# huggingface/diffusers

Measured on AMD Instinct MI355X. Metric: images/sec @ SDXL-base 1024x1024 50-step EulerDiscrete CFG bf16, higher is better.
Workload: dtype bf16

## Files before the change

diffusers_amd/_lib.py:

```python
from __future__ import annotations

import ctypes as C
import threading
from pathlib import Path

_PKG = Path(__file__).resolve().parent
LIB_PATH = _PKG / "_C" / "libdiffusers_amd.so"

DA_OK = 0
ERRORS = {1: "DA_ERR_INVALID", 2: "DA_ERR_LAUNCH", 3: "DA_ERR_UNSUPPORTED"}
ACT_NONE, ACT_GEGLU, ACT_GELU_TANH, ACT_SILU, ACT_GELU_ERF, ACT_QUICK_GELU, ACT_GEGLU_TANH = 0, 1, 2, 3, 4, 5, 6
(TILE_AUTO, TILE_128x128, TILE_64x128, TILE_128x64, TILE_64x64, TILE_256x128, TILE_128x256, TILE_256x256,
 TILE_128x128_W8, TILE_K2_128x128, TILE_K2_128x80, TILE_K2_128x160, TILE_K2_80x128, TILE_K2_128x64,
 TILE_K1_128x320, TILE_K1_256x128, TILE_K1_128x256, TILE_K1_256x160, TILE_K1_256x256, TILE_K1_256x320,
 TILE_K3_256x256, TILE_K3_256x320) = range(22)
TILE_NAMES = ("auto", "128x128", "64x128", "128x64", "64x64", "256x128", "128x256", "256x256", "128x128w8",
              "k2:128x128", "k2:128x80", "k2:128x160", "k2:80x128", "k2:128x64",
              "k1:128x320", "k1:256x128", "k1:128x256", "k1:256x160", "k1:256x256", "k1:256x320",
              "k3:256x256", "k3:256x320")
FIRST_K2_TILE = TILE_K2_128x128
STAGE_REGISTER, STAGE_LDS_DIRECT, STAGE_LDS_DIRECT3, STAGE_LDS_DIRECT4, STAGE_LDS_DIRECT6, STAGE_LDS_DIRECT8 = range(6)
STAGE_PINGPONG, STAGE_PINGPONG3 = 6, 7
RING_SLOTS = (2, 2, 3, 4, 6, 8)
DTYPE_BF16, DTYPE_F32 = 0, 1
SPLITK_FLAGS = 4096
SPLITK_ERR_SLOT = SPLITK_FLAGS - 1
SPLITK_MAX = 24
PRED_EPSILON, PRED_V, PRED_SAMPLE = 0, 1, 2
PRED_TYPES = {"epsilon": PRED_EPSILON, "v_prediction": PRED_V, "sample": PRED_SAMPLE}


class GemmParams(C.Structure):
    _fields_ = [
        ("A", C.c_void_p), ("A2", C.c_void_p), ("W", C.c_void_p), ("C", C.c_void_p),
        ("bias", C.c_void_p), ("rowvec", C.c_void_p), ("residual", C.c_void_p),
        ("bias_rows", C.c_void_p), ("gate", C.c_void_p),
        ("M", C.c_int), ("N", C.c_int), ("K", C.c_int),
        ("lda", C.c_int), ("ldw", C.c_int), ("ldc", C.c_int), ("ldr", C.c_int), ("ld_rowvec", C.c_int),
        ("ld_gate", C.c_int),
        ("rows_per_batch", C.c_int),
        ("alpha", C.c_float), ("out_scale", C.c_float),
        ("act", C.c_int), ("out_f32", C.c_int), ("conv", C.c_int),
        ("Hin", C.c_int), ("Win", C.c_int), ("C1", C.c_int), ("C2", C.c_int),
        ("Hout", C.c_int), ("Wout", C.c_int), ("stride", C.c_int), ("up", C.c_int), ("pad", C.c_int),
        ("tile", C.c_int), ("staging", C.c_int), ("gate_f32", C.c_int),
        ("split_k", C.c_int), ("workspace", C.c_void_p), ("sync_flags", C.c_void_p), ("workspace_bytes", C.c_longlong),
        ("stats_out", C.c_void_p), ("stats_ld", C.c_int), ("ln_stats", C.c_void_p), ("ln_stats_ld", C.c_int),
        ("ln_parts", C.c_int), ("ln_s", C.c_void_p), ("ln_c", C.c_void_p), ("ln_eps", C.c_float), ("k_valid", C.c_int),
        ("prefetch", C.c_void_p), ("prefetch_bytes", C.c_longlong),
        ("vt", C.c_void_p), ("vt_col0", C.c_int), ("ld_vt", C.c_longlong),
        ("xa_k", C.c_void_p), ("xa_vt", C.c_void_p), ("xa_skv", C.c_int), ("xa_skv_alloc", C.c_int), ("xa_k_ld", C.c_int),
        ("xa_vt_ld", C.c_longlong), ("xa_scale", C.c_float),
    ]


class AttentionParams(C.Structure):
    _fields_ = [
        ("q", C.c_void_p), ("k", C.c_void_p), ("vt", C.c_void_p), ("out", C.c_void_p),
        ("B", C.c_int), ("H", C.c_int), ("Sq", C.c_int), ("Skv", C.c_int), ("Skv_alloc", C.c_int), ("D", C.c_int),
        ("q_batch_stride", C.c_longlong), ("k_batch_stride", C.c_longlong),
        ("vt_batch_stride", C.c_longlong), ("o_batch_stride", C.c_longlong),
        ("q_row_stride", C.c_int), ("k_row_stride", C.c_int), ("vt_ld", C.c_int), ("o_row_stride", C.c_int),
        ("scale", C.c_float), ("ring_slots", C.c_int),
        ("bias", C.c_void_p), ("bias_batch_stride", C.c_longlong), ("bias_head_stride", C.c_longlong),
        ("bias_row_stride", C.c_int), ("bias_f32", C.c_int), ("causal", C.c_int), ("q_block", C.c_int), ("pv_delay", C.c_int),
        ("algo", C.c_int),
        ("split_ws", C.c_void_p), ("split_ws_bytes", C.c_longlong), ("kv_split", C.c_int),
    ]


ATTN_SPLIT_COUNTER_BYTES = 16384


PLAN_MAX_ARGS = 16
FN_IDS = {name: i + 1 for i, name in enumerate((
    "da_gemm_bf16", "da_gemm_pair_bf16", "da_attention_bf16", "da_groupnorm_nhwc_bf16", "da_rmsnorm_bf16", "da_layernorm_bf16",
    "da_rmsnorm_rope_bf16", "da_softmax_rows_f32_bf16", "da_rmsnorm_channels_bf16", "da_euler_scale_model_input", "da_euler_step",
    "da_x0_linear_step", "da_flowmatch_step", "da_unipc_flow_step", "da_advance_step", "da_cfg_rescale", "da_cast_f32_bf16",
    "da_mul_scalar", "da_bcast_add_f32", "da_patchify3d_bf16", "da_unpatchify3d_bf16", "da_transpose_bf16",
    "da_nhwc_take_nchw_bf16", "da_nhwc_take_postprocess", "da_permute_0213_bf16", "da_image_postprocess",
    "da_frames_to_ncthw_bf16", "da_timestep_embedding", "da_linear_small_m_bf16", "da_conv_thin_in_bf16",
    "da_conv_thin_out_bf16"))}
FN_COUNT = len(FN_IDS) + 1


class PlanOp(C.Structure):
    _fields_ = [("fn", C.c_int), ("reserved", C.c_int), ("arg", C.c_ulonglong * PLAN_MAX_ARGS)]


_vp, _i, _f, _ll = C.c_void_p, C.c_int, C.c_float, C.c_longlong

SIGNATURES = {
    "da_version": (_i, []),
    "da_sizeof_gemm_params": (C.c_size_t, []),
    "da_sizeof_attention_params": (C.c_size_t, []),
    "da_last_error": (C.c_char_p, []),
    "da_set_launch_events": (_i, [_vp, _vp]),
    "da_set_launch_flags": (_i, [C.c_uint]),
    "da_mfma_probe": (_i, [_i, _i, _vp, C.POINTER(C.c_double), _vp]),
    "da_gemm_bf16": (_i, [C.POINTER(GemmParams), _vp]),
    "da_gemm_pair_bf16": (_i, [C.POINTER(GemmParams), C.POINTER(GemmParams), _vp]),
    "da_gemm_stats_parts": (_i, [C.POINTER(GemmParams)]),
    "da_conv_chunk_channels": (_i, [C.POINTER(GemmParams), _i]),
    "da_gemm_tune": (_i, [C.POINTER(GemmParams), C.POINTER(GemmParams), _vp, _i, _vp, C.c_size_t, C.POINTER(C.c_int),
                          C.POINTER(C.c_int), C.POINTER(C.c_int), C.POINTER(C.c_float)]),
    "da_attention_bf16": (_i, [C.POINTER(AttentionParams), _vp]),
    "da_attention_split_plan": (_ll, [C.POINTER(AttentionParams), C.POINTER(C.c_int), C.POINTER(C.c_int), C.POINTER(C.c_int)]),
    "da_groupnorm_workspace_bytes": (C.c_size_t, [_i, _i, _i, _i]),
    "da_groupnorm_sync_bytes": (C.c_size_t, []),
    "da_groupnorm_nhwc_bf16": (_i, [_vp, _vp, _i, _vp, _vp, _vp, _vp, _i, _i, _i, _i, _f, _i, _vp, _vp]),
    "da_rmsnorm_bf16": (_i, [_vp, _vp, _vp, _i, _i, _i, _i, _f, _vp]),
    "da_layernorm_bf16": (_i, [_vp, _vp, _vp, _vp, _vp, _vp, _i, _i, _i, _i, _i, _i, _i, _f, _vp]),
    "da_rmsnorm_rope_bf16": (_i, [_vp, _i, _i, _i, _i, _i, _i, C.POINTER(C.c_int), C.POINTER(C.c_void_p), _f, _vp, _vp,
                                  _i, _i, _vp]),
    "da_softmax_rows_f32_bf16": (_i, [_vp, _vp, _i, _i, _ll, _ll, _vp]),
    "da_euler_scale_model_input": (_i, [_vp, _vp, _vp, _vp, _i, _ll, _i, _vp]),
    "da_euler_step": (_i, [_vp, _vp, _vp, _vp, _vp, _i, _f, _ll, _i, _i, _vp]),
    "da_x0_linear_step": (_i, [_vp, _vp, _vp, _ll, _vp, _vp, _vp, _i, _f, _ll, _i, _i, _vp]),
    "da_flowmatch_step": (_i, [_vp, _vp, _vp, _vp, _vp, _i, _f, _ll, _i, _i, _vp]),
    "da_unipc_flow_step": (_i, [_vp, _vp, _vp, _vp, _vp, _vp, _vp, _i, _f, _ll, _i, _i, _vp]),
    "da_advance_step": (_i, [_vp, _vp]),
    "da_cfg_rescale": (_i, [_vp, _vp, _vp, _i, _ll, _f, _f, _i, _vp]),
    "da_cast_f32_bf16": (_i, [_vp, _vp, _i, _ll, _vp]),
    "da_mul_scalar": (_i, [_vp, _vp, _f, _i, _ll, _i, _vp]),
    "da_bcast_add_f32": (_i, [_vp, _vp, _vp, _i, _i, _vp]),
    "da_patchify3d_bf16": (_i, [_vp, _vp, _i, _i, _i, _i, _i, _i, _i, _i, _vp]),
    "da_unpatchify3d_bf16": (_i, [_vp, _vp, _i, _i, _i, _i, _i, _i, _i, _i, _vp]),
    "da_transpose_bf16": (_i, [_vp, _vp, _i, _i, _ll, _ll, _vp]),
    "da_nhwc_take_nchw_bf16": (_i, [_vp, _vp, _ll, _ll, _i, _i, _vp]),
    "da_nhwc_take_postprocess": (_i, [_vp, _vp, _ll, _ll, _i, _i, _i, _vp]),
    "da_image_postprocess": (_i, [_vp, _vp, _i, _i, _ll, _i, _i, _vp]),
    "da_permute_0213_bf16": (_i, [_vp, _vp, _ll, _i, _i, _i, _vp]),
    "da_frames_to_ncthw_bf16": (_i, [_vp, _vp, _i, _i, _ll, _i, _i, _f, _f, _i, _vp]),
    "da_rmsnorm_channels_bf16": (_i, [_vp, _vp, _vp, _ll, _i, _f, _i, _vp]),
    "da_timestep_embedding": (_i, [_vp, _vp, _vp, _vp, _i, _i, _i, _f, _f, _f, _i, _vp]),
    "da_linear_small_m_bf16": (_i, [_vp, _vp, _vp, _vp, _vp, _i, _i, _i, _i, _i, _i, _i, _i, _vp]),
    "da_conv_thin_in_bf16": (_i, [_vp, _vp, _vp, _vp, _i, _i, _i, _i, _i, _i, _i, _f, _f, _vp]),
    "da_conv_thin_out_bf16": (_i, [_vp, _vp, _vp, _vp, _i, _i, _i, _i, _i, _i, _vp]),
    "da_vae_conv_in_image": (_i, [_vp, _i, _vp, _vp, _vp, _i, _i, _i, _i, _i, _vp]),
    "da_vae_posterior_latents": (_i, [_vp, _ll, _ll, _ll, _vp, _vp, _vp, _vp, _vp, _i, _ll, _i, _i, _i, _f, _f, _f, _f, _vp]),
    "da_plan_create": (_i, [C.POINTER(PlanOp), _i, C.POINTER(C.c_void_p)]),
    "da_plan_launch": (_i, [_vp, _vp, C.POINTER(C.c_int)]),
    "da_plan_relocate": (_i, [_vp, _i, C.POINTER(C.c_void_p), C.POINTER(C.c_ulonglong), C.POINTER(C.c_void_p),
                              C.POINTER(C.c_int)]),
    "da_plan_op_count": (_i, [_vp]),
    "da_plan_destroy": (None, [_vp]),
    "da_plan_arg_count": (_i, [_i]),
    "da_plan_arg_kinds": (C.c_char_p, [_i]),
}

IMAGE_F32_NCHW, IMAGE_F32_NHWC, IMAGE_U8_NHWC = 0, 1, 2
POSTERIOR_MOMENTS, POSTERIOR_MEAN, POSTERIOR_SAMPLE, POSTERIOR_NOISE = 0, 1, 2, 3
LATENTS_SHIFT, LATENTS_SCALE = 1, 2

ABI_VERSION = 6
_lib = None
_tls = threading.local()


def load() -> C.CDLL:
    global _lib
    rec = getattr(_tls, "recorder", None)
    if _lib is not None:
        return _lib if rec is None else rec.proxy
    if not LIB_PATH.exists():
        raise RuntimeError(
            f"{LIB_PATH} not found: the HIP extension is not built. Run `python -m diffusers_amd.build` "
            "(or __graft_entry__.build()). diffusers_amd has no CPU / PyTorch fallback path."
        )
    import torch
    lib = C.CDLL(str(LIB_PATH))
    for name, (res, args) in SIGNATURES.items():
        fn = getattr(lib, name)
        fn.restype = res
        fn.argtypes = args
    got = (lib.da_version(), lib.da_sizeof_gemm_params(), lib.da_sizeof_attention_params())
    want = (ABI_VERSION, C.sizeof(GemmParams), C.sizeof(AttentionParams))
    if got != want:
        raise RuntimeError(f"{LIB_PATH} has ABI (version, sizeof da_gemm_params, sizeof da_attention_params) = {got}, this package "
                           f"expects {want}: rebuild the extension (`python -m diffusers_amd.build`)")
    _lib = lib
    return lib if rec is None else rec.proxy


def check(status: int, what: str) -> None:
    if status != DA_OK:
        detail = ""
        if status == 2 and _lib is not None:
            detail = f" ({_lib.da_last_error().decode()})"
        raise RuntimeError(f"{what} failed: {ERRORS.get(status, status)}{detail}")
```

diffusers_amd/csrc/gemm.hip:

```cpp
#include "gemm_kernel.cuh"
#include "gemm2_shared.cuh"

namespace da_gemm {
int dispatch_conv(const da_gemm_params& p, int tile, int staging, hipStream_t s);
}
namespace da_gemm2 {
int dispatch_lin(const da_gemm_params& p, int tile, int staging, hipStream_t s);
int dispatch_conv(const da_gemm_params& p, int tile, int staging, hipStream_t s);
}
namespace da_gemm3 {
int dispatch_lin(const da_gemm_params& p, int tile, int staging, hipStream_t s);
}

namespace {

struct TileShape {
  int bm, bn, waves;
};
constexpr TileShape kTiles[] = {{0, 0, 0},      {128, 128, 4}, {64, 128, 4},  {128, 64, 4}, {64, 64, 4},
                                {256, 128, 8},  {128, 256, 8}, {256, 256, 8}, {128, 128, 8},
                                {128, 128, 8},  {128, 80, 8},  {128, 160, 8}, {80, 128, 8}, {128, 64, 8},
                                {128, 320, 8},  {256, 128, 8}, {128, 256, 8}, {256, 160, 8}, {256, 256, 8}, {256, 320, 8},
                                {256, 256, 8},  {256, 320, 8}};
static_assert(sizeof(kTiles) / sizeof(kTiles[0]) == DA_TILE_COUNT, "kTiles / DA_TILE_* mismatch");
inline bool is_k3(int tile) { return tile == DA_TILE_K3_256x256 || tile == DA_TILE_K3_256x320; }
inline bool is_k2(int tile) { return tile >= DA_TILE_K2_128x128 && !is_k3(tile); }
constexpr int kNumTiles = sizeof(kTiles) / sizeof(kTiles[0]);

int pick_tile(const da_gemm_params& p) {
  auto nblk = [&](int t) {
    return (long)((p.M + kTiles[t].bm - 1) / kTiles[t].bm) * ((p.N + kTiles[t].bn - 1) / kTiles[t].bn);
  };
  const bool geglu = (p.act == DA_ACT_GEGLU || p.act == DA_ACT_GEGLU_TANH);
  const bool narrow = !geglu && ((p.N & 127) != 0) && ((p.N % 128) <= 64);
  if (narrow) return (nblk(DA_TILE_128x64) >= 200) ? DA_TILE_128x64 : DA_TILE_64x64;
  if (nblk(DA_TILE_256x128) >= 480) return DA_TILE_256x128;
  if (nblk(DA_TILE_128x128) >= 128) return DA_TILE_128x128;
  if (nblk(DA_TILE_64x128) >= 128 || geglu) return DA_TILE_64x128;
  return DA_TILE_64x64;
}

int validate_conv(const da_gemm_params& p) {
  if (p.C1 <= 0 || (p.C1 & 63) || (p.C2 & 63) || p.C2 < 0) return DA_ERR_UNSUPPORTED;
  if (p.conv != 1 && p.conv != 3) return DA_ERR_UNSUPPORTED;
  if (p.K != p.conv * p.conv * (p.C1 + p.C2)) return DA_ERR_INVALID;
  if (p.stride != 1 && p.stride != 2) return DA_ERR_UNSUPPORTED;
  if (p.up != 0 && p.up != 1) return DA_ERR_INVALID;
  if (p.Hin <= 0 || p.Win <= 0 || p.Hout <= 0 || p.Wout <= 0) return DA_ERR_INVALID;
  if (p.M % (p.Hout * p.Wout)) return DA_ERR_INVALID;
  return DA_OK;
}

int validate(da_gemm_params& p) {
  if (p.M <= 0 || p.N <= 0 || p.K <= 0) return DA_ERR_INVALID;
  if ((p.K & 63) || (p.N & 3) || (p.ldc & 3)) return DA_ERR_UNSUPPORTED;
  if (!p.A || !p.W || !p.C) return DA_ERR_INVALID;
  if (p.residual && (p.ldr & 3)) return DA_ERR_UNSUPPORTED;
  if (p.rowvec && (p.rows_per_batch <= 0 || (p.ld_rowvec & 3))) return DA_ERR_INVALID;
  if (p.gate && (p.rows_per_batch <= 0 || (p.ld_gate & 3))) return DA_ERR_INVALID;
  if (p.alpha == 0.0f) p.alpha = 1.0f;
  if (p.out_scale == 0.0f) p.out_scale = 1.0f;
  if (p.conv) {
    const int v = validate_conv(p);
    if (v != DA_OK) return v;
    if (p.C2 > 0 && !p.A2) return DA_ERR_INVALID;
  } else {
    if ((p.lda & 7) || (p.ldw & 7)) return DA_ERR_UNSUPPORTED;
  }
  if ((p.act == DA_ACT_GEGLU || p.act == DA_ACT_GEGLU_TANH) &&
      ((p.N & 127) || p.out_f32 || p.residual || p.rowvec || p.gate || p.bias_rows))
    return DA_ERR_UNSUPPORTED;
  if (p.act < 0 || p.act > DA_ACT_GEGLU_TANH) return DA_ERR_INVALID;
  if (p.split_k < 0 || p.split_k > DA_SPLITK_MAX) return DA_ERR_INVALID;
  if (p.split_k > 1 && (p.stats_out || p.ln_stats)) return DA_ERR_UNSUPPORTED;
  if (p.k_valid < 0 || (p.k_valid > 0 && (p.k_valid > (p.conv ? p.C1 : p.K) || (p.conv && p.C2 != 0)))) return DA_ERR_INVALID;
  if (p.stats_out && (p.conv || p.out_f32 || p.act == DA_ACT_GEGLU || p.act == DA_ACT_GEGLU_TANH || p.stats_ld <= 0 || (p.stats_ld & 1)))
    return DA_ERR_UNSUPPORTED;
  if (p.ln_stats && (p.conv || !p.ln_s || !p.ln_c || p.ln_parts <= 0 || p.ln_parts > 4 * DA_LN_PAIR_LOADS ||
                     p.ln_stats_ld < 2 * DA_LN_MAX_PARTS || (p.ln_stats_ld & 3)))
    return DA_ERR_INVALID;
  return DA_OK;
}

int stats_parts(const da_gemm_params& p, int tile) {
  if (is_k2(tile)) {
    const int band = (tile == DA_TILE_K2_128x80 || tile == DA_TILE_K2_128x160) ? 80 : 0;
    return band ? (p.N + band - 1) / band : 0;
  }
  return (p.N + kTiles[tile].bn - 1) / kTiles[tile].bn;
}

bool tile_ok(const da_gemm_params& p, int tile) {
  if (tile <= 0 || tile >= kNumTiles) return false;
  if (is_k3(tile)) {
    if (p.conv || p.split_k > 1 || p.stats_out || (p.ln_stats && tile != DA_TILE_K3_256x320) || p.vt || p.xa_k) return false;
    if (tile == DA_TILE_K3_256x320)
      return (p.act == DA_ACT_GEGLU || p.act == DA_ACT_GEGLU_TANH) && (p.M % 256) == 0 && (p.N % 320) == 0 && !(p.ldc & 7) &&
             !((size_t)p.C & 15);
    return true;
  }
  if (is_k2(tile)) {
    const bool geglu = (p.act == DA_ACT_GEGLU || p.act == DA_ACT_GEGLU_TANH);
    const bool geglu_ok = tile == DA_TILE_K2_128x128 || tile == DA_TILE_K1_256x128 || tile == DA_TILE_K1_128x256 ||
                          tile == DA_TILE_K1_256x256 || tile == DA_TILE_K1_256x320 || (tile == DA_TILE_K1_128x320 && !p.conv);
    const bool lnf_lin = tile == DA_TILE_K2_128x80 || tile == DA_TILE_K2_128x160;
    const bool lnf_cons = lnf_lin || tile == DA_TILE_K1_128x256 || tile == DA_TILE_K1_256x128;
    if (p.xa_k) return !p.conv && p.split_k <= 1 && !geglu && !p.stats_out && !p.vt && tile == DA_TILE_K2_128x128;
    if (p.vt) return !p.conv && p.split_k <= 1 && !geglu && !p.stats_out && lnf_cons;
    if (p.stats_out || p.ln_stats) {
      if (p.conv || p.split_k > 1) return false;
      if (p.stats_out && (geglu || !lnf_lin)) return false;
      return geglu ? tile == DA_TILE_K1_128x320 : lnf_cons;
    }
    return p.split_k <= 1 && (!geglu || geglu_ok) &&
           !(p.conv && (tile == DA_TILE_K2_80x128 || tile == DA_TILE_K1_256x256 || tile == DA_TILE_K1_256x320));
  }
  if (p.vt || p.xa_k) return false;
  if ((p.act == DA_ACT_GEGLU || p.act == DA_ACT_GEGLU_TANH) &&
      (tile == DA_TILE_128x64 || tile == DA_TILE_64x64 || tile == DA_TILE_128x128_W8))
    return false;
  if (tile == DA_TILE_256x256 && (p.stats_out || p.ln_stats)) return false;
  return true;
}

__global__ __launch_bounds__(256) void touch_kernel(const uint4* __restrict__ src, size_t n, unsigned* __restrict__ sink) {
  unsigned acc = 0;
  for (size_t i = (size_t)blockIdx.x * 256 + threadIdx.x; i < n; i += (size_t)gridDim.x * 256) {
    const uint4 v = src[i];
    acc ^= v.x ^ v.y ^ v.z ^ v.w;
  }
  if (acc == 0x9e3779b9u) sink[0] = acc;
}

int run(const da_gemm_params& p, int tile, int staging, hipStream_t s, const da_gemm_params* pb = nullptr) {
  if (is_k3(tile)) return pb ? DA_ERR_UNSUPPORTED : da_gemm3::dispatch_lin(p, tile, staging, s);
  if (is_k2(tile)) {
    if (pb) return DA_ERR_UNSUPPORTED;
    return p.conv ? da_gemm2::dispatch_conv(p, tile, staging, s) : da_gemm2::dispatch_lin(p, tile, staging, s);
  }
  if (p.conv) return pb ? DA_ERR_UNSUPPORTED : da_gemm::dispatch_conv(p, tile, staging, s);
  return da_gemm::dispatch<false>(p, tile, staging, s, pb);
}

}

extern "C" int da_gemm_bf16(const da_gemm_params* pp, void* stream) {
  if (!pp) return DA_ERR_INVALID;
  da_gemm_params p = *pp;
  const int v = validate(p);
  if (v != DA_OK) return v;
  int tile = p.tile;
  if (tile == DA_TILE_AUTO) tile = pick_tile(p);
  if (!tile_ok(p, tile)) return DA_ERR_UNSUPPORTED;
  if (p.stats_out && (stats_parts(p, tile) <= 0 || p.stats_ld < 2 * stats_parts(p, tile))) return DA_ERR_INVALID;
  return run(p, tile, p.staging, (hipStream_t)stream);
}

extern "C" int da_gemm_stats_parts(const da_gemm_params* pp) {
  if (!pp || pp->N <= 0) return 0;
  int tile = pp->tile;
  if (tile == DA_TILE_AUTO) tile = pick_tile(*pp);
  if (tile <= 0 || tile >= kNumTiles) return 0;
  return stats_parts(*pp, tile);
}

extern "C" int da_conv_chunk_channels(const da_gemm_params* pp, int tile) {
  if (!pp || !pp->conv || pp->M <= 0 || pp->N <= 0) return -DA_ERR_INVALID;
  const da_gemm_params& p = *pp;
  const int v = validate_conv(p);
  if (v != DA_OK) return -v;
  if (!is_k2(tile) || !tile_ok(p, tile)) return -DA_ERR_UNSUPPORTED;
  return da_gemm2::conv_chunk_channels(p, kTiles[tile].bm, kTiles[tile].bn);
}

extern "C" int da_gemm_pair_bf16(const da_gemm_params* pa, const da_gemm_params* pb, void* stream) {
  if (!pa || !pb) return DA_ERR_INVALID;
  da_gemm_params a = *pa, b = *pb;
  int v = validate(a);
  if (v != DA_OK) return v;
  v = validate(b);
  if (v != DA_OK) return v;
  if (a.conv || b.conv || a.split_k > 1 || b.split_k > 1) return DA_ERR_UNSUPPORTED;
  int tile = a.tile;
  if (tile == DA_TILE_AUTO) tile = pick_tile(a);
  if (!tile_ok(a, tile) || !tile_ok(b, tile)) return DA_ERR_UNSUPPORTED;
  return run(a, tile, a.staging, (hipStream_t)stream, &b);
}

extern "C" int da_gemm_tune(const da_gemm_params* pp, const da_gemm_params* pair, void* stream, int iters, void* scratch,
                            size_t scratch_bytes, int* best_tile, int* best_staging, int* best_split, float* best_us) {
  if (!pp || !best_tile || !best_staging) return DA_ERR_INVALID;
  da_gemm_params p = *pp;
  int v = validate(p);
  if (v != DA_OK) return v;
  da_gemm_params pb{};
  if (pair) {
    pb = *pair;
    v = validate(pb);
    if (v != DA_OK) return v;
    if (p.conv || pb.conv) return DA_ERR_UNSUPPORTED;
  }
  if (iters <= 0) iters = 3;
  hipStream_t s = (hipStream_t)stream;
  hipEvent_t e0, e1;
  if (hipEventCreate(&e0) != hipSuccess || hipEventCreate(&e1) != hipSuccess) return DA_ERR_LAUNCH;
  float best = 3.0e38f;
  int bt = 0, bs = 0, bk = 1;
  static const int stagings[] = {DA_STAGE_LDS_DIRECT, DA_STAGE_LDS_DIRECT3, DA_STAGE_LDS_DIRECT4, DA_STAGE_LDS_DIRECT6,
                                 DA_STAGE_LDS_DIRECT8, DA_STAGE_PINGPONG, DA_STAGE_PINGPONG3};
  constexpr int n_stagings = sizeof(stagings) / sizeof(stagings[0]);
  static const int splits[] = {1, 2, 3, 4, 6, 8, 12, 16, 24};
  const int n_splits = (best_split && !pair && p.workspace && p.sync_flags) ? (int)(sizeof(splits) / sizeof(splits[0])) : 1;
  const int family = pp->tile;
  for (int spi = 0; spi < n_splits; ++spi) {
    const int split = splits[spi];
    p.split_k = split;
    for (int tile = 1; tile < kNumTiles; ++tile) {
      if ((family == DA_TILE_FAMILY_1 && (is_k2(tile) || is_k3(tile))) || (family == DA_TILE_FAMILY_K2 && !is_k2(tile) && !is_k3(tile))) continue;
      if (!tile_ok(p, tile) || (pair && !tile_ok(pb, tile))) continue;
      if (kTiles[tile].bm >= 2 * p.M + 64 || kTiles[tile].bn >= 2 * p.N + 64) continue;
      if (split > 1) {
        const long tiles = (long)((p.M + kTiles[tile].bm - 1) / kTiles[tile].bm) * ((p.N + kTiles[tile].bn - 1) / kTiles[tile].bn);
        if (tiles >= 256 || (p.K >> 6) < 4 * split) continue;
      }
      for (int si = 0; si < n_stagings; ++si) {
        const int st = stagings[si];
        int rc = run(p, tile, st, s, pair ? &pb : nullptr);
        if (rc == DA_ERR_UNSUPPORTED || (split > 1 && rc == DA_ERR_INVALID)) continue;
        if (rc != DA_OK) { (void)hipEventDestroy(e0); (void)hipEventDestroy(e1); return rc; }
        float tmin = 3.0e38f;
        for (int it = 0; it < iters; ++it) {
          if (scratch && scratch_bytes) {
            (void)hipMemsetAsync(scratch, 0, scratch_bytes, s);
            const da_gemm_params* both[2] = {&p, pair ? &pb : nullptr};
            for (int w = 0; w < 2; ++w) {
              if (!both[w]) continue;
              const da_gemm_params& q = *both[w];
              const size_t na = q.conv ? (size_t)(q.M / ((size_t)q.Hout * q.Wout)) * q.Hin * q.Win * q.C1 * 2
                                       : ((size_t)(q.M - 1) * q.lda + q.K) * 2;
              if (na <= ((size_t)192 << 20))
                DA_LAUNCH(touch_kernel, dim3(1024), dim3(256), 0, s, (const uint4*)q.A, na / 16, (unsigned*)scratch);
            }
          }
          (void)hipEventRecord(e0, s);
          rc = run(p, tile, st, s, pair ? &pb : nullptr);
          (void)hipEventRecord(e1, s);
// ... 20 lines not shown
```

diffusers_amd/csrc/gemm2_kernel.cuh:

```cuda
#pragma once
#include <cstdlib>
#include <type_traits>

#include "common.cuh"
#include "diffusers_amd.h"
#include "gemm2_shared.cuh"

namespace da_gemm2 {


#if defined(DA_GEMM2_TRACE)
__device__ unsigned long long* g_da2_trace;
#define DA2_TRACE(i) tr_[i] = __builtin_readcyclecounter()
#else
#define DA2_TRACE(i) ((void)0)
#endif



template <int KG, int WM, int WN, int MT, int NT, int NSLOT, bool CONV, bool PP = false, bool STREAMW = false, bool GIL = false,
          bool LNF = false, int XA = 0>
__global__ __launch_bounds__(512) void igemm2_bf16_kernel(const da_gemm_params p, const int xcd_gx_chunk) {
#if defined(__HIP_DEVICE_COMPILE__)
  const int xcd_gx = xcd_gx_chunk & 255;
  static_assert((KG == 1 || KG == 2) && KG * WM * WN == 8, "eight waves: one or two K-groups");
  constexpr int BM = 16 * MT * WM, BN = 16 * NT * WN;
  constexpr int PX = BM / 8, PW = BN / 8;
  constexpr int XBYTES = BM * 128, SLICE = (BM + BN) * 128, PAIR = KG * SLICE;
  static_assert(!PP || KG == 2, "ping-pong is a property of the two K-groups");
  static_assert(!STREAMW || (KG == 1 && NSLOT == 2 && !CONV), "streaming-W loop: one K-group, two-slice ring, nn.Linear");
  static_assert(!GIL || (KG == 1 && !CONV && WN == 2 && (NT % 2) == 0), "GEGLU-interleaved ownership: two wave columns, value / gate tile pairs");
  static_assert(!LNF || (!CONV && !STREAMW), "LayerNorm fold: nn.Linear instantiations of the ring loops");
  static_assert(XA == 0 || (LNF && KG == 2 && WM == 2 && WN == 2 && MT == 4 && NT == 4 && NSLOT == 2 && XA <= 8),
                "cross-attention epilogue: the 128 x 128 two-K-group tile (a wave finishes 32 rows x one 64-wide head)");
  constexpr int SW = PP ? 4 : 8;
  constexpr int UX = PP ? PX : KG * PX, UW = PP ? PW : KG * PW;
  constexpr int XI = (UX + SW - 1) / SW, WI = (UW + SW - 1) / SW;
  constexpr int XRAG = UX % SW ? 1 : 0, WRAG = UW % SW ? 1 : 0;
  static_assert(NSLOT == 2 || NSLOT == 3, "ring of 2 or 3 slice pairs");
  constexpr int DUMP = 1024;
  constexpr int LNSC = LNF ? 2 * BN * 4 : 0;
  constexpr int XA_K_OFF = 4 * MT * NT * 1024, XA_KB = XA * 16 * 128, XA_V_OFF = XA_K_OFF + 32768;
  static_assert(XA == 0 || (2 * XA_KB <= 32768 && XA_V_OFF + 32768 <= NSLOT * PAIR), "cross-attention operands do not fit the ring");
  static_assert(NSLOT * PAIR + DUMP + LNSC <= 160 * 1024, "LDS ring exceeds the 160 KiB of a CU");
  static_assert(BM % 8 == 0 && BN % 8 == 0, "tile rows are staged in 8-row pieces");
  static_assert(!CONV || (UX % SW) == 0, "conv: the slice of an activation piece must be a compile-time constant");
  static_assert((NSLOT - 1) * (XI + WI) <= 63, "vmcnt is a 6-bit counter");
  static_assert(KG == 1 || MT * NT * 1024 * 4 <= NSLOT * PAIR, "partial-sum exchange does not fit the ring");
  extern __shared__ __attribute__((aligned(16))) unsigned char smem[];

#if defined(DA_GEMM2_TRACE)
  unsigned long long tr_[8] = {0, 0, 0, 0, 0, 0, 0, 0};
#endif
  DA2_TRACE(0);
  const int t = threadIdx.x;
  const int lane = t & 63, wave = __builtin_amdgcn_readfirstlane(t >> 6);
  const int g = KG == 2 ? wave >> 2 : 0, wq = KG == 2 ? wave & 3 : wave;
  const int wm = wq / WN, wn = wq - wm * WN;
  const int r16 = lane & 15, kq = lane >> 4;

  const int tiles_n = (p.N + BN - 1) / BN, tiles_m = (p.M + BM - 1) / BM;
  const int gyn = 8 / xcd_gx;
  const int tm_per = (tiles_m + gyn - 1) / gyn, tn_per = (tiles_n + xcd_gx - 1) / xcd_gx;
  const int bid = (int)blockIdx.x;
  const int xcd = bid & 7, kblk = bid >> 3;
  const int gy = xcd / xcd_gx, gx = xcd - gy * xcd_gx;
  const int lm = kblk / tn_per, ln = kblk - lm * tn_per;
  const int tm = gy * tm_per + lm, tn = gx * tn_per + ln;
  if (tm >= tiles_m || tn >= tiles_n) return;
  const int m0 = tm * BM, n0 = tn * BN;

  const uint16_t* __restrict__ A = (const uint16_t*)p.A;
  const uint16_t* __restrict__ A2 = (const uint16_t*)p.A2;
  const uint16_t* __restrict__ Wt = (const uint16_t*)p.W;
  const int nk = p.K >> 6;
  const int nk2 = (nk + KG - 1) / KG;
  const int Ctot = CONV ? (p.C1 + p.C2) : 0;
  const int Hv = CONV ? (p.Hin << p.up) : 0, Wv = CONV ? (p.Win << p.up) : 0;

  int x_h[XI], x_r[XI], w_h[WI], w_r[WI];
  bool x_ok[XI], w_ok[WI];
#pragma unroll
  for (int i = 0; i < XI; ++i) {
    const int q = i * SW + (PP ? wq : wave);
    x_ok[i] = (i * SW + SW - 1 < UX) ? true : (q < UX);
    x_h[i] = (KG == 1 || PP) ? 0 : (i * 8 >= PX) ? 1 : (i * 8 + 7 < PX) ? 0 : (q >= PX ? 1 : 0);
    x_r[i] = q - x_h[i] * PX;
    if (!x_ok[i]) x_h[i] = 0, x_r[i] = 0;
  }
#pragma unroll
  for (int i = 0; i < WI; ++i) {
    const int q = i * SW + (PP ? wq : wave);
    w_ok[i] = (i * SW + SW - 1 < UW) ? true : (q < UW);
    w_h[i] = (KG == 1 || PP) ? 0 : (i * 8 >= PW) ? 1 : (i * 8 + 7 < PW) ? 0 : (q >= PW ? 1 : 0);
    w_r[i] = q - w_h[i] * PW;
    if (!w_ok[i]) w_h[i] = 0, w_r[i] = 0;
  }
  const int own_half = PP ? g * SLICE : 0;
  constexpr int my_loads = XI + WI;

  int xr_base[XI], xr_oy[XI], xr_ox[XI];
  if constexpr (CONV) {
    const int hw = p.Hout * p.Wout;
#pragma unroll
    for (int i = 0; i < XI; ++i) {
      const int m = m0 + x_r[i] * 8 + (lane >> 3);
      if (m < p.M) {
        const int b = m / hw;
        const int rem = m - b * hw;
        const int oy = rem / p.Wout;
        xr_base[i] = b * p.Hin;
        xr_oy[i] = oy * p.stride - p.pad;
        xr_ox[i] = (rem - oy * p.Wout) * p.stride - p.pad;
      } else {
        xr_base[i] = 0;
// ... 73 lines not shown
    if (PP) {
      if (g == 1 && nk > 1) cursor_step(0);
    } else if (KG == 2 && nk > 1) {
      cursor_step(1);
    }
    tap_offsets(0);
    if (KG == 2 && !PP) tap_offsets(1);
  }
  int st_woff[2] = {CONV ? w_off(0) : 0, CONV ? w_off(1) : 0};

#define DA2_LDS(ptr) ((__attribute__((address_space(3))) void*)(ptr))
  auto stage_issue_base = [&](unsigned char* base, auto which_c) {
    constexpr int WHICH = decltype(which_c)::value;
    auto issue_x = [&](auto ic) {
      constexpr int i = decltype(ic)::value;
      const int h = x_h[i];
      const int z = x_ok[i] ? (h ? st_zero[1] : st_zero[0]) : (int)0x80000000;
      unsigned char* dst = x_ok[i] ? base + own_half + h * SLICE + x_r[i] * 1024 : smem + NSLOT * PAIR;
      if constexpr (CONV) {
        const int c0 = h ? c_c0[1] : c_c0[0];
        if (p.C2 > 0 && c0 >= p.C1)
          __builtin_amdgcn_raw_ptr_buffer_load_lds(rs_x2, DA2_LDS(dst), 16, vo_x2[i] | z, (c0 - p.C1) * 2, 0, 0);
        else
          __builtin_amdgcn_raw_ptr_buffer_load_lds(rs_x, DA2_LDS(dst), 16, vo_x[i] | z, c0 * 2, 0, 0);
      } else {
        __builtin_amdgcn_raw_ptr_buffer_load_lds(rs_x, DA2_LDS(dst), 16, vo_x[i] | z, (h ? st_s[1] : st_s[0]) * 128, 0, 0);
      }
    };
    auto issue_w = [&](auto ic) {
      constexpr int i = decltype(ic)::value;
      const int h = w_h[i];
      const int z = w_ok[i] ? (h ? st_zero[1] : st_zero[0]) : (int)0x80000000;
      unsigned char* dst = w_ok[i] ? base + own_half + h * SLICE + XBYTES + w_r[i] * 1024 : smem + NSLOT * PAIR;
      if constexpr (CONV)
        __builtin_amdgcn_raw_ptr_buffer_load_lds(rs_w, DA2_LDS(dst), 16, vo_w[i] | z, h ? st_woff[1] : st_woff[0], 0, 0);
      else
        __builtin_amdgcn_raw_ptr_buffer_load_lds(rs_w, DA2_LDS(dst), 16, vo_w[i] | z, (h ? st_s[1] : st_s[0]) * 128, 0, 0);
    };
    if constexpr (WHICH >= 0) {
      if constexpr (WHICH < WI) issue_w(std::integral_constant<int, WHICH < WI ? WHICH : 0>{});
      else issue_x(std::integral_constant<int, WHICH >= WI ? WHICH - WI : 0>{});
    } else {
      static_for<XI>(issue_x);
      static_for<WI>(issue_w);
    }
  };
  auto stage_issue = [&](int slot) { stage_issue_base(smem + slot * PAIR, std::integral_constant<int, -1>{}); };
  auto stage_issue_one = [&](unsigned char* base, auto k_c) { stage_issue_base(base, k_c); };
  auto stage_advance = [&]() {
    ++st_pr;
#pragma unroll
    for (int h = 0; h < (PP ? 1 : KG); ++h) {
      const int want = min(KG * st_pr + (PP ? g : h), nk - 1);
      if constexpr (CONV) {
        const int kh0 = c_kh[h], kw0 = c_kw[h];
        while (st_s[h] < want) {
          cursor_step(h);
          ++st_s[h];
        }
        if (c_kh[h] != kh0 || c_kw[h] != kw0) tap_offsets(h);
        st_woff[h] = w_off(h);
      } else {
        st_s[h] = want;
      }
    }
    st_zero[0] = (KG * st_pr + (PP ? g : 0) < nk) ? 0 : (int)0x80000000;
    st_zero[1] = (KG * st_pr + 1 < nk) ? 0 : (int)0x80000000;
  };
#define DA2_WAIT_PAIRS(PAIRS) asm volatile("s_waitcnt vmcnt(%0)" ::"n"((PAIRS) * my_loads) : "memory")

  constexpr bool SPLIT_M = KG == 1 || (MT % 2) == 0;
  static_assert(SPLIT_M || (NT % 2) == 0, "one of the wave tile's dimensions must split between the two K-groups");
  constexpr int MH = (KG == 2 && SPLIT_M) ? MT / 2 : MT, NH = (KG == 1 || SPLIT_M) ? NT : NT / 2;
  const bool geglu = (p.act == DA_ACT_GEGLU || p.act == DA_ACT_GEGLU_TANH);
  auto row_of = [&](int ih) { return m0 + (wm * MT + (SPLIT_M ? g * MH : 0) + ih) * 16 + r16; };
  auto col_tile = [&](int jh) { return GIL ? 4 * (jh >> 1) + 2 * (jh & 1) + wn : wn * NT + (SPLIT_M ? 0 : g * NH) + jh; };
  auto col_of = [&](int jh) { return n0 + col_tile(jh) * 16 + 4 * kq; };
  constexpr bool PF = MH * NH <= (CONV ? 8 : 12);
  constexpr bool STG = NH >= 2;
  constexpr int PPR = 2 * NH, NPIECE = 16 * PPR, TT = (NPIECE + 63) / 64, ROWB = NH * 64 + 32;
  static_assert(!STG || (KG == 2 ? 4 * MT * NT * 1024 : 0) + 8 * 16 * ROWB <= NSLOT * PAIR, "output staging does not fit the ring");
  constexpr int STATS_OFF = (KG == 2 ? 4 * MT * NT * 1024 : 0) + 8 * 16 * ROWB;
  static_assert(!(LNF && STG) || STATS_OFF + 8 * TT * 64 * 8 <= NSLOT * PAIR, "statistics scratch does not fit the ring");
  const bool wide = STG && !GIL && !geglu && !p.out_f32 && !(p.ldc & 7) && !((size_t)p.C & 15) && !(p.N & 7) &&
                    (!p.residual || (!(p.ldr & 7) && !((size_t)p.residual & 15)));
  const int band_col0 = n0 + (wn * NT + (SPLIT_M ? 0 : g * NH)) * 16;
  auto band_row0 = [&](int ih) { return m0 + (wm * MT + (SPLIT_M ? g * MH : 0) + ih) * 16; };
  constexpr bool PFN = PF && !STG;
  uint2 res_v[PFN ? MH : 1][PFN ? NH : 1], bias_v[NH], rowvec_v[PF ? MH : 1][PF ? NH : 1];
  uint4 resw[(PF && STG) ? MH : 1][(PF && STG) ? TT : 1];
#pragma unroll
  for (int ih = 0; ih < (PF ? MH : 1); ++ih)
#pragma unroll
    for (int jh = 0; jh < (PF ? NH : 1); ++jh) rowvec_v[ih][jh] = make_uint2(0, 0);
#pragma unroll
  for (int ih = 0; ih < (PFN ? MH : 1); ++ih)
#pragma unroll
    for (int jh = 0; jh < (PFN ? NH : 1); ++jh) res_v[ih][jh] = make_uint2(0, 0);
#pragma unroll
  for (int ih = 0; ih < ((PF && STG) ? MH : 1); ++ih)
#pragma unroll
    for (int t = 0; t < ((PF && STG) ? TT : 1); ++t) resw[ih][t] = make_uint4(0, 0, 0, 0);
#pragma unroll
  for (int jh = 0; jh < NH; ++jh) bias_v[jh] = make_uint2(0, 0);
  constexpr bool LN_PF = LNF;
  float4 lnq[LN_PF ? MH : 1][3];
#pragma unroll
  for (int ih = 0; ih < (LN_PF ? MH : 1); ++ih)
#pragma unroll
    for (int u = 0; u < 3; ++u) lnq[ih][u] = make_float4(0.f, 0.f, 0.f, 0.f);
  auto ln_load = [&](int ih, float4* dst) {
    const int m = min(row_of(ih), p.M - 1);
    const float* sp = p.ln_stats + (size_t)m * p.ln_stats_ld;
#pragma unroll
    for (int u = 0; u < 3; ++u) dst[u] = *(const float4*)(sp + ((6 * kq + 2 * u < p.ln_parts) ? 12 * kq + 4 * u : 0));
  };
  float4 lnsc_v = make_float4(0.f, 0.f, 0.f, 0.f);
  auto prefetch_epilogue_operands = [&]() {
    if constexpr (LNF) {
      if (p.ln_stats) {
        if (t < BN / 2) {
          const int j = t < BN / 4 ? t : t - BN / 4;
          const int n = min(n0 + 4 * j, p.N - 4);
          lnsc_v = *(const float4*)((t < BN / 4 ? p.ln_s : p.ln_c) + n);
        }
      }
    }
    if constexpr (LN_PF) {
      if (p.ln_stats) {
#pragma unroll
        for (int ih = 0; ih < MH; ++ih) ln_load(ih, lnq[ih]);
      }
    }
    const uint16_t* __restrict__ resid = (const uint16_t*)p.residual;
    const uint16_t* __restrict__ bias = (const uint16_t*)p.bias;
    const uint16_t* __restrict__ rowvec = (const uint16_t*)p.rowvec;
    if constexpr (PFN) {
      if (resid) {
#pragma unroll
        for (int ih = 0; ih < MH; ++ih) {
          const int m = min(row_of(ih), p.M - 1);
#pragma unroll
          for (int jh = 0; jh < NH; ++jh) res_v[ih][jh] = *(const uint2*)(resid + (size_t)m * p.ldr + min(col_of(jh), p.N - 4));
        }
      }
    }
    if constexpr (PF && STG) {
      if (resid && wide) {
#pragma unroll
        for (int ih = 0; ih < MH; ++ih)
#pragma unroll
          for (int t = 0; t < TT; ++t) {
            const int q = (NPIECE % 64 == 0) ? lane + 64 * t : min(lane + 64 * t, NPIECE - 1);
            const int m = min(band_row0(ih) + q / PPR, p.M - 1), n = min(band_col0 + (q % PPR) * 8, p.N - 8);
            resw[ih][t] = *(const uint4*)(resid + (size_t)m * p.ldr + n);
          }
      }
    }
    if (!STREAMW && bias) {
#pragma unroll
      for (int jh = 0; jh < NH; ++jh) bias_v[jh] = *(const uint2*)(bias + min(col_of(jh), p.N - 4));
    }
    if (PF && rowvec) {
#pragma unroll
      for (int ih = 0; ih < (PF ? MH : 0); ++ih) {
        const int m = min(row_of(ih), p.M - 1);
// ... 420 lines not shown
          for (int u = 0; u < NT / 2; ++u) {
            const uint2 bh = bias_v[2 * u], bg = bias_v[2 * u + 1];
            float o[4], hq[4], gq[4];
#pragma unroll
            for (int e = 0; e < 4; ++e) hq[e] = keep[ih][2 * u][e] * p.alpha, gq[e] = keep[ih][2 * u + 1][e] * p.alpha;
            ln_apply4(hq, ih, min(col_of(2 * u), p.N - 4));
            ln_apply4(gq, ih, min(col_of(2 * u + 1), p.N - 4));
#pragma unroll
            for (int e = 0; e < 4; ++e) {
              float hv = hq[e], gv = gq[e];
              hv += (e == 0) ? bf_lo(bh.x) : (e == 1) ? bf_hi(bh.x) : (e == 2) ? bf_lo(bh.y) : bf_hi(bh.y);
              gv += (e == 0) ? bf_lo(bg.x) : (e == 1) ? bf_hi(bg.x) : (e == 2) ? bf_lo(bg.y) : bf_hi(bg.y);
              hv = bf2f(f2bf(hv));
              gv = bf2f(f2bf(gv));
              o[e] = hv * bf2f(f2bf(TANH ? gelu_tanh_f(gv) : gelu_erf_f(gv)));
            }
            uint2 pk;
            pk.x = pack_bf2(o[0], o[1]);
            pk.y = pack_bf2(o[2], o[3]);
            *(uint2*)(orow + u * 64) = pk;
          }
        }
      };
      if (p.act == DA_ACT_GEGLU) body(std::false_type{});
      else body(std::true_type{});
      asm volatile("s_waitcnt lgkmcnt(0)" ::: "memory");
      __builtin_amdgcn_s_barrier();
      asm volatile("" ::: "memory");
      constexpr int OPR = BN / 16, NOP = BM * OPR;
      const int no0 = n0 >> 1, Nout = p.N >> 1;
#pragma unroll
      for (int k = 0; k < (NOP + 511) / 512; ++k) {
        const int q = t + 512 * k;
        if (NOP % 512 != 0 && q >= NOP) continue;
        const int row = q / OPR, c = q % OPR;
        if (m0 + row >= p.M || no0 + c * 8 >= Nout) continue;
        *(uint4*)((uint16_t*)p.C + (size_t)(m0 + row) * p.ldc + no0 + c * 8) = *(const uint4*)(smem + row * OROW + c * 16);
      }
      DA2_TRACE_END();
      return;
    }
    if constexpr (!GIL && SPLIT_M && (NT % 4) == 0) {
      auto body = [&](auto tanh_c) __attribute__((always_inline)) {
        constexpr bool TANH = decltype(tanh_c)::value;
#pragma unroll
        for (int ih = 0; ih < MH; ++ih) {
          const int m = row_of(ih);
          if (m >= p.M) continue;
#pragma unroll
          for (int u = 0; u < NT / 4; ++u)
#pragma unroll
            for (int v = 0; v < 2; ++v) {
              const int jv = 4 * u + v, jg = jv + 2;
              const int nv = col_of(jv);
              if (nv >= p.N) continue;
              const int no = (n0 >> 1) + (wn * (NT / 4) + u) * 32 + v * 16 + 4 * kq;
              const uint2 bh = bias_v[jv], bg = bias_v[jg];
              float o[4], hq[4], gq[4];
#pragma unroll
              for (int e = 0; e < 4; ++e) hq[e] = keep[ih][jv][e] * p.alpha, gq[e] = keep[ih][jg][e] * p.alpha;
              ln_apply4(hq, ih, nv);
              ln_apply4(gq, ih, col_of(jg));
#pragma unroll
              for (int e = 0; e < 4; ++e) {
                float hv = hq[e], gv = gq[e];
                hv += (e == 0) ? bf_lo(bh.x) : (e == 1) ? bf_hi(bh.x) : (e == 2) ? bf_lo(bh.y) : bf_hi(bh.y);
                gv += (e == 0) ? bf_lo(bg.x) : (e == 1) ? bf_hi(bg.x) : (e == 2) ? bf_lo(bg.y) : bf_hi(bg.y);
                hv = bf2f(f2bf(hv));
                gv = bf2f(f2bf(gv));
                o[e] = hv * bf2f(f2bf(TANH ? gelu_tanh_f(gv) : gelu_erf_f(gv)));
              }
              uint2 pk;
              pk.x = pack_bf2(o[0], o[1]);
              pk.y = pack_bf2(o[2], o[3]);
              *(uint2*)((uint16_t*)p.C + (size_t)m * p.ldc + no) = pk;
            }
        }
      };
      if (p.act == DA_ACT_GEGLU) body(std::false_type{});
      else body(std::true_type{});
    }
    return;
  }
  auto wide_body = [&](auto act_c, auto gate_c, auto packed_c) __attribute__((always_inline)) {
    constexpr int ACT = decltype(act_c)::value, GATE = decltype(gate_c)::value;
    constexpr bool PACKED = decltype(packed_c)::value;
    if constexpr (STG) {
      if constexpr (KG == 1) {
        asm volatile("s_waitcnt lgkmcnt(0)" ::: "memory");
        __builtin_amdgcn_s_barrier();
        asm volatile("" ::: "memory");
      }
      unsigned char* stg = smem + ((KG == 2 && !xa_on) ? 4 * MT * NT * 1024 : 0) + wave * (16 * ROWB);
      unsigned char* stg_w = stg + r16 * ROWB + kq * 16;
      const uint16_t* __restrict__ resid = (const uint16_t*)p.residual;
#pragma unroll
      for (int ih = 0; ih < MH; ++ih) {
        const int mc = min(row_of(ih), p.M - 1);
        const int bidx = (GATE != 0 || (!PF && has_rowvec)) ? (mc / p.rows_per_batch) : 0;
        const float brow = bias_rows ? bf2f(bias_rows[mc]) : 0.f;
#pragma unroll
        for (int jh = 0; jh < NH; ++jh) {
          const int n = min(col_of(jh), p.N - 4);
          float o[4];
          if (XA > 0 && xa_on) {
#pragma unroll
            for (int e = 0; e < 4; ++e) o[e] = keep[ih][jh][e];
          } else {
#pragma unroll
          for (int e = 0; e < 4; ++e) o[e] = keep[ih][jh][e] * p.alpha;
          ln_apply4(o, ih, n);
          uint2 rvv = make_uint2(0, 0);
          if constexpr (PF) rvv = rowvec_v[ih][jh];
          else if (has_rowvec) rvv = *(const uint2*)((const uint16_t*)p.rowvec + (size_t)bidx * p.ld_rowvec + n);
          epilogue4<ACT, GATE, false>(p, o, n, bidx, brow, bias_v[jh], rvv, make_uint2(0, 0));
          }
          if constexpr (PACKED) {
            uint2 pk;
            pk.x = pack_bf2(o[0], o[1]);
            pk.y = pack_bf2(o[2], o[3]);
            *(uint2*)(stg + r16 * (ROWB / 2) + kq * 8 + jh * 32) = pk;
          } else {
            *(float4*)(stg_w + jh * 64) = make_float4(o[0], o[1], o[2], o[3]);
          }
        }
        float2* part = (float2*)(smem + STATS_OFF) + wave * (TT * 64);
#pragma unroll
        for (int t = 0; t < TT; ++t) {
          const int q = lane + 64 * t;
          if (NPIECE % 64 != 0 && q >= NPIECE) continue;
          const int row = q / PPR, c8 = q % PPR;
          const int mo = band_row0(ih) + row, no = band_col0 + c8 * 8;
          const bool inside = mo < p.M && no < p.N;
          uint4 pk;
          if constexpr (PACKED) {
            pk = *(const uint4*)(stg + row * (ROWB / 2) + c8 * 16);
          } else {
            const float4 lo = *(const float4*)(stg + row * ROWB + c8 * 32), hi = *(const float4*)(stg + row * ROWB + c8 * 32 + 16);
            float o[8] = {lo.x, lo.y, lo.z, lo.w, hi.x, hi.y, hi.z, hi.w};
            uint4 rw = make_uint4(0, 0, 0, 0);
            if constexpr (PF) rw = resw[ih][t];
            else if (has_res && inside) rw = *(const uint4*)(resid + (size_t)mo * p.ldr + no);
            o[0] += bf_lo(rw.x); o[1] += bf_hi(rw.x); o[2] += bf_lo(rw.y); o[3] += bf_hi(rw.y);
            o[4] += bf_lo(rw.z); o[5] += bf_hi(rw.z); o[6] += bf_lo(rw.w); o[7] += bf_hi(rw.w);
#pragma unroll
            for (int e = 0; e < 8; ++e) o[e] *= p.out_scale;
            pk.x = pack_bf2(o[0], o[1]); pk.y = pack_bf2(o[2], o[3]); pk.z = pack_bf2(o[4], o[5]); pk.w = pack_bf2(o[6], o[7]);
          }
          if (inside) *(uint4*)((uint16_t*)p.C + (size_t)mo * p.ldc + no) = pk;
          if constexpr (LNF) {
            if (p.stats_out) {
              float r[8];
              unpack8(pk, r);
              const float s1 = ((r[0] + r[1]) + (r[2] + r[3])) + ((r[4] + r[5]) + (r[6] + r[7]));
              const float s2 = ((r[0] * r[0] + r[1] * r[1]) + (r[2] * r[2] + r[3] * r[3])) +
                               ((r[4] * r[4] + r[5] * r[5]) + (r[6] * r[6] + r[7] * r[7]));
              part[q] = inside ? make_float2(s1, s2) : make_float2(0.f, 0.f);
            }
          }
        }
        if constexpr (LNF) {
          if (p.stats_out) {
            asm volatile("s_waitcnt lgkmcnt(0)" ::: "memory");
            if (lane < 16) {
              float a = 0.f, b = 0.f;
#pragma unroll
              for (int c = 0; c < PPR; ++c) {
                const float2 v = part[lane * PPR + c];
                a += v.x;
                b += v.y;
              }
              const int mo = band_row0(ih) + lane;
              if (mo < p.M && band_col0 < p.N)
                *(float2*)(p.stats_out + (size_t)mo * p.stats_ld + 2 * (band_col0 / (16 * NH))) = make_float2(a, b);
            }
            asm volatile("s_waitcnt lgkmcnt(0)" ::: "memory");
          }
        }
      }
    }
  };
  auto narrow_body = [&](auto act_c, auto gate_c) __attribute__((always_inline)) {
    constexpr int ACT = decltype(act_c)::value, GATE = decltype(gate_c)::value;
#pragma unroll
    for (int ih = 0; ih < MH; ++ih) {
      const int m = row_of(ih);
      if (m >= p.M) continue;
      const int bidx = (GATE != 0 || (!PF && has_rowvec)) ? (m / p.rows_per_batch) : 0;
      const float brow = bias_rows ? bf2f(bias_rows[m]) : 0.f;
#pragma unroll
      for (int jh = 0; jh < NH; ++jh) {
        const int n = col_of(jh);
        if (n >= p.N) continue;
        float o[4];
#pragma unroll
        for (int e = 0; e < 4; ++e) o[e] = keep[ih][jh][e] * p.alpha;
        ln_apply4(o, ih, n);
        uint2 rvv = make_uint2(0, 0), rsv = make_uint2(0, 0);
        if constexpr (PF) rvv = rowvec_v[ih][jh];
        else if (has_rowvec) rvv = *(const uint2*)((const uint16_t*)p.rowvec + (size_t)bidx * p.ld_rowvec + n);
        if constexpr (PFN) rsv = res_v[ih][jh];
        else if (has_res) rsv = *(const uint2*)((const uint16_t*)p.residual + (size_t)m * p.ldr + n);
        epilogue4<ACT, GATE, true>(p, o, n, bidx, brow, bias_v[jh], rvv, rsv);
        if (p.out_f32) {
          *(float4*)((float*)p.C + (size_t)m * p.ldc + n) = make_float4(o[0], o[1], o[2], o[3]);
        } else {
          uint2 pk;
          pk.x = pack_bf2(o[0], o[1]);
          pk.y = pack_bf2(o[2], o[3]);
          *(uint2*)((uint16_t*)p.C + (size_t)m * p.ldc + n) = pk;
        }
      }
    }
  };
  if constexpr (LNF && !GIL) {
    if (p.vt && n0 >= p.vt_col0) {
      uint16_t* __restrict__ vt = (uint16_t*)p.vt;
#pragma unroll
      for (int ih = 0; ih < MH; ++ih) {
        const int m = row_of(ih);
#pragma unroll
        for (int jh = 0; jh < NH; ++jh) {
          const int n = col_of(jh);
          if (n >= p.N) continue;
          float o[4];
#pragma unroll
          for (int e = 0; e < 4; ++e) o[e] = keep[ih][jh][e] * p.alpha;
          ln_apply4(o, ih, n);
          const uint2 bv = bias_v[jh];
          o[0] += bf_lo(bv.x); o[1] += bf_hi(bv.x); o[2] += bf_lo(bv.y); o[3] += bf_hi(bv.y);
          if (m < p.M) {
            uint16_t* dst = vt + (size_t)(n - p.vt_col0) * p.ld_vt + m;
#pragma unroll
            for (int e = 0; e < 4; ++e) dst[(size_t)e * p.ld_vt] = f2bf(o[e]);
          }
        }
      }
      DA2_TRACE_END();
      return;
    }
  }
  {
    using std::integral_constant;
    auto by_act = [&](auto&& f, auto... tail) __attribute__((always_inline)) {
      if (p.act == DA_ACT_NONE) f(integral_constant<int, DA_ACT_NONE>{}, tail...);
      else if (p.act == DA_ACT_GELU_TANH) f(integral_constant<int, DA_ACT_GELU_TANH>{}, tail...);
      else if (p.act == DA_ACT_SILU) f(integral_constant<int, DA_ACT_SILU>{}, tail...);
      else if (p.act == DA_ACT_GELU_ERF) f(integral_constant<int, DA_ACT_GELU_ERF>{}, tail...);
      else f(integral_constant<int, DA_ACT_QUICK_GELU>{}, tail...);
    };
    constexpr integral_constant<int, -1> RT{};
    constexpr integral_constant<int, 0> G0{};
    if (STG && wide) {
      const bool packed = !has_res && p.out_scale == 1.0f;
      if (p.gate && p.gate_f32) wide_body(RT, integral_constant<int, 2>{}, std::false_type{});
      else if (p.gate) wide_body(RT, integral_constant<int, 1>{}, std::false_type{});
      else if (packed) by_act(wide_body, G0, std::true_type{});
      else by_act(wide_body, G0, std::false_type{});
    } else {
      if (p.gate && p.gate_f32) narrow_body(RT, integral_constant<int, 2>{});
      else if (p.gate) narrow_body(RT, integral_constant<int, 1>{});
      else if constexpr (STG) narrow_body(RT, G0);
      else by_act(narrow_body, G0);
    }
  }
  DA2_TRACE_END();
#undef DA2_TRACE_END
#undef DA2_LDS
#undef DA2_WAIT_PAIRS
#undef DA2_SG_DS
#undef DA2_SG_MF
#undef DA2_SG_VM
#endif
}



template <int KG, int WM, int WN, int MT, int NT, int NSLOT, bool CONV, bool PP = false, bool STREAMW = false, bool GIL = false,
          bool LNF = false, int XA = 0>
int launch(const da_gemm_params& p, hipStream_t s) {
  constexpr int BM = 16 * MT * WM, BN = 16 * NT * WN;
  const LaunchGeom geom = launch_geom(p, BM, BN, CONV);
  constexpr size_t lds = (size_t)NSLOT * KG * (BM + BN) * 128 + 1024 + (LNF ? 2 * BN * 4 : 0);
  auto kern = igemm2_bf16_kernel<KG, WM, WN, MT, NT, NSLOT, CONV, PP, STREAMW, GIL, LNF, XA>;
  static bool attr_set = false;
  if (!attr_set) {
    if (hipFuncSetAttribute((const void*)kern, hipFuncAttributeMaxDynamicSharedMemorySize, (int)lds) != hipSuccess)
      return DA_ERR_LAUNCH;
    attr_set = true;
  }
  DA_LAUNCH(kern, dim3(geom.grid), dim3(512), lds, s, p, geom.gx | (CONV ? conv_chunk_slices(p, geom.rows_xcd) << 8 : 0));
  DA_CHECK_LAUNCH();
  return DA_OK;
}

inline int stats_band_cols(int tile) { return (tile == DA_TILE_K2_128x80 || tile == DA_TILE_K2_128x160) ? 80 : 0; }

inline int dispatch_lnf(const da_gemm_params& p, int tile, int staging, hipStream_t s) {
  const bool geglu = (p.act == DA_ACT_GEGLU || p.act == DA_ACT_GEGLU_TANH);
  const int ns = (staging == DA_STAGE_LDS_DIRECT || staging == DA_STAGE_PINGPONG) ? 2
                 : (staging == DA_STAGE_LDS_DIRECT3 || staging == DA_STAGE_PINGPONG3) ? 3 : 0;
  const bool pp = staging == DA_STAGE_PINGPONG || staging == DA_STAGE_PINGPONG3;
  if (ns == 0) return DA_ERR_UNSUPPORTED;
  if (p.xa_k) {
    if (tile != DA_TILE_K2_128x128 || ns != 2 || geglu || !p.xa_vt || p.vt || p.stats_out || p.residual || p.gate || p.rowvec ||
        p.bias_rows || p.out_f32 || p.act != DA_ACT_NONE || p.out_scale != 1.0f || (p.N & 127) || (p.ldc & 7) ||
        ((size_t)p.C & 15) || p.rows_per_batch <= 0 || (p.rows_per_batch & 127) || (p.M % p.rows_per_batch) || p.xa_skv <= 0 ||
        p.xa_skv > p.xa_skv_alloc || p.xa_skv_alloc > 80 || (p.xa_skv_alloc & 7) || (p.xa_k_ld & 7) || (p.xa_vt_ld & 7) ||
        p.xa_k_ld < p.N || p.xa_vt_ld < (long long)(p.M / p.rows_per_batch) * p.xa_skv_alloc ||
        ((size_t)p.xa_k & 15) || ((size_t)p.xa_vt & 15) ||
        (size_t)(p.M / p.rows_per_batch) * p.xa_skv_alloc * p.xa_k_ld * 2 >= 0x7fffffffull || (size_t)p.N * p.xa_vt_ld * 2 >= 0x7fffffffull)
      return DA_ERR_UNSUPPORTED;
    return pp ? launch<2, 2, 2, 4, 4, 2, false, true, false, false, true, 5>(p, s)
              : launch<2, 2, 2, 4, 4, 2, false, false, false, false, true, 5>(p, s);
  }
  if (p.vt) {
    const int bn = tile == DA_TILE_K2_128x80 ? 80 : tile == DA_TILE_K2_128x160 ? 160 : tile == DA_TILE_K1_128x256 ? 256
                   : tile == DA_TILE_K1_256x128 ? 128 : 0;
    if (bn == 0 || geglu || p.stats_out || p.residual || p.gate || p.rowvec || p.bias_rows || p.out_f32 || p.act != DA_ACT_NONE ||
        p.vt_col0 <= 0 || p.vt_col0 >= p.N || (p.vt_col0 % bn) || (p.vt_col0 & 15) || p.ld_vt < p.M || p.out_scale != 1.0f)
      return DA_ERR_UNSUPPORTED;
  }
  if (p.stats_out) {
    if (geglu || p.out_f32 || (p.ldc & 7) || ((size_t)p.C & 15) || (p.N & 7) || p.gate ||
        (p.residual && ((p.ldr & 7) || ((size_t)p.residual & 15))) || stats_band_cols(tile) == 0)
      return DA_ERR_UNSUPPORTED;
  }
  switch (tile) {
    case DA_TILE_K2_128x80:
      if (geglu) break;
      if (pp) return ns == 2 ? launch<2, 4, 1, 2, 5, 2, false, true, false, false, true>(p, s)
                             : launch<2, 4, 1, 2, 5, 3, false, true, false, false, true>(p, s);
      return ns == 2 ? launch<2, 4, 1, 2, 5, 2, false, false, false, false, true>(p, s)
                     : launch<2, 4, 1, 2, 5, 3, false, false, false, false, true>(p, s);
    case DA_TILE_K2_128x160:
      if (geglu || ns != 2) break;
      return pp ? launch<2, 2, 2, 4, 5, 2, false, true, false, false, true>(p, s)
                : launch<2, 2, 2, 4, 5, 2, false, false, false, false, true>(p, s);
    case DA_TILE_K1_128x320:
      if (!geglu || p.stats_out || ns != 2 || pp || (p.ldc & 7) || ((size_t)p.C & 15) || (p.N & 15)) break;
      return launch<1, 4, 2, 2, 10, 2, false, false, false, true, true>(p, s);
    case DA_TILE_K1_128x256:
      if (geglu || p.stats_out || pp) break;
      return ns == 2 ? launch<1, 2, 4, 4, 4, 2, false, false, false, false, true>(p, s)
                     : launch<1, 2, 4, 4, 4, 3, false, false, false, false, true>(p, s);
    case DA_TILE_K1_256x128:
      if (geglu || p.stats_out || pp) break;
      return ns == 2 ? launch<1, 4, 2, 4, 4, 2, false, false, false, false, true>(p, s)
                     : launch<1, 4, 2, 4, 4, 3, false, false, false, false, true>(p, s);
  }
  return DA_ERR_UNSUPPORTED;
}

template <bool CONV>
int dispatch(const da_gemm_params& p, int tile, int staging, hipStream_t s) {
  if (p.split_k > 1 || !staging_fits(p)) return DA_ERR_UNSUPPORTED;
  if (p.stats_out || p.ln_stats || p.vt || p.xa_k) {
    if constexpr (CONV) return DA_ERR_UNSUPPORTED;
    else return dispatch_lnf(p, tile, staging, s);
  }
  const bool geglu = (p.act == DA_ACT_GEGLU || p.act == DA_ACT_GEGLU_TANH);
  if (geglu && tile != DA_TILE_K2_128x128 && tile != DA_TILE_K1_256x128 && tile != DA_TILE_K1_128x256 && tile != DA_TILE_K1_256x256 &&
      tile != DA_TILE_K1_256x320 && tile != DA_TILE_K1_128x320)
    return DA_ERR_UNSUPPORTED;
  const int ns = (staging == DA_STAGE_LDS_DIRECT || staging == DA_STAGE_PINGPONG) ? 2
                 : (staging == DA_STAGE_LDS_DIRECT3 || staging == DA_STAGE_PINGPONG3) ? 3 : 0;
  if (ns == 0) return DA_ERR_UNSUPPORTED;
  if (staging == DA_STAGE_PINGPONG || staging == DA_STAGE_PINGPONG3) {
    switch (tile) {
      case DA_TILE_K2_128x128:
        if (ns == 2) return launch<2, 2, 2, 4, 4, 2, CONV, true>(p, s);
        break;
      case DA_TILE_K2_128x80:
        return ns == 2 ? launch<2, 4, 1, 2, 5, 2, CONV, true>(p, s) : launch<2, 4, 1, 2, 5, 3, CONV, true>(p, s);
      case DA_TILE_K2_128x160:
        if (ns == 2) return launch<2, 2, 2, 4, 5, 2, CONV, true>(p, s);
        break;
      case DA_TILE_K2_80x128:
        if constexpr (!CONV) return ns == 2 ? launch<2, 1, 4, 5, 2, 2, false, true>(p, s) : launch<2, 1, 4, 5, 2, 3, false, true>(p, s);
        break;
      case DA_TILE_K2_128x64:
        return ns == 2 ? launch<2, 2, 2, 4, 2, 2, CONV, true>(p, s) : launch<2, 2, 2, 4, 2, 3, CONV, true>(p, s);
    }
    return DA_ERR_UNSUPPORTED;
  }
  switch (tile) {
    case DA_TILE_K2_128x128:
      if (ns == 2) return launch<2, 2, 2, 4, 4, 2, CONV>(p, s);
      break;
    case DA_TILE_K2_128x80:
      return ns == 2 ? launch<2, 4, 1, 2, 5, 2, CONV>(p, s) : launch<2, 4, 1, 2, 5, 3, CONV>(p, s);
    case DA_TILE_K2_128x160:
      if (ns == 2) return launch<2, 2, 2, 4, 5, 2, CONV>(p, s);
      break;
    case DA_TILE_K2_80x128:
      if constexpr (!CONV) return ns == 2 ? launch<2, 1, 4, 5, 2, 2, false>(p, s) : launch<2, 1, 4, 5, 2, 3, false>(p, s);
      break;
    case DA_TILE_K2_128x64:
      return ns == 2 ? launch<2, 2, 2, 4, 2, 2, CONV>(p, s) : launch<2, 2, 2, 4, 2, 3, CONV>(p, s);
    case DA_TILE_K1_128x320:
      if (ns != 2) break;
      if (!geglu) return launch<1, 4, 2, 2, 10, 2, CONV>(p, s);
      if constexpr (!CONV) {
        if ((p.ldc & 7) || ((size_t)p.C & 15) || (p.N & 15)) break;
        return launch<1, 4, 2, 2, 10, 2, false, false, false, true>(p, s);
      }
      break;
    case DA_TILE_K1_256x128:
      return ns == 2 ? launch<1, 4, 2, 4, 4, 2, CONV>(p, s) : launch<1, 4, 2, 4, 4, 3, CONV>(p, s);
    case DA_TILE_K1_128x256:
      return ns == 2 ? launch<1, 2, 4, 4, 4, 2, CONV>(p, s) : launch<1, 2, 4, 4, 4, 3, CONV>(p, s);
    case DA_TILE_K1_256x160:
      if (ns == 2) return launch<1, 4, 2, 4, 5, 2, CONV>(p, s);
      break;
    case DA_TILE_K1_256x320:
      if constexpr (!CONV) {
        if (ns != 2) break;
        if (!geglu) return launch<1, 4, 2, 4, 10, 2, false, false, true, false>(p, s);
        if ((p.ldc & 7) || ((size_t)p.C & 15) || (p.N & 15)) break;
        return launch<1, 4, 2, 4, 10, 2, false, false, true, true>(p, s);
      }
      break;
    case DA_TILE_K1_256x256:
      if constexpr (!CONV) {
        if (ns == 2) return launch<1, 2, 4, 8, 4, 2, false>(p, s);
      }
      break;
  }
  return DA_ERR_UNSUPPORTED;
}

}
```

diffusers_amd/csrc/norm.hip:

```cpp
#include <cstdlib>

#include "common.cuh"

namespace {

__global__ void gn_stats_kernel(const uint16_t* __restrict__ x, const uint16_t* __restrict__ x2, int C1,
                                float* __restrict__ ws, int HW, int C, int G, int pix_per_blk, int krows) {
  extern __shared__ __attribute__((aligned(16))) float sm[];
  const int cpr = C >> 3;
  const int t = threadIdx.x;
  const int cc = t % cpr, prow = t / cpr;
  const int b = blockIdx.y, blk = blockIdx.x;
  const int p0 = blk * pix_per_blk;
  const int p1 = min(HW, p0 + pix_per_blk);
  float s[8], q[8];
#pragma unroll
  for (int e = 0; e < 8; ++e) s[e] = q[e] = 0.f;
  const bool second = (cc * 8 >= C1);
  const int Cs = second ? (C - C1) : C1;
  const uint16_t* xb = (second ? x2 + (size_t)(cc * 8 - C1) : x + (size_t)cc * 8) + (size_t)b * HW * Cs;
  for (int pix = p0 + prow; pix < p1; pix += 4 * krows) {
    uint4 v[4];
#pragma unroll
    for (int u = 0; u < 4; ++u) {
// ... 625 lines not shown
  if (!on) return f;
  const int cpg = C / G;
  int gs = 1;
  while (gs <= 4 && ((gs * cpg) & 7)) ++gs;
  if (gs > 4 || (G % gs)) return f;
  const int cw = gs * cpg, nch = cw / 8;
  int lcm = 64;
  while (lcm % nch) lcm += 64;
  if (lcm > 1024) return f;
  const int threads = (1024 / lcm) * lcm;
  const size_t slab = (size_t)HW * cw * 2;
  const long long wgs = (long long)B * (G / gs);
  if (wgs < min_wg) return f;
  const bool res = slab <= 144 * 1024;
  if (!res && multi && have_sync && gs <= 2 && wgs <= kGnSyncCounters) {
    int parts = 2;
    while (parts <= 32 && (size_t)((HW + parts - 1) / parts) * cw * 2 > 144 * 1024) parts *= 2;
    while (parts * 2 <= 32 && wgs * parts * 2 <= 256 && (HW + parts * 2 - 1) / (parts * 2) >= 4 * (threads / nch)) parts *= 2;
    if (parts <= 32 && wgs * parts <= 256) {
      f.gs = gs, f.threads = threads, f.resident = 1, f.parts = parts;
      f.lds = (size_t)((HW + parts - 1) / parts) * cw * 2;
      return f;
    }
  }
  if (!res && slab > (size_t)max_kb * 1024) return f;
  f.gs = gs, f.threads = threads, f.resident = res, f.lds = res ? slab : 0;
  return f;
}

extern "C" size_t da_groupnorm_workspace_bytes(int B, int HW, int C, int G) {
  if (B <= 0 || HW <= 0 || C <= 0 || G <= 0) return 0;
  GnPlan g = gn_plan(B, HW, C);
  return (size_t)B * g.nblk * G * 2 * sizeof(float);
}

extern "C" size_t da_groupnorm_sync_bytes(void) { return kGnSyncBytes; }

extern "C" int da_groupnorm_nhwc_bf16(const void* x, const void* x2, int C1, const void* gamma, const void* beta,
                                      void* y, void* workspace, int B, int HW, int C, int G, float eps, int act,
                                      void* sync, void* stream) {
  if (!x || !gamma || !beta || !y || !workspace) return DA_ERR_INVALID;
  if (!x2) C1 = C;
  if (C1 <= 0 || C1 > C || (C1 & 7) || (x2 == nullptr && C1 != C)) return DA_ERR_INVALID;
  if (B <= 0 || HW <= 0 || C <= 0 || G <= 0 || G > 64 || (C % G) || (C & 7)) return DA_ERR_UNSUPPORTED;
  if (C / 8 > 512) return DA_ERR_UNSUPPORTED;
  hipStream_t s = (hipStream_t)stream;
  const GnFused ff = gn_fused_plan(B, HW, C, C1, G, sync != nullptr);
  if (ff.gs) {
    const dim3 grid(G / ff.gs, B, ff.parts), block(ff.threads);
#define DA_GNF(GS_, RES_)                                                                                              \
  do {                                                                                                                 \
    auto kern = gn_fused_kernel<GS_, RES_>;                                                                            \
    static bool attr_set = false;                                                                                      \
    if (RES_ && !attr_set) {                                                                                           \
      if (hipFuncSetAttribute((const void*)kern, hipFuncAttributeMaxDynamicSharedMemorySize, 144 * 1024) != hipSuccess) \
        return DA_ERR_LAUNCH;                                                                                          \
      attr_set = true;                                                                                                 \
    }                                                                                                                  \
    DA_LAUNCH(kern, grid, block, ff.lds, s, (const uint16_t*)x, (const uint16_t*)x2, C1, (const uint16_t*)gamma,       \
              (const uint16_t*)beta, (uint16_t*)y, HW, C, G, eps, act, (unsigned char*)sync);                          \
  } while (0)
    if (ff.resident) {
      if (ff.gs == 1) DA_GNF(1, true); else if (ff.gs == 2) DA_GNF(2, true); else if (ff.gs == 3) DA_GNF(3, true); else DA_GNF(4, true);
    } else {
      if (ff.gs == 1) DA_GNF(1, false); else if (ff.gs == 2) DA_GNF(2, false); else if (ff.gs == 3) DA_GNF(3, false); else DA_GNF(4, false);
    }
#undef DA_GNF
    DA_CHECK_LAUNCH();
    return DA_OK;
  }
  GnPlan g = gn_plan(B, HW, C);
  const size_t lds = (size_t)g.krows * C * 2 * sizeof(float);
  if (lds > 64 * 1024) return DA_ERR_UNSUPPORTED;
  DA_LAUNCH(gn_stats_kernel, dim3(g.nblk, B), dim3(g.threads), lds, s, (const uint16_t*)x, (const uint16_t*)x2,
                     C1, (float*)workspace, HW, C, G, g.pix_per_blk, g.krows);
  DA_CHECK_LAUNCH();
  DA_LAUNCH(gn_apply_kernel, dim3(g.nblk, B), dim3(g.threads), 0, s, (const uint16_t*)x,
                     (const uint16_t*)x2, C1, (const uint16_t*)gamma, (const uint16_t*)beta, (uint16_t*)y, (const float*)workspace, g.nblk, HW,
                     C, G, eps, act, g.pix_per_blk, g.krows);
  DA_CHECK_LAUNCH();
  return DA_OK;
}

template <int NCH>
__global__ __launch_bounds__(256) void rmsnorm_rows_kernel(const uint16_t* __restrict__ x, const uint16_t* __restrict__ gamma,
                                                           uint16_t* __restrict__ y, int M, int C, int ldx, int ldy, float eps) {
  const int lane = threadIdx.x & 63;
  const int row = blockIdx.x * 4 + (threadIdx.x >> 6);
  if (row >= M) return;
  const int nchunks = C >> 3;
  float v[NCH][8];
  const uint16_t* xr = x + (size_t)row * ldx;
  float sq = 0.f;
  uint4 xq[NCH];
#pragma unroll
  for (int i = 0; i < NCH; ++i) xq[i] = *(const uint4*)(xr + min(lane + 64 * i, nchunks - 1) * 8);
#pragma unroll
  for (int i = 0; i < NCH; ++i) {
    const int ch = lane + 64 * i;
    unpack8(xq[i], v[i]);
    if (ch < nchunks) {
#pragma unroll
      for (int e = 0; e < 8; ++e) sq += v[i][e] * v[i][e];
    }
  }
  sq = wave_sum(sq);
  const float rstd = rsqrtf(sq / (float)C + eps);
  uint16_t* yr = y + (size_t)row * ldy;
#pragma unroll
  for (int i = 0; i < NCH; ++i) {
    const int ch = lane + 64 * i;
    if (ch < nchunks) {
      float g[8], o[8];
      unpack8(*(const uint4*)(gamma + ch * 8), g);
#pragma unroll
      for (int e = 0; e < 8; ++e) o[e] = g[e] * bf2f(f2bf(v[i][e] * rstd));
      *(uint4*)(yr + ch * 8) = pack8(o);
    }
  }
}

extern "C" int da_rmsnorm_bf16(const void* x, const void* gamma, void* y, int M, int C, int ldx, int ldy, float eps,
                               void* stream) {
  if (!x || !gamma || !y) return DA_ERR_INVALID;
  if (M <= 0 || C <= 0 || (C & 7) || (ldx & 7) || (ldy & 7)) return DA_ERR_UNSUPPORTED;
  hipStream_t s = (hipStream_t)stream;
  const int nch = (C / 8 + 63) / 64;
  dim3 grid((M + 3) / 4), block(256);
#define DA_RMS(N) \
  DA_LAUNCH(rmsnorm_rows_kernel<N>, grid, block, 0, s, (const uint16_t*)x, (const uint16_t*)gamma, (uint16_t*)y, M, C, ldx, ldy, eps)
  if (nch <= 1) DA_RMS(1);
  else if (nch <= 2) DA_RMS(2);
  else if (nch <= 4) DA_RMS(4);
  else if (nch <= 8) DA_RMS(8);
  else return DA_ERR_UNSUPPORTED;
#undef DA_RMS
  DA_CHECK_LAUNCH();
  return DA_OK;
}

extern "C" int da_layernorm_bf16(const void* x, const void* gamma, const void* beta, void* y, const void* mod_scale,
                                 const void* mod_shift, int mod_ld, int mod_f32, int rows_per_batch, int M, int C,
                                 int ldx, int ldy, float eps, void* stream) {
  if (!x || !y) return DA_ERR_INVALID;
  if (M <= 0 || C <= 0 || (C & 7) || (ldx & 7) || (ldy & 7)) return DA_ERR_UNSUPPORTED;
  if ((mod_scale == nullptr) != (mod_shift == nullptr)) return DA_ERR_INVALID;
  if (mod_scale && (rows_per_batch <= 0 || (mod_ld & 7))) return DA_ERR_INVALID;
  hipStream_t s = (hipStream_t)stream;
  const int nch = (C / 8 + 63) / 64;
  dim3 grid((M + 3) / 4), block(256);
#define DA_LN(N)                                                                                                  \
  DA_LAUNCH(layernorm_kernel<N>, grid, block, 0, s, (const uint16_t*)x, (const uint16_t*)gamma,          \
                     (const uint16_t*)beta, (uint16_t*)y, (const uint16_t*)mod_scale, (const uint16_t*)mod_shift, \
                     mod_ld, mod_f32, rows_per_batch, M, C, ldx, ldy, eps)
  if (nch <= 1) DA_LN(1);
  else if (nch <= 2) DA_LN(2);
  else if (nch <= 3) DA_LN(3);
  else if (nch <= 4) DA_LN(4);
  else if (nch <= 6) DA_LN(6);
  else if (nch <= 8) DA_LN(8);
  else return DA_ERR_UNSUPPORTED;
#undef DA_LN
  DA_CHECK_LAUNCH();
  return DA_OK;
}

// ... 55 lines not shown
```

diffusers_amd/csrc/plan.hip:

```cpp
#include <cstdint>
#include <cstring>
#include <memory>
#include <vector>

#include "common.cuh"

namespace {

const char* const kSig[DA_FN_COUNT] = {
    nullptr,
     "G",
     "GG",
     "A",
     "ppippppiiiifip",
     "pppiiiif",
     "ppppppiiiiiiif",
     "piiiiinIQfppii",
     "ppiill",
     "ppplifi",
     "ppppili",
     "pppppiflii",
     "ppplpppiflii",
     "pppppiflii",
     "pppppppiflii",
     "p",
     "pppilffi",
     "ppil",
     "ppfili",
     "pppii",
     "ppiiiiiiii",
     "ppiiiiiiii",
     "ppiill",
     "ppllii",
     "ppllii" "i",
     "ppliii",
     "ppiilii",
     "ppiiliiffi",
     "ppppiiifffi",
     "pppppiiiiiiii",
     "ppppiiiiiiiff",
     "ppppiiiiii",
};

struct Op {
  int fn;
  unsigned long long a[DA_PLAN_MAX_ARGS];
};

}

struct da_plan {
  std::vector<Op> ops;
  std::vector<std::unique_ptr<da_gemm_params>> gemm;
  std::vector<std::unique_ptr<da_attention_params>> attn;
  std::vector<std::unique_ptr<std::vector<int>>> ints;
  std::vector<std::unique_ptr<std::vector<const void*>>> ptrs;
};

namespace {

inline float as_float(unsigned long long v) {
  uint32_t u = (uint32_t)v;
  float f;
  std::memcpy(&f, &u, 4);
  return f;
}

template <class F>
void for_each_device_pointer(da_plan* plan, F&& f) {
  for (Op& op : plan->ops) {
    const char* sig = kSig[op.fn];
    for (int i = 0; sig[i]; ++i)
      if (sig[i] == 'p') {
        void* p = (void*)(uintptr_t)op.a[i];
        f(p);
        op.a[i] = (unsigned long long)(uintptr_t)p;
      }
  }
  auto cv = [&](const void*& p) { void* q = const_cast<void*>(p); f(q); p = q; };
  auto cf = [&](const float*& p) { void* q = (void*)p; f(q); p = (const float*)q; };
  for (auto& g : plan->gemm) {
    cv(g->A), cv(g->A2), cv(g->W), f(g->C), cv(g->bias), cv(g->rowvec), cv(g->residual), cv(g->bias_rows), cv(g->gate);
    f(g->workspace), f(g->sync_flags);
    { void* q = g->stats_out; f(q); g->stats_out = (float*)q; }
    cf(g->ln_stats), cf(g->ln_s), cf(g->ln_c), cv(g->prefetch), f(g->vt), cv(g->xa_k), cv(g->xa_vt);
  }
  for (auto& t : plan->attn) cv(t->q), cv(t->k), cv(t->vt), f(t->out), cv(t->bias), f(t->split_ws);
  for (auto& v : plan->ptrs)
    for (const void*& p : *v) cv(p);
}

int run_op(const Op& op, void* s) {
  const unsigned long long* a = op.a;
#define P(i) ((void*)(uintptr_t)a[i])
#define CF(i) ((const float*)(uintptr_t)a[i])
#define CI(i) ((const int*)(uintptr_t)a[i])
#define I(i) ((int)(long long)a[i])
#define LL(i) ((long long)a[i])
#define F(i) (as_float(a[i]))
  switch (op.fn) {
    case DA_FN_GEMM: return da_gemm_bf16((const da_gemm_params*)P(0), s);
    case DA_FN_GEMM_PAIR: return da_gemm_pair_bf16((const da_gemm_params*)P(0), (const da_gemm_params*)P(1), s);
    case DA_FN_ATTENTION: return da_attention_bf16((const da_attention_params*)P(0), s);
    case DA_FN_GROUPNORM_NHWC:
      return da_groupnorm_nhwc_bf16(P(0), P(1), I(2), P(3), P(4), P(5), P(6), I(7), I(8), I(9), I(10), F(11), I(12), P(13), s);
    case DA_FN_RMSNORM: return da_rmsnorm_bf16(P(0), P(1), P(2), I(3), I(4), I(5), I(6), F(7), s);
    case DA_FN_LAYERNORM:
      return da_layernorm_bf16(P(0), P(1), P(2), P(3), P(4), P(5), I(6), I(7), I(8), I(9), I(10), I(11), I(12), F(13), s);
    case DA_FN_RMSNORM_ROPE:
      return da_rmsnorm_rope_bf16(P(0), I(1), I(2), I(3), I(4), I(5), I(6), CI(7), (const void* const*)P(8), F(9), CF(10), CF(11),
                                  I(12), I(13), s);
    case DA_FN_SOFTMAX_ROWS: return da_softmax_rows_f32_bf16(P(0), P(1), I(2), I(3), LL(4), LL(5), s);
    case DA_FN_RMSNORM_CHANNELS: return da_rmsnorm_channels_bf16(P(0), P(1), P(2), LL(3), I(4), F(5), I(6), s);
    case DA_FN_EULER_SCALE_MODEL_INPUT: return da_euler_scale_model_input(P(0), P(1), CF(2), CI(3), I(4), LL(5), I(6), s);
    case DA_FN_EULER_STEP: return da_euler_step(P(0), P(1), P(2), CF(3), CI(4), I(5), F(6), LL(7), I(8), I(9), s);
    case DA_FN_X0_LINEAR_STEP:
      return da_x0_linear_step(P(0), P(1), P(2), LL(3), P(4), CF(5), CI(6), I(7), F(8), LL(9), I(10), I(11), s);
    case DA_FN_FLOWMATCH_STEP: return da_flowmatch_step(P(0), P(1), P(2), CF(3), CI(4), I(5), F(6), LL(7), I(8), I(9), s);
    case DA_FN_UNIPC_FLOW_STEP:
      return da_unipc_flow_step(P(0), P(1), P(2), P(3), P(4), CF(5), CI(6), I(7), F(8), LL(9), I(10), I(11), s);
    case DA_FN_ADVANCE_STEP: return da_advance_step((int*)P(0), s);
    case DA_FN_CFG_RESCALE: return da_cfg_rescale(P(0), P(1), (float*)P(2), I(3), LL(4), F(5), F(6), I(7), s);
    case DA_FN_CAST_F32_BF16: return da_cast_f32_bf16(CF(0), P(1), I(2), LL(3), s);
    case DA_FN_MUL_SCALAR: return da_mul_scalar(P(0), P(1), F(2), I(3), LL(4), I(5), s);
    case DA_FN_BCAST_ADD_F32: return da_bcast_add_f32(CF(0), P(1), (float*)P(2), I(3), I(4), s);
    case DA_FN_PATCHIFY3D: return da_patchify3d_bf16(P(0), P(1), I(2), I(3), I(4), I(5), I(6), I(7), I(8), I(9), s);
    case DA_FN_UNPATCHIFY3D: return da_unpatchify3d_bf16(P(0), P(1), I(2), I(3), I(4), I(5), I(6), I(7), I(8), I(9), s);
    case DA_FN_TRANSPOSE: return da_transpose_bf16(P(0), P(1), I(2), I(3), LL(4), LL(5), s);
    case DA_FN_NHWC_TAKE_NCHW: return da_nhwc_take_nchw_bf16(P(0), P(1), LL(2), LL(3), I(4), I(5), s);
    case DA_FN_NHWC_TAKE_POSTPROCESS: return da_nhwc_take_postprocess(P(0), P(1), LL(2), LL(3), I(4), I(5), I(6), s);
    case DA_FN_PERMUTE_0213: return da_permute_0213_bf16(P(0), P(1), LL(2), I(3), I(4), I(5), s);
    case DA_FN_IMAGE_POSTPROCESS: return da_image_postprocess(P(0), P(1), I(2), I(3), LL(4), I(5), I(6), s);
    case DA_FN_FRAMES_TO_NCTHW:
      return da_frames_to_ncthw_bf16(P(0), P(1), I(2), I(3), LL(4), I(5), I(6), F(7), F(8), I(9), s);
    case DA_FN_TIMESTEP_EMBEDDING:
      return da_timestep_embedding(CF(0), CF(1), CI(2), P(3), I(4), I(5), I(6), F(7), F(8), F(9), I(10), s);
    case DA_FN_LINEAR_SMALL_M:
      return da_linear_small_m_bf16(P(0), P(1), P(2), P(3), P(4), I(5), I(6), I(7), I(8), I(9), I(10), I(11), I(12), s);
    case DA_FN_CONV_THIN_IN:
      return da_conv_thin_in_bf16(P(0), P(1), P(2), P(3), I(4), I(5), I(6), I(7), I(8), I(9), I(10), F(11), F(12), s);
    case DA_FN_CONV_THIN_OUT: return da_conv_thin_out_bf16(P(0), P(1), P(2), P(3), I(4), I(5), I(6), I(7), I(8), I(9), s);
  }
#undef P
#undef CF
#undef CI
#undef I
#undef LL
#undef F
  return DA_ERR_INVALID;
}

}

extern "C" int da_plan_arg_count(int fn) {
  if (fn <= 0 || fn >= DA_FN_COUNT) return -1;
  return (int)std::strlen(kSig[fn]);
}

extern "C" const char* da_plan_arg_kinds(int fn) { return (fn <= 0 || fn >= DA_FN_COUNT) ? nullptr : kSig[fn]; }

extern "C" int da_plan_create(const da_plan_op* ops, int n_ops, da_plan** out) {
  if (!out) return DA_ERR_INVALID;
  *out = nullptr;
  if (n_ops < 0 || (n_ops > 0 && !ops)) return DA_ERR_INVALID;
  std::unique_ptr<da_plan> plan(new da_plan);
  plan->ops.reserve(n_ops);
  for (int o = 0; o < n_ops; ++o) {
    const da_plan_op& src = ops[o];
    if (src.fn <= 0 || src.fn >= DA_FN_COUNT) return DA_ERR_INVALID;
    const char* sig = kSig[src.fn];
    Op op;
    op.fn = src.fn;
    std::memset(op.a, 0, sizeof(op.a));
    int parts = 0;
    for (int i = 0; sig[i]; ++i) {
      const unsigned long long v = src.arg[i];
      switch (sig[i]) {
        case 'G': {
          if (!v) return DA_ERR_INVALID;
          plan->gemm.emplace_back(new da_gemm_params(*(const da_gemm_params*)(uintptr_t)v));
          op.a[i] = (unsigned long long)(uintptr_t)plan->gemm.back().get();
          break;
        }
        case 'A': {
          if (!v) return DA_ERR_INVALID;
          plan->attn.emplace_back(new da_attention_params(*(const da_attention_params*)(uintptr_t)v));
          op.a[i] = (unsigned long long)(uintptr_t)plan->attn.back().get();
          break;
        }
        case 'n':
          parts = (int)(long long)v;
          if (parts < 0 || parts > 64) return DA_ERR_INVALID;
          op.a[i] = v;
          break;
        case 'I': {
          if (!v && parts) return DA_ERR_INVALID;
          const int* h = (const int*)(uintptr_t)v;
          plan->ints.emplace_back(new std::vector<int>(h, h + parts));
          op.a[i] = (unsigned long long)(uintptr_t)plan->ints.back()->data();
          break;
        }
        case 'Q': {
          if (!v && parts) return DA_ERR_INVALID;
          const void* const* h = (const void* const*)(uintptr_t)v;
          plan->ptrs.emplace_back(new std::vector<const void*>(h, h + parts));
          op.a[i] = (unsigned long long)(uintptr_t)plan->ptrs.back()->data();
          break;
        }
        default: op.a[i] = v;
      }
    }
    plan->ops.push_back(op);
  }
  *out = plan.release();
  return DA_OK;
}

extern "C" int da_plan_op_count(const da_plan* plan) { return plan ? (int)plan->ops.size() : -1; }

extern "C" int da_plan_launch(const da_plan* plan, void* stream, int* failed_op) {
  if (failed_op) *failed_op = -1;
  if (!plan) return DA_ERR_INVALID;
  const int n = (int)plan->ops.size();
  for (int o = 0; o < n; ++o) {
// ... 32 lines not shown
```

diffusers_amd/layers.py:

```python
from __future__ import annotations

import os
from typing import Dict, Optional

import torch

from . import _lib as L
from . import ops

bf16 = torch.bfloat16


class Weights:

    def __init__(self, state_dict: Dict[str, torch.Tensor], device):
        self.sd = state_dict
        self.device = torch.device(device)
        self.used = set()

    def has(self, name: str) -> bool:
        return name in self.sd

    def get(self, name: str) -> torch.Tensor:
        if name not in self.sd:
            raise KeyError(f"missing weight '{name}' in state_dict")
        self.used.add(name)
        return self.sd[name].detach().to(device=self.device, dtype=bf16).contiguous()

    def get_f32(self, name: str) -> torch.Tensor:
        if name not in self.sd:
            raise KeyError(f"missing weight '{name}' in state_dict")
        self.used.add(name)
        return self.sd[name].detach().to(device=self.device, dtype=torch.float32).contiguous()

    def opt(self, name: str) -> Optional[torch.Tensor]:
        return self.get(name) if name in self.sd else None

    def unused(self):
        return sorted(set(self.sd.keys()) - self.used)


class Linear:

    def __init__(self, w: Weights, prefix: str):
        self.weight = w.get(prefix + ".weight")
        self.bias = w.opt(prefix + ".bias")

    def __call__(self, x, **kw):
        return ops.linear(x, self.weight, self.bias, **kw)

    @property
    def in_features(self) -> int:
        return self.weight.shape[1]

    @property
    def out_features(self) -> int:
        return self.weight.shape[0]


class Conv3x3:

    def __init__(self, w: Weights, prefix: str):
        self.weight = ops.pack_conv_weight(w.get(prefix + ".weight"))
        self.bias = w.opt(prefix + ".bias")
        self.ksize = 3

    def __call__(self, x, **kw):
        return ops.conv2d_nhwc(x, self.weight, self.bias, ksize=3, **kw)


class Conv1x1:

    def __init__(self, w: Weights, prefix: str):
        wt = w.get(prefix + ".weight")
        self.weight = wt.reshape(wt.shape[0], -1).contiguous()
        self.bias = w.opt(prefix + ".bias")

    def __call__(self, x, x2=None, **kw):
        if x2 is None:
            B, H, W_, C = x.shape
            y = ops.linear(x.view(B * H * W_, C), self.weight, self.bias, **kw)
            return y.view(B, H, W_, -1)
        return ops.conv2d_nhwc(x, self.weight, self.bias, ksize=1, x2=x2, **kw)


class GroupNorm:
    def __init__(self, w: Weights, prefix: str, groups: int, eps: float):
        self.weight = w.get(prefix + ".weight")
        self.bias = w.get(prefix + ".bias")
        self.groups, self.eps = groups, eps

    def __call__(self, x, silu=False, x2=None):
        return ops.group_norm_nhwc(x, self.weight, self.bias, self.groups, self.eps, silu=silu, x2=x2)


class LayerNorm:
    def __init__(self, w: Weights, prefix: str, eps: float = 1e-5, affine: bool = True):
        self.weight = w.get(prefix + ".weight") if affine else None
        self.bias = w.get(prefix + ".bias") if affine else None
        self.eps = eps

    def __call__(self, x, **kw):
        return ops.layer_norm(x, self.weight, self.bias, self.eps, **kw)


class ResnetBlock2D:

    def __init__(self, w: Weights, prefix: str, groups: int, eps: float, output_scale_factor: float = 1.0):
        self.norm1 = GroupNorm(w, prefix + ".norm1", groups, eps)
        self.conv1 = Conv3x3(w, prefix + ".conv1")
        self.has_temb = w.has(prefix + ".time_emb_proj.weight")
        if self.has_temb:
            self.time_emb_proj = Linear(w, prefix + ".time_emb_proj")
        self.norm2 = GroupNorm(w, prefix + ".norm2", groups, eps)
        self.conv2 = Conv3x3(w, prefix + ".conv2")
        self.shortcut = Conv1x1(w, prefix + ".conv_shortcut") if w.has(prefix + ".conv_shortcut.weight") else None
        self.out_scale = 1.0 / output_scale_factor

    def __call__(self, x, temb=None, skip=None):
        h = self.norm1(x, silu=True, x2=skip)
        tvec = None
        if self.has_temb and temb is not None:
            if isinstance(temb, ProjectedTemb):
                tvec = temb.all[:, self.temb_off:self.temb_off + self.temb_c]
            elif self.time_emb_proj is None:
                raise ValueError("ResnetBlock2D: this block's time_emb_proj lives in the model's TimeProjections; pass its output")
            else:
                tvec = ops.linear_small_m(temb, self.time_emb_proj.weight, self.time_emb_proj.bias, act_in=L.ACT_SILU)
        h = self.conv1(h, rowvec=tvec)
        h = self.norm2(h, silu=True)
        if self.shortcut is not None:
            res = self.shortcut(x, x2=skip)
        else:
            if skip is not None:
                raise ValueError("ResnetBlock2D: concat input requires a conv_shortcut")
            res = x
        return self.conv2(h, residual=res, out_scale=self.out_scale)


class ProjectedTemb:

    def __init__(self, t: torch.Tensor):
        self.all = t


class TimeProjections:

    def __init__(self, resnets):
        rs = [r for r in resnets if r.has_temb]
        self.weight = self.bias = None
        if not rs or os.environ.get("DIFFUSERS_AMD_TEMB_STACK", "1") == "0":
            return
        biased = [r.time_emb_proj.bias is not None for r in rs]
        if any(biased) and not all(biased):
            return
        self.weight = torch.cat([r.time_emb_proj.weight for r in rs], dim=0).contiguous()
        self.bias = torch.cat([r.time_emb_proj.bias for r in rs], dim=0).contiguous() if all(biased) else None
        off = 0
        for r in rs:
            r.temb_off, r.temb_c = off, r.time_emb_proj.weight.shape[0]
            off += r.temb_c
            r.time_emb_proj = None

    def __call__(self, temb: torch.Tensor):
        if self.weight is None:
            return temb
        return ProjectedTemb(ops.linear_small_m(temb, self.weight, self.bias, act_in=L.ACT_SILU))


class Downsample2D:

    def __init__(self, w: Weights, prefix: str, padding: int = 1):
        if padding not in (0, 1):
            raise ValueError("Downsample2D: padding must be 0 or 1")
        self.conv = Conv3x3(w, prefix + ".conv")
        self.padding = padding

    def __call__(self, x):
        if self.padding == 1:
            return self.conv(x, stride=2)
        return self.conv(x, stride=2, pad=0, pad_after=1)


class Upsample2D:

    def __init__(self, w: Weights, prefix: str):
        self.conv = Conv3x3(w, prefix + ".conv")

    def __call__(self, x):
        return self.conv(x, up=True)


class CrossKV:

    __slots__ = ("k", "vt", "skv", "skv_alloc", "batch", "bias", "buf")

    def __init__(self, k, vt, skv, skv_alloc, batch, bias=None, buf=None):
        self.k, self.vt, self.skv, self.skv_alloc, self.batch = k, vt, skv, skv_alloc, batch
        self.buf = buf
        self.bias = bias


KERNEL_HEAD_DIMS = (64, 96, 128, 160)


def kernel_head_dim(d: int) -> int:
    for k in KERNEL_HEAD_DIMS:
        if d <= k:
            return k
    raise ValueError(f"attention head_dim {d} exceeds the largest flash-kernel head size {KERNEL_HEAD_DIMS[-1]}")


def pad_head_rows(w: torch.Tensor, heads: int, d: int, dp: int) -> torch.Tensor:
    if d == dp:
        return w
    out = torch.zeros((heads, dp) + tuple(w.shape[1:]), device=w.device, dtype=w.dtype)
    out[:, :d] = w.view((heads, d) + tuple(w.shape[1:]))
    return out.view((heads * dp,) + tuple(w.shape[1:])).contiguous()


def pad_head_cols(w: torch.Tensor, heads: int, d: int, dp: int) -> torch.Tensor:
    if d == dp:
        return w
    out = torch.zeros((w.shape[0], heads, dp), device=w.device, dtype=w.dtype)
    out[:, :, :d] = w.view(w.shape[0], heads, d)
    return out.view(w.shape[0], heads * dp).contiguous()


class Attention:

    def __init__(self, w: Weights, prefix: str, heads: int, cross: bool):
        self.heads = heads
        self.cross = cross
        wq = w.get(prefix + ".to_q.weight")
        wk = w.get(prefix + ".to_k.weight")
        wv = w.get(prefix + ".to_v.weight")
        inner = wq.shape[0]
        self.head_dim = inner // heads
        self.kdim = kernel_head_dim(self.head_dim)
        self.inner = heads * self.kdim
        d, dp = self.head_dim, self.kdim
        wq, wk, wv = (pad_head_rows(t, heads, d, dp) for t in (wq, wk, wv))
        if cross:
            self.wq, self.wk, self.wv = wq, wk, wv
        else:
            self.wqk = torch.cat([wq, wk], dim=0).contiguous()
            self.wv = wv
            self.wqkv_ln = self.fold1 = None
        self.to_out = Linear(w, prefix + ".to_out.0")
        self.to_out.weight = pad_head_cols(self.to_out.weight, heads, d, dp)
        self.scale = self.head_dim ** -0.5

    def precompute_kv(self, ehs_pad: torch.Tensor, batch: int, skv: int, skv_alloc: int, bias=None) -> CrossKV:
        if bias is not None and self.kdim != 64:
            raise ValueError(f"encoder_attention_mask: the masked attention kernel exists for head sizes <= 64 "
                             f"(this layer: {self.head_dim})")
        rows, inner = ehs_pad.shape[0], self.wk.shape[0]
        buf = torch.empty(2 * rows * inner, device=ehs_pad.device, dtype=ehs_pad.dtype)
        k = ops.linear(ehs_pad, self.wk, out=buf[: rows * inner].view(rows, inner))
        vt = ops.linear(self.wv, ehs_pad, out=buf[rows * inner:].view(inner, rows))
        return CrossKV(k, vt, skv, skv_alloc, batch, bias, buf)

    def fold_norm(self, norm: "LayerNorm") -> None:
        self.wq_ln, self.fold = ops.fold_layernorm(self.wq, norm.weight, norm.bias, norm.eps)

    def fold_norm1(self, norm: "LayerNorm") -> None:
        if (2 * self.inner) % 80 != 0:
            return
        wqkv = torch.cat([self.wqk, self.wv], dim=0).contiguous()
        self.wqkv_ln, self.fold1 = ops.fold_layernorm(wqkv, norm.weight, norm.bias, norm.eps)

    def __call__(self, x, batch: int, seq: int, residual, kv: Optional[CrossKV] = None, stats=None, stats_out=None):
        Hh, D = self.heads, self.kdim
# ... 32 lines not shown
            wl, fold = ops.fold_layernorm(w1, norm.weight, norm.bias, norm.eps)
            wl, _ = ops.pack_geglu(wl, None)
            n = w1.shape[0] // 2
            idx = torch.arange(n, device=w1.device).view(n // 32, 32)
            order = torch.cat([idx, idx + n], dim=1).reshape(-1)
            self.w1_ln = wl
            self.fold = ops.LNFold(fold.s.index_select(0, order).contiguous(), fold.c.index_select(0, order).contiguous(),
                                   fold.eps)

    def folds_here(self, rows: int) -> bool:
        if self.w1_ln is None:
            return False
        return int(ops.LN_FOLD) == 1 or ops.geglu_fold_on_k3(rows, self.w1_ln.shape[0], self.w1_ln.shape[1])

    def __call__(self, x, residual, stats=None, stats_out=None):
        if stats is not None:
            h = ops.linear(x, self.w1_ln, self.b1, act=L.ACT_GEGLU, ln=(stats, self.fold))
        else:
            h = ops.linear(x, self.w1, self.b1, act=L.ACT_GEGLU)
        return self.out(h, residual=residual, stats_out=stats_out)


class BasicTransformerBlock:

    def __init__(self, w: Weights, prefix: str, heads: int):
        self.norm1 = LayerNorm(w, prefix + ".norm1")
        self.attn1 = Attention(w, prefix + ".attn1", heads, cross=False)
        self.norm2 = LayerNorm(w, prefix + ".norm2")
        self.attn2 = Attention(w, prefix + ".attn2", heads, cross=True)
        self.norm3 = LayerNorm(w, prefix + ".norm3")
        self.folded = int(ops.LN_FOLD)
        self.ff = FeedForwardGEGLU(w, prefix + ".ff", norm=self.norm3 if self.folded in (1, 3) else None)
        if self.folded:
            self.attn2.fold_norm(self.norm2)
            self.attn1.fold_norm1(self.norm1)
        self.folds_norm1 = bool(self.folded) and self.attn1.wqkv_ln is not None

    def __call__(self, x, batch, seq, kv: CrossKV, stats_in=None, stats_out=None):
        mode = int(ops.LN_FOLD)
        if mode and (not self.folded or (mode in (1, 3) and self.folded not in (1, 3))):
            raise RuntimeError("ops.LN_FOLD was switched on after this model was loaded: the folded weights are built at "
                               "load_state_dict() time (set DIFFUSERS_AMD_LN_FOLD / ops.LN_FOLD before loading)")
        if not mode:
            x = self.attn1(self.norm1(x), batch, seq, residual=x)
            x = self.attn2(self.norm2(x), batch, seq, residual=x, kv=kv)
            return self.ff(self.norm3(x), residual=x)
        use1 = stats_in is not None and self.folds_norm1
        if mode == 2:
            st1 = ops.RowStats(x.shape[0], x.device)
            if use1:
                x = self.attn1(x, batch, seq, residual=x, stats=stats_in, stats_out=st1)
            else:
                x = self.attn1(self.norm1(x), batch, seq, residual=x, stats_out=st1)
            x = self.attn2(x, batch, seq, residual=x, kv=kv, stats=st1)
            return self.ff(self.norm3(x), residual=x, stats_out=stats_out)
        fold3 = self.ff.folds_here(x.shape[0])
        st1 = ops.RowStats(x.shape[0], x.device)
        st2 = ops.RowStats(x.shape[0], x.device) if fold3 else None
        if use1:
            x = self.attn1(x, batch, seq, residual=x, stats=stats_in, stats_out=st1)
        else:
            x = self.attn1(self.norm1(x), batch, seq, residual=x, stats_out=st1)
        x = self.attn2(x, batch, seq, residual=x, kv=kv, stats=st1, stats_out=st2)
        if fold3:
            return self.ff(x, residual=x, stats=st2, stats_out=stats_out)
        return self.ff(self.norm3(x), residual=x, stats_out=stats_out)


class Transformer2DModel:

    def __init__(self, w: Weights, prefix: str, heads: int, layers: int, groups: int):
        self.norm = GroupNorm(w, prefix + ".norm", groups, 1e-6)
        pw = w.get(prefix + ".proj_in.weight")
        self.proj_in_w = pw.reshape(pw.shape[0], -1).contiguous()
        self.proj_in_b = w.opt(prefix + ".proj_in.bias")
        self.blocks = [BasicTransformerBlock(w, f"{prefix}.transformer_blocks.{i}", heads) for i in range(layers)]
        pw = w.get(prefix + ".proj_out.weight")
        self.proj_out_w = pw.reshape(pw.shape[0], -1).contiguous()
        self.proj_out_b = w.opt(prefix + ".proj_out.bias")

    def precompute_kv(self, ehs_pad, batch, skv, skv_alloc, bias=None):
        return [blk.attn2.precompute_kv(ehs_pad, batch, skv, skv_alloc, bias) for blk in self.blocks]

    def __call__(self, x, kvs):
        B, H, W_, C = x.shape
        res = x.view(B * H * W_, C)
        h = self.norm(x).view(B * H * W_, C)
        chain = bool(ops.LN_FOLD) and ops.LN_FOLD_NORM1 and all(b.folds_norm1 for b in self.blocks)
        st = ops.RowStats(h.shape[0], h.device) if chain else None
        h = ops.linear(h, self.proj_in_w, self.proj_in_b, stats_out=st)
        for i, (blk, kv) in enumerate(zip(self.blocks, kvs)):
            nxt = ops.RowStats(h.shape[0], h.device) if chain and i + 1 < len(self.blocks) else None
            h = blk(h, B, H * W_, kv, stats_in=st, stats_out=nxt)
            st = nxt
        h = ops.linear(h, self.proj_out_w, self.proj_out_b, residual=res)
        return h.view(B, H, W_, C)


class TimestepEmbedding:

    def __init__(self, w: Weights, prefix: str):
        self.l1 = Linear(w, prefix + ".linear_1")
        self.l2 = Linear(w, prefix + ".linear_2")

    def __call__(self, x, residual=None):
        h = ops.linear_small_m(x, self.l1.weight, self.l1.bias, act_out=L.ACT_SILU)
        return ops.linear_small_m(h, self.l2.weight, self.l2.bias, residual=residual)

    @property
    def linear_1(self) -> Linear:
        return self.l1

    @property
    def linear_2(self) -> Linear:
        return self.l2


def encoder_mask_bias(mask: torch.Tensor, batch: int, skv: int) -> torch.Tensor:
    if mask.dim() == 2:
        bias = (1 - mask.to(bf16)) * -10000.0
    elif mask.dim() == 3 and mask.shape[1] == 1:
        bias = mask[:, 0].to(bf16)
    else:
        raise ValueError("encoder_attention_mask must be [batch][key_tokens] or a [batch][1][key_tokens] bias")
    if bias.shape[0] != batch or bias.shape[1] != skv:
        raise ValueError(f"encoder_attention_mask shape {tuple(mask.shape)} does not match ({batch}, {skv}) text tokens")
    out = torch.zeros((batch, 1, 1, (skv + 63) // 64 * 64), device=mask.device, dtype=bf16)
    out[:, 0, 0, :skv] = bias
    return out


def pad_encoder_states(ehs: torch.Tensor):
    B, S, C = ehs.shape
    s_alloc = ((S + 15) // 16) * 16
    if s_alloc == S:
        return ehs.reshape(B * S, C).contiguous(), S, s_alloc
    pad = torch.zeros((B, s_alloc, C), device=ehs.device, dtype=ehs.dtype)
    pad[:, :S].copy_(ehs)
    return pad.view(B * s_alloc, C), S, s_alloc
```

diffusers_amd/ops.py:

```python
from __future__ import annotations

import ctypes as C
import os
import threading
import weakref
from typing import Optional

import torch

from . import _lib as L
from . import tuning

bf16 = torch.bfloat16

DEFAULT_STAGING = L.STAGE_LDS_DIRECT
DEFAULT_TILE = L.TILE_AUTO
TUNING = True

PREFETCH = os.environ.get("DIFFUSERS_AMD_PREFETCH", "1") != "0"
_prefetch_tls = threading.local()


class WeightPrefetch:
    def __init__(self, models=(), owner=None, slots=()):
        self._models = tuple(m for m in models if m is not None)
        self._owner = weakref.ref(owner) if owner is not None else None
        self._slots = tuple(slots)
        self.ptrs = set()
        self.seq = []
        self.mode = None
        self.idx = 0
        self.ok = True
        self.applied = 0

    @property
    def models(self):
        owner = self._owner() if self._owner is not None else None
        found = tuple(m for m in (getattr(owner, n, None) for n in self._slots) if m is not None) if owner is not None else ()
        return self._models + found

    def refresh(self):
        from .packed_cache import packed_tensors
        self.ptrs = {t.data_ptr() for m in self.models for t in packed_tensors(m).values() if t.is_cuda}


class weight_prefetch:

    def __init__(self, pf: Optional[WeightPrefetch], mode: str):
        self.pf, self.mode = pf, mode

    def __enter__(self):
        self.prev = getattr(_prefetch_tls, "pf", None)
        if self.pf is not None and PREFETCH:
            pf = self.pf
            pf.mode, pf.idx, pf.applied = self.mode, 0, 0
            pf.ok = True
            if self.mode == "record":
                pf.seq = []
                pf.refresh()
            _prefetch_tls.pf = pf
        return self.pf

    def __exit__(self, *exc):
        pf = self.pf
        if pf is not None and PREFETCH and getattr(_prefetch_tls, "pf", None) is pf and pf.mode == "apply" and pf.idx != len(pf.seq):
            pf.ok = False
        _prefetch_tls.pf = self.prev
        return False


def _nbytes16(t: torch.Tensor) -> int:
    return (t.numel() * t.element_size()) & ~15


PREFETCH_CAP_BYTES = int(float(os.environ.get("DIFFUSERS_AMD_PREFETCH_CAP_MB", "0")) * (1 << 20)) & ~1023


def _prefetch_hook(p: "L.GemmParams", x: torch.Tensor, w: torch.Tensor) -> None:
    pf = getattr(_prefetch_tls, "pf", None)
    if pf is None:
        return
    mine = (w.data_ptr(), _nbytes16(w)) if w.data_ptr() in pf.ptrs else (x.data_ptr(), _nbytes16(x)) if x.data_ptr() in pf.ptrs else None
    if pf.mode == "record":
        pf.seq.append(mine)
        return
    i = pf.idx
    pf.idx += 1
    if not pf.ok or i >= len(pf.seq) or pf.seq[i] != mine:
        if pf.ok and os.environ.get("DIFFUSERS_AMD_PREFETCH_DEBUG"):
            print(f"[prefetch] launch {i}: operands {tuple(x.shape)} / {tuple(w.shape)} are not the recorded step's", flush=True)
        pf.ok = False
        return
    nxt = pf.seq[(i + 1) % len(pf.seq)]
    if nxt is not None:
        p.prefetch, p.prefetch_bytes = nxt[0], (min(nxt[1], PREFETCH_CAP_BYTES) if PREFETCH_CAP_BYTES else nxt[1])
        pf.applied += 1


SPLITK_WS_BYTES = 64 << 20
_splitk_ws = {}


def splitk_workspace(device: torch.device, stream: int):
    key = (device.index if device.index is not None else torch.cuda.current_device(), stream)
    ent = _splitk_ws.get(key)
    if ent is None:
        ent = (torch.empty(SPLITK_WS_BYTES, dtype=torch.uint8, device=device),
               torch.zeros(L.SPLITK_FLAGS, dtype=torch.int32, device=device))
        _splitk_ws[key] = ent
    return ent


ATTN_SPLIT = os.environ.get("DIFFUSERS_AMD_ATTN_SPLIT", "1") == "1"
ATTN_SPLIT_WS_BYTES = 128 << 20
_attn_split_ws = {}


def attn_split_workspace(device: torch.device, stream: int) -> torch.Tensor:
    key = (device.index if device.index is not None else torch.cuda.current_device(), stream)
    ws = _attn_split_ws.get(key)
    if ws is None:
        ws = torch.empty(ATTN_SPLIT_WS_BYTES, dtype=torch.uint8, device=device)
        ws[:L.ATTN_SPLIT_COUNTER_BYTES].zero_()
        _attn_split_ws[key] = ws
    return ws


def splitk_error(device=None) -> bool:
    return any(bool(f[L.SPLITK_ERR_SLOT].item()) for (d, _), (_, f) in _splitk_ws.items()
               if device is None or d == torch.device(device).index)


LN_FOLD = int(os.environ.get("DIFFUSERS_AMD_LN_FOLD", "3"))
LN_FOLD_NORM1 = os.environ.get("DIFFUSERS_AMD_LN_FOLD_NORM1", "1") == "1"
LN_FOLD_K2 = os.environ.get("DIFFUSERS_AMD_LN_FOLD_K2", "1") == "1"
LN_FOLD_K3 = os.environ.get("DIFFUSERS_AMD_LN_FOLD_K3", "1") == "1"
STATS_MAX_PARTS = 64
STATS_MAX_CONSUMED = 24


class RowStats:

    __slots__ = ("buf", "parts")

    def __init__(self, rows: int, device):
        self.buf = torch.empty((rows, STATS_MAX_PARTS, 2), device=device, dtype=torch.float32)
        self.parts = 0


def geglu_fold_on_k3(rows: int, n_packed: int, k: int) -> bool:
    if not (LN_FOLD_K3 and TUNING) or rows % 256 or n_packed % 320:
        return False
    ent = tuning.table().get(f"lin:M{tuning._m_key(int(rows))}:N{int(n_packed)}:K{int(k)}:a{L.ACT_GEGLU}:f0:r0")
    return ent is not None and ent[0] == L.TILE_K3_256x320


class LNFold:

    def __init__(self, s, c, eps):
        self.s, self.c, self.eps = s, c, eps


def fold_layernorm(w: torch.Tensor, gamma: Optional[torch.Tensor], beta: Optional[torch.Tensor], eps: float):
    wf = w.float()
    wp = (wf * gamma.float()[None, :]).to(bf16) if gamma is not None else w
    s = wp.float().sum(dim=1).contiguous()
    c = (wf @ beta.float()).contiguous() if beta is not None else torch.zeros_like(s)
    return wp.contiguous(), LNFold(s, c, float(eps))


def _select_variant(p: "L.GemmParams", tile: Optional[int], staging: Optional[int], stream: int,
                    inplace: bool = False, split_k: Optional[int] = None, device=None) -> None:
    p.split_k = 1
    auto = (TUNING and tile is None and staging is None and split_k is None and DEFAULT_TILE == L.TILE_AUTO
            and DEFAULT_STAGING == L.STAGE_LDS_DIRECT)
    ent = tuning.table().get(tuning.key_of(p)) if auto else None
    want_ws = device is not None and ((auto and (tuning.SPLIT_K or (ent is not None and ent[3] > 1))) or (split_k or 1) > 1)
    if want_ws and not inplace:
        ws, flags = splitk_workspace(device, stream)
        p.workspace, p.sync_flags, p.workspace_bytes = ws.data_ptr(), flags.data_ptr(), ws.numel()
    p._auto = auto
    if auto:
        p.tile, p.staging, sk = tuning.lookup(p, stream, inplace=inplace)
        p.split_k = sk if p.workspace else 1
    else:
        p.tile = DEFAULT_TILE if tile is None else tile
        p.staging = DEFAULT_STAGING if staging is None else staging
        p.split_k = split_k or 1


def _stream() -> int:
    return torch.cuda.current_stream().cuda_stream


DA_ERR_UNSUPPORTED = 3


def _launch_gemm(p: "L.GemmParams", st: int, what: str) -> None:
    rc = L.load().da_gemm_bf16(C.byref(p), st)
    if rc == DA_ERR_UNSUPPORTED and getattr(p, "_auto", False) and p.tile != L.TILE_AUTO:
        p.tile, p.staging, p.split_k = L.TILE_AUTO, L.STAGE_LDS_DIRECT, 1
        rc = L.load().da_gemm_bf16(C.byref(p), st)
    L.check(rc, what)


def _ptr(t: Optional[torch.Tensor]) -> Optional[int]:
    return None if t is None else t.data_ptr()


def _req(t: torch.Tensor, name: str, dtype=bf16) -> None:
    if not t.is_cuda:
        raise RuntimeError(f"{name}: diffusers_amd ops need a HIP device tensor (got {t.device}); there is no CPU path")
    if dtype is not None and t.dtype != dtype:
        raise TypeError(f"{name}: expected {dtype}, got {t.dtype}")


def require_hip(t: torch.Tensor, name: str, dtypes=(bf16,)) -> None:
    if t.dtype not in dtypes or not t.is_cuda:
        kinds = " / ".join(str(d).replace("torch.", "").replace("bfloat16", "bf16").replace("float32", "fp32") for d in dtypes)
        raise ValueError(f"{name} must be a {kinds} HIP tensor (there is no CPU / fp32 fallback)")


def _rows2d(t: torch.Tensor, name: str) -> int:
    if t.dim() != 2 or t.stride(1) != 1:
        raise ValueError(f"{name}: expected a 2-D tensor with contiguous last dim, got shape {tuple(t.shape)} "
                         f"strides {t.stride()}")
    return t.stride(0) if t.shape[0] > 1 else max(t.stride(0), t.shape[1])


QKV_CANDIDATES = ((L.TILE_K2_128x80, L.STAGE_PINGPONG), (L.TILE_K2_128x80, L.STAGE_PINGPONG3), (L.TILE_K2_128x160, L.STAGE_PINGPONG),
                  (L.TILE_K2_128x160, L.STAGE_LDS_DIRECT), (L.TILE_K1_128x256, L.STAGE_LDS_DIRECT), (L.TILE_K1_128x256, L.STAGE_LDS_DIRECT3),
                  (L.TILE_K1_256x128, L.STAGE_LDS_DIRECT), (L.TILE_K1_256x128, L.STAGE_LDS_DIRECT3))
QKV_RETUNE = os.environ.get("DIFFUSERS_AMD_QKV_RETUNE", "0") == "1"
_qkv_retuned = set()
QKV_TILE_COLS = {L.TILE_K2_128x80: 80, L.TILE_K2_128x160: 160, L.TILE_K1_128x256: 256, L.TILE_K1_256x128: 128}


def qkv_variant(p: "L.GemmParams", stream: int):
    key = "qkv:" + tuning.key_of(p)
    ent = tuning.table().get(key) if TUNING else None
    if ent is not None and not (QKV_RETUNE and key not in _qkv_retuned):
        return ent[0], ent[1]
    _qkv_retuned.add(key)
    field = QKV_CANDIDATES if tuning.FAMILY == "all" else tuple(c for c in QKV_CANDIDATES if c[0] < L.TILE_K1_128x320)
    ok = [(t, s) for t, s in field if p.vt_col0 % QKV_TILE_COLS[t] == 0]
    if not ok:
        raise ValueError(f"linear(vt_out=): column origin {p.vt_col0} is not a multiple of a tile width {sorted(set(QKV_TILE_COLS.values()))}")
    if not (TUNING and tuning.LIVE) or torch.cuda.is_current_stream_capturing():
        return ok[0]
    lib, best = L.load(), None
    for t, s in ok:
        p.tile, p.staging, p.split_k = t, s, 1
        if lib.da_gemm_bf16(C.byref(p), stream) != 0:
            continue
        e0, e1 = torch.cuda.Event(enable_timing=True), torch.cuda.Event(enable_timing=True)
        e0.record()
        for _ in range(3):
            lib.da_gemm_bf16(C.byref(p), stream)
        e1.record()
        e1.synchronize()
        us = e0.elapsed_time(e1) * 1e3 / 3
        if best is None or us < best[2]:
            best = (t, s, us)
    if best is None:
        raise RuntimeError("linear(vt_out=): no kernel variant accepted this problem")
    tuning.table()[key] = (best[0], best[1], best[2], 1)
    tuning.mark_dirty()
    return best[0], best[1]


XATTN = os.environ.get("DIFFUSERS_AMD_XATTN", "0") == "1"
KV_PREFETCH = os.environ.get("DIFFUSERS_AMD_KV_PREFETCH", "0") == "1"
XATTN_MAX_KEYS = 80
XATTN_STAGING = L.STAGE_PINGPONG if os.environ.get("DIFFUSERS_AMD_XATTN_STAGE", "pp") == "pp" else L.STAGE_LDS_DIRECT
XATTN_MIN_TILES = int(os.environ.get("DIFFUSERS_AMD_XATTN_MIN_TILES", "0"))


def xattn_eligible(M: int, N: int, seq: int, head_dim: int, skv_alloc: int) -> bool:
    return head_dim == 64 and N % 128 == 0 and seq > 0 and seq % 128 == 0 and M % seq == 0 and M > 8 and \
        0 < skv_alloc <= XATTN_MAX_KEYS and skv_alloc % 8 == 0


def linear_qkv(x: torch.Tensor, wqkv: torch.Tensor, col0: int, bias: Optional[torch.Tensor] = None, ln: Optional[tuple] = None):
    M = x.shape[0]
    vt = torch.empty((wqkv.shape[0] - col0, M), device=x.device, dtype=bf16)
    qk = linear(x, wqkv, bias, ln=ln, vt_out=(vt, col0))
    return qk, vt


def linear(x: torch.Tensor, w: torch.Tensor, bias: Optional[torch.Tensor] = None, *, act: int = L.ACT_NONE,
           residual: Optional[torch.Tensor] = None, rowvec: Optional[torch.Tensor] = None, rows_per_batch: int = 0,
           alpha: float = 1.0, out_scale: float = 1.0, out: Optional[torch.Tensor] = None, out_f32: bool = False,
           bias_rows: Optional[torch.Tensor] = None, gate: Optional[torch.Tensor] = None,
           tile: Optional[int] = None, staging: Optional[int] = None, split_k: Optional[int] = None,
           stats_out: Optional[RowStats] = None, ln: Optional[tuple] = None, k_valid: int = 0,
           prefetch: Optional[torch.Tensor] = None, vt_out: Optional[tuple] = None,
           xattn: Optional[dict] = None) -> torch.Tensor:
    p, st = _linear_params(x, w, bias, act=act, residual=residual, rowvec=rowvec, rows_per_batch=rows_per_batch,
                           alpha=alpha, out_scale=out_scale, out=out, out_f32=out_f32, bias_rows=bias_rows, gate=gate,
                           tile=tile, staging=staging, split_k=split_k, stats_out=stats_out, ln=ln, k_valid=k_valid,
                           prefetch=prefetch, vt_out=vt_out, xattn=xattn)
    if p is None:
        return st
    _launch_gemm(p, st, "da_gemm_bf16(linear)")
    return p._out


def linear_pair(a: dict, b: dict):
    if a["x"].shape[0] <= 8 or b["x"].shape[0] <= 8:
        return linear(**a), linear(**b)
    pa, st = _linear_params(**a)
    pb, _ = _linear_params(**b)
    if pa is None or pb is None:
        raise ValueError("linear_pair: both problems must take the MFMA GEMM path (M > 8)")
    lib = L.load()
    pair = tuning.lookup_pair(pa, pb, st) if TUNING else None
    if pair is not None:
        sep = (tuning.table().get(tuning.key_of(pa)), tuning.table().get(tuning.key_of(pb)))
        if all(sep) and pair[2] >= sep[0][2] + sep[1][2]:
            pair = None
    if pair is None:
        _launch_gemm(pa, st, "da_gemm_bf16(linear)")
        _launch_gemm(pb, st, "da_gemm_bf16(linear)")
    else:
        pa.tile, pa.staging, pa.split_k, pb.split_k = pair[0], pair[1], 1, 1
        L.check(lib.da_gemm_pair_bf16(C.byref(pa), C.byref(pb), st), "da_gemm_pair_bf16")
    return pa._out, pb._out


def _linear_params(x: torch.Tensor, w: torch.Tensor, bias: Optional[torch.Tensor] = None, *, act: int = L.ACT_NONE,
                   residual: Optional[torch.Tensor] = None, rowvec: Optional[torch.Tensor] = None,
                   rows_per_batch: int = 0, alpha: float = 1.0, out_scale: float = 1.0,
                   out: Optional[torch.Tensor] = None, out_f32: bool = False, bias_rows: Optional[torch.Tensor] = None,
                   gate: Optional[torch.Tensor] = None, tile: Optional[int] = None, staging: Optional[int] = None,
                   split_k: Optional[int] = None, stats_out: Optional[RowStats] = None, ln: Optional[tuple] = None,
                   k_valid: int = 0, prefetch: Optional[torch.Tensor] = None, vt_out: Optional[tuple] = None,
                   xattn: Optional[dict] = None):
    _req(x, "x"), _req(w, "w")
    M, K = x.shape
    N, Kw = w.shape
    if K != Kw:
        raise ValueError(f"linear: K mismatch {K} vs {Kw}")
    n_out = N // 2 if act in (L.ACT_GEGLU, L.ACT_GEGLU_TANH) else N
    if vt_out is not None:
        vt_t, vt_col0 = vt_out
        _req(vt_t, "vt_out")
        if vt_t.dim() != 2 or vt_t.stride(1) != 1 or vt_t.shape[0] != N - vt_col0 or vt_t.shape[1] < M or not 0 < vt_col0 < N:
            raise ValueError("linear(vt_out=): expected (bf16 [N - col0][>= M], col0)")
        if M <= 8 or act != L.ACT_NONE or residual is not None or gate is not None or rowvec is not None or stats_out is not None:
            raise ValueError("linear(vt_out=): plain / LayerNorm-folded projections of more than 8 rows only")
        n_out = vt_col0
    if M <= 8 and act in (L.ACT_NONE, L.ACT_SILU, L.ACT_GELU_TANH) and rowvec is None and not out_f32 \
            and alpha == 1.0 and out_scale == 1.0 and bias_rows is None and gate is None and stats_out is None and ln is None:
        return None, linear_small_m(x, w, bias, act_out=act, residual=residual, out=out)
    if out is None:
        out = torch.empty((M, n_out), device=x.device, dtype=torch.float32 if out_f32 else bf16)
    p = L.GemmParams()
    p.A, p.A2, p.W, p.C = x.data_ptr(), None, w.data_ptr(), out.data_ptr()
    p.bias, p.rowvec, p.residual = _ptr(bias), _ptr(rowvec), _ptr(residual)
    p.M, p.N, p.K = M, N, K
    p.lda, p.ldw, p.ldc = _rows2d(x, "x"), _rows2d(w, "w"), _rows2d(out, "out")
    p.ldr = _rows2d(residual, "residual") if residual is not None else 0
    p.ld_rowvec = _rows2d(rowvec, "rowvec") if rowvec is not None else 0
    p.bias_rows, p.gate = _ptr(bias_rows), _ptr(gate)
    p.ld_gate = _rows2d(gate, "gate") if gate is not None else 0
    _prefetch_hook(p, x, w)
    if prefetch is not None:
        p.prefetch, p.prefetch_bytes = prefetch.data_ptr(), (prefetch.numel() * prefetch.element_size()) & ~15
    if gate is not None:
        if gate.dtype not in (bf16, torch.float32):
            raise TypeError("linear: gate must be bf16 (Flux rounding) or float32 (Wan rounding)")
        p.gate_f32 = int(gate.dtype == torch.float32)
    inplace = residual is not None and out.data_ptr() == residual.data_ptr()
    if inplace and p.ldr != p.ldc:
        raise ValueError("linear: an aliased residual must have the output's row stride")
    p.rows_per_batch = rows_per_batch
    p.alpha, p.out_scale, p.act, p.out_f32, p.conv = alpha, out_scale, act, int(out_f32), 0
    if not 0 <= k_valid <= K:
        raise ValueError(f"linear: k_valid {k_valid} outside [0, K = {K}]")
    p.k_valid = 0 if k_valid == K else k_valid
    st = _stream()
    if ln is not None:
        rs, fold = ln
        if rs.parts <= 0 or rs.buf.shape[0] != M or fold.s.numel() != N or fold.c.numel() != N:
            raise ValueError("linear(ln=): statistics / fold vectors do not match this problem (was the producer run?)")
        p.ln_stats, p.ln_stats_ld, p.ln_parts = rs.buf.data_ptr(), rs.buf.shape[1] * 2, rs.parts
        p.ln_s, p.ln_c, p.ln_eps = fold.s.data_ptr(), fold.c.data_ptr(), fold.eps
    if vt_out is not None:
        p.vt, p.vt_col0, p.ld_vt = vt_out[0].data_ptr(), int(vt_out[1]), vt_out[0].stride(0)
    if xattn is not None:
        xk, xvt = xattn["k"], xattn["vt"]
        _req(xk, "xattn k"), _req(xvt, "xattn vt")
        if not xattn_eligible(M, N, xattn["seq"], 64, xattn["skv_alloc"]) or xk.shape[1] != N or xvt.shape[0] != N:
            raise ValueError("linear(xattn=): heads of 64 channels in pairs (N % 128 == 0), row tiles of 128 inside one batch, "
                             f"<= {XATTN_MAX_KEYS} text tokens")
        if act != L.ACT_NONE or residual is not None or gate is not None or rowvec is not None or stats_out is not None \
                or vt_out is not None or out_f32 or out_scale != 1.0 or bias_rows is not None or M <= 8:
            raise ValueError("linear(xattn=): nothing but bias / the LayerNorm fold combines with the attention epilogue")
        p.xa_k, p.xa_vt = xk.data_ptr(), xvt.data_ptr()
        p.xa_skv, p.xa_skv_alloc, p.xa_k_ld, p.xa_vt_ld = int(xattn["skv"]), int(xattn["skv_alloc"]), _rows2d(xk, "xattn k"), _rows2d(xvt, "xattn vt")
        p.xa_scale = float(xattn["scale"])
        p.rows_per_batch = int(xattn["seq"])
        p._keep_xa = (xk, xvt)
        if tile is None:
            tile, staging, split_k = L.TILE_K2_128x128, XATTN_STAGING, 1
    tile_given = tile is not None
    if vt_out is not None and tile is None:
        tile, staging = qkv_variant(p, st)
        split_k = 1
    if (stats_out is not None or ln is not None) and tile is None:
        geglu_ = act in (L.ACT_GEGLU, L.ACT_GEGLU_TANH)
        ent = tuning.table().get(tuning.key_of(p)) if TUNING else None
        k3_geglu = (geglu_ and LN_FOLD_K3 and ent is not None and ent[0] == L.TILE_K3_256x320 and ln is not None and stats_out is None
                    and M % 256 == 0 and N % 320 == 0)
        if geglu_ and not k3_geglu and ent is not None and ent[0] in (L.TILE_K1_256x256, L.TILE_K1_128x256, L.TILE_K1_256x128,
                                                                      L.TILE_K1_256x320, L.TILE_K3_256x256, L.TILE_K3_256x320):
            ent = (L.TILE_K1_128x320, L.STAGE_LDS_DIRECT) + tuple(ent[2:])
        k2_ok = (ent is not None and ent[0] in ((L.TILE_K1_128x320, L.TILE_K3_256x320) if geglu_ else (L.TILE_K2_128x80, L.TILE_K2_128x160))
                 and not out_f32 and p.ldc % 8 == 0 and out.data_ptr() % 16 == 0 and N % 16 == 0 and gate is None
                 and (residual is None or (p.ldr % 8 == 0 and residual.data_ptr() % 16 == 0))
                 and not (ent[0] == L.TILE_K2_128x160 and ent[1] in (L.STAGE_LDS_DIRECT3, L.STAGE_PINGPONG3))
                 and not (geglu_ and ent[1] != L.STAGE_LDS_DIRECT))
        if k2_ok and LN_FOLD_K2:
            tile, staging, split_k = ent[0], ent[1], 1
        else:
            tile, staging, split_k = ((L.TILE_128x128, L.STAGE_LDS_DIRECT) if geglu_ else (L.TILE_128x64, L.STAGE_LDS_DIRECT3)) + (1,)
    _select_variant(p, tile, staging, st, inplace=inplace, split_k=split_k, device=x.device)
    if stats_out is not None:
        if act in (L.ACT_GEGLU, L.ACT_GEGLU_TANH) or out_f32 or stats_out.buf.shape[0] != M:
            raise ValueError("linear(stats_out=): bf16 non-GEGLU outputs only, one statistics row per output row")
        p.stats_out, p.stats_ld = stats_out.buf.data_ptr(), stats_out.buf.shape[1] * 2
        stats_out.parts = int(L.load().da_gemm_stats_parts(C.byref(p)))
        if stats_out.parts > STATS_MAX_CONSUMED and not tile_given:
            p.tile, p.staging, p.split_k = (L.TILE_128x128 if N <= 128 * STATS_MAX_CONSUMED else L.TILE_128x256), L.STAGE_LDS_DIRECT, 1
            stats_out.parts = int(L.load().da_gemm_stats_parts(C.byref(p)))
        if not 0 < stats_out.parts <= min(stats_out.buf.shape[1], STATS_MAX_CONSUMED):
            raise ValueError(f"linear(stats_out=): {stats_out.parts} column tiles: the consumer reads at most "
                             f"{STATS_MAX_CONSUMED} partials per row (use a wider tile for this producer)")
    p._out = out
    p._keep = (x, w, bias, residual, rowvec, bias_rows, gate, stats_out, ln, vt_out)
    return p, st


def conv2d_nhwc(x: torch.Tensor, w: torch.Tensor, bias: Optional[torch.Tensor] = None, *, ksize: int = 3,
                x2: Optional[torch.Tensor] = None, stride: int = 1, up: bool = False, pad: Optional[int] = None,
                rowvec: Optional[torch.Tensor] = None, residual: Optional[torch.Tensor] = None,
                out_scale: float = 1.0, act: int = L.ACT_NONE, tile: Optional[int] = None,
                staging: Optional[int] = None, pad_after: int = 0, out: Optional[torch.Tensor] = None,
                split_k: Optional[int] = None, k_valid: int = 0) -> torch.Tensor:
    _req(x, "x"), _req(w, "w")
    if x2 is not None:
        _req(x2, "x2")
    p = _conv_params(x, w, ksize, x2, stride, up, pad, pad_after)
    B, Hout, Wout, Cout = x.shape[0], p.Hout, p.Wout, p.N
    if out is None:
        out = torch.empty((B, Hout, Wout, Cout), device=x.device, dtype=bf16)
    else:
        _req(out, "out")
        if tuple(out.shape) != (B, Hout, Wout, Cout) or not out.is_contiguous():
            raise ValueError("conv2d_nhwc: out must be contiguous [B][Hout][Wout][Cout]")
    inplace = residual is not None and residual.data_ptr() == out.data_ptr()
    p.A, p.A2, p.W, p.C = x.data_ptr(), _ptr(x2), w.data_ptr(), out.data_ptr()
    p.bias, p.rowvec, p.residual = _ptr(bias), _ptr(rowvec), _ptr(residual)
    if residual is not None:
        _req(residual, "residual")
        if tuple(residual.shape) != (B, Hout, Wout, Cout) or not residual.is_contiguous():
            raise ValueError("conv2d_nhwc: residual must be contiguous [B][Hout][Wout][Cout]")
        p.ldr = Cout
    if rowvec is not None:
        _req(rowvec, "rowvec")
        p.ld_rowvec = _rows2d(rowvec, "rowvec")
        p.rows_per_batch = Hout * Wout
    p.alpha, p.out_scale, p.act, p.out_f32 = 1.0, out_scale, act, 0
    C1, C2 = p.C1, p.C2
    if not 0 <= k_valid <= C1 or (k_valid and C2):
        raise ValueError(f"conv2d_nhwc: k_valid {k_valid} outside [0, C1 = {C1}] (or given with a second source)")
    p.k_valid = 0 if k_valid == C1 else k_valid
    _prefetch_hook(p, x, w)
    st = _stream()
    _select_variant(p, tile, staging, st, inplace=inplace, split_k=split_k, device=x.device)
    _launch_gemm(p, st, "da_gemm_bf16(conv)")
    return out


def _conv_params(x: torch.Tensor, w: torch.Tensor, ksize: int, x2: Optional[torch.Tensor], stride: int, up: bool,
                 pad: Optional[int], pad_after: int) -> "L.GemmParams":
    B, H, W_, C1 = x.shape
    C2 = 0
    if x2 is not None:
        if x2.shape[:3] != x.shape[:3]:
            raise ValueError("conv2d_nhwc: x2 spatial shape mismatch")
        C2 = x2.shape[3]
    if not x.is_contiguous() or (x2 is not None and not x2.is_contiguous()):
        raise ValueError("conv2d_nhwc: inputs must be contiguous NHWC")
    Cout, K = w.shape
    if K != ksize * ksize * (C1 + C2):
        raise ValueError(f"conv2d_nhwc: weight K={K} != {ksize}*{ksize}*{C1 + C2}")
    if pad is None:
        pad = (ksize - 1) // 2
    Hv, Wv = (2 * H, 2 * W_) if up else (H, W_)
    Hout = (Hv + 2 * pad + pad_after - ksize) // stride + 1
    Wout = (Wv + 2 * pad + pad_after - ksize) // stride + 1
    p = L.GemmParams()
    p.M, p.N, p.K = B * Hout * Wout, Cout, K
    p.lda, p.ldw, p.ldc = 0, K, Cout
    p.conv = ksize
    p.Hin, p.Win, p.C1, p.C2, p.Hout, p.Wout = H, W_, C1, C2, Hout, Wout
    p.stride, p.up, p.pad = stride, int(up), pad
    return p


def conv_chunk_channels(x: torch.Tensor, w: torch.Tensor, tile: int, *, ksize: int = 3, x2: Optional[torch.Tensor] = None,
                        stride: int = 1, up: bool = False, pad: Optional[int] = None, pad_after: int = 0) -> int:
    p = _conv_params(x, w, ksize, x2, stride, up, pad, pad_after)
    r = int(L.load().da_conv_chunk_channels(C.byref(p), int(tile)))
    if r < 0:
        L.check(-r, f"da_conv_chunk_channels(tile {L.TILE_NAMES[tile] if 0 <= tile < len(L.TILE_NAMES) else tile})")
    return r


def linear_small_m(x: torch.Tensor, w: torch.Tensor, bias: Optional[torch.Tensor] = None, *, act_in: int = L.ACT_NONE,
                   act_out: int = L.ACT_NONE, residual: Optional[torch.Tensor] = None,
                   out: Optional[torch.Tensor] = None) -> torch.Tensor:
    _req(x, "x"), _req(w, "w")
    M, K = x.shape
    N = w.shape[0]
    if w.shape[1] != K or not w.is_contiguous():
        raise ValueError("linear_small_m: weight must be contiguous [N][K]")
    if out is None:
        out = torch.empty((M, N), device=x.device, dtype=bf16)
    L.check(L.load().da_linear_small_m_bf16(
        x.data_ptr(), w.data_ptr(), _ptr(bias), _ptr(residual), out.data_ptr(), M, N, K, _rows2d(x, "x"),
        _rows2d(out, "out"), _rows2d(residual, "residual") if residual is not None else 0, act_in, act_out, _stream()),
        "da_linear_small_m_bf16")
    return out


def pack_geglu(w: torch.Tensor, bias: Optional[torch.Tensor]):
    n2 = w.shape[0]
    n = n2 // 2
    if n % 64:
        raise ValueError("pack_geglu: inner dim must be a multiple of 64")
    idx = torch.arange(n, device=w.device).view(n // 32, 32)
    order = torch.cat([idx, idx + n], dim=1).reshape(-1)
    wp = w.index_select(0, order).contiguous()
    bp = bias.index_select(0, order).contiguous() if bias is not None else None
    return wp, bp


def pack_conv_weight(w: torch.Tensor) -> torch.Tensor:
    co, ci, kh, kw = w.shape
    return w.permute(0, 2, 3, 1).reshape(co, kh * kw * ci).contiguous()


def attention(q: torch.Tensor, k: torch.Tensor, vt: torch.Tensor, *, B: int, H: int, D: int, Sq: int, Skv: int,
              Skv_alloc: int, q_row_stride: int, k_row_stride: int, q_batch_stride: int, k_batch_stride: int,
              vt_ld: int, vt_batch_stride: int, scale: Optional[float] = None,
              out: Optional[torch.Tensor] = None, ring_slots: int = 0, causal: bool = False,
              bias: Optional[torch.Tensor] = None, q_block: int = 0, pv_delay: int = 0, algo: int = 0,
              kv_split: int = 0) -> torch.Tensor:
    _req(q, "q"), _req(k, "k"), _req(vt, "vt")
    if out is None:
        out = torch.empty((B * Sq, H * D), device=q.device, dtype=bf16)
    o_row_stride = _rows2d(out, "out")
    p = L.AttentionParams()
    p.q, p.k, p.vt, p.out = q.data_ptr(), k.data_ptr(), vt.data_ptr(), out.data_ptr()
    p.B, p.H, p.Sq, p.Skv, p.Skv_alloc, p.D = B, H, Sq, Skv, Skv_alloc, D
    p.q_batch_stride, p.k_batch_stride, p.vt_batch_stride = q_batch_stride, k_batch_stride, vt_batch_stride
    p.o_batch_stride = Sq * o_row_stride
    p.q_row_stride, p.k_row_stride, p.vt_ld, p.o_row_stride = q_row_stride, k_row_stride, vt_ld, o_row_stride
    p.scale = (D ** -0.5) if scale is None else scale
    p.ring_slots = ring_slots
    p.q_block = q_block
    p.pv_delay = pv_delay
    p.algo = algo
    p.causal = int(causal)
    p.kv_split = kv_split if ATTN_SPLIT or kv_split > 1 else 1
    if p.kv_split != 1 and bias is None and not causal and D in (64, 128) and Skv >= 256 and B * H * ((Sq + 127) // 128) >= 64:
        ws = attn_split_workspace(q.device, _stream())
        p.split_ws, p.split_ws_bytes = ws.data_ptr(), ws.numel()
    if bias is not None:
        _req(bias, "bias", None)
        if bias.dtype not in (bf16, torch.float32) or bias.dim() != 4 or bias.stride(3) != 1 or \
                (bias.shape[2] != 1 and bias.shape[2] < Sq):
            raise ValueError("attention: bias must be a bf16 / fp32 [B|1][H|1][Sq|1][>= ceil64(Skv)] tensor, last dim contiguous")
        if bias.shape[0] not in (1, B) or bias.shape[1] not in (1, H):
            raise ValueError("attention: bias batch / head dims must be 1 or match")
        p.bias, p.bias_f32 = bias.data_ptr(), int(bias.dtype == torch.float32)
        p.bias_batch_stride = bias.stride(0) if bias.shape[0] > 1 else 0
        p.bias_head_stride = bias.stride(1) if bias.shape[1] > 1 else 0
        p.bias_row_stride = bias.stride(2) if bias.shape[2] > 1 else 0
    L.check(L.load().da_attention_bf16(C.byref(p), _stream()), "da_attention_bf16")
    return out


def softmax_rows(scores: torch.Tensor, out: Optional[torch.Tensor] = None) -> torch.Tensor:
    _req(scores, "scores", torch.float32)
    M, N = scores.shape
    if out is None:
        out = torch.empty((M, N), device=scores.device, dtype=bf16)
    else:
        _req(out, "out")
        if out.shape[0] != M or out.shape[1] < N:
            raise ValueError("softmax_rows: out must be [M][>= N]")
    L.check(L.load().da_softmax_rows_f32_bf16(scores.data_ptr(), out.data_ptr(), M, N, _rows2d(scores, "scores"),
                                              _rows2d(out, "out"), _stream()), "da_softmax_rows_f32_bf16")
    return out


_gn_ws = {}
GN_MULTI = os.environ.get("DIFFUSERS_AMD_GN_MULTI", "0") == "1"
_gn_sync = {}


def gn_sync_workspace(device: torch.device, stream: int) -> torch.Tensor:
    key = (device.index if device.index is not None else torch.cuda.current_device(), stream)
    ws = _gn_sync.get(key)
    if ws is None:
        ws = torch.zeros(int(L.load().da_groupnorm_sync_bytes()), dtype=torch.uint8, device=device)
        _gn_sync[key] = ws
    return ws


def gn_sync_error(device=None) -> bool:
    off = 4096 * 4
    return any(bool(w[off:off + 4].view(torch.int32).item()) for (d, _), w in _gn_sync.items()
               if device is None or d == torch.device(device).index)


def group_norm_nhwc(x: torch.Tensor, gamma: torch.Tensor, beta: torch.Tensor, groups: int, eps: float,
                    silu: bool = False, x2: Optional[torch.Tensor] = None) -> torch.Tensor:
    _req(x, "x"), _req(gamma, "gamma"), _req(beta, "beta")
    if not x.is_contiguous() or (x2 is not None and not x2.is_contiguous()):
        raise ValueError("group_norm_nhwc: contiguous channels-last input required")
    B = x.shape[0]
    C1 = x.shape[-1]
    Ctot = C1 + (x2.shape[-1] if x2 is not None else 0)
    HW = x.numel() // (B * C1)
    lib = L.load()
    nbytes = lib.da_groupnorm_workspace_bytes(B, HW, Ctot, groups)
    ws = torch.empty((max(nbytes, 4) // 4,), device=x.device, dtype=torch.float32)
    y = torch.empty(tuple(x.shape[:-1]) + (Ctot,), device=x.device, dtype=bf16)
    sync = gn_sync_workspace(x.device, _stream()).data_ptr() if GN_MULTI and B * HW * Ctot >= (1 << 20) else None
    L.check(lib.da_groupnorm_nhwc_bf16(x.data_ptr(), _ptr(x2), C1, gamma.data_ptr(), beta.data_ptr(), y.data_ptr(),
                                       ws.data_ptr(), B, HW, Ctot, groups, eps, L.ACT_SILU if silu else L.ACT_NONE,
                                       sync, _stream()), "da_groupnorm_nhwc_bf16")
    return y


def rms_norm(x: torch.Tensor, gamma: torch.Tensor, eps: float) -> torch.Tensor:
    _req(x, "x"), _req(gamma, "gamma")
    M, Cc = x.shape
    y = torch.empty((M, Cc), device=x.device, dtype=bf16)
    L.check(L.load().da_rmsnorm_bf16(x.data_ptr(), gamma.data_ptr(), y.data_ptr(), M, Cc, _rows2d(x, "x"), Cc, eps, _stream()),
            "da_rmsnorm_bf16")
    return y


def rmsnorm_channels(x: torch.Tensor, gamma: torch.Tensor, *, real_channels: int, silu: bool = False) -> torch.Tensor:
    _req(x, "x"), _req(gamma, "gamma")
    Cc = x.shape[-1]
    if not x.is_contiguous() or gamma.numel() != Cc:
        raise ValueError("rmsnorm_channels: contiguous channels-last input and a [C] gamma required")
    y = torch.empty_like(x)
    L.check(L.load().da_rmsnorm_channels_bf16(x.data_ptr(), gamma.data_ptr(), y.data_ptr(), x.numel() // Cc, Cc,
                                              float(real_channels) ** 0.5, L.ACT_SILU if silu else L.ACT_NONE,
                                              _stream()), "da_rmsnorm_channels_bf16")
    return y


def layer_norm(x: torch.Tensor, gamma: Optional[torch.Tensor], beta: Optional[torch.Tensor], eps: float, *,
               mod_scale: Optional[torch.Tensor] = None, mod_shift: Optional[torch.Tensor] = None,
               rows_per_batch: int = 0) -> torch.Tensor:
    _req(x, "x")
    M, Cc = x.shape
    y = torch.empty((M, Cc), device=x.device, dtype=bf16)
    mod_ld = _rows2d(mod_scale, "mod_scale") if mod_scale is not None else 0
    mod_f32 = 0
    if mod_scale is not None:
        if mod_scale.dtype != mod_shift.dtype or mod_scale.dtype not in (bf16, torch.float32):
            raise TypeError("layer_norm: mod_scale / mod_shift must both be bf16 or both float32")
        mod_f32 = int(mod_scale.dtype == torch.float32)
    L.check(L.load().da_layernorm_bf16(x.data_ptr(), _ptr(gamma), _ptr(beta), y.data_ptr(), _ptr(mod_scale),
                                       _ptr(mod_shift), mod_ld, mod_f32, rows_per_batch, M, Cc, _rows2d(x, "x"), Cc,
                                       eps, _stream()), "da_layernorm_bf16")
    return y


def rmsnorm_rope_(x: torch.Tensor, *, heads: int, head_dim: int, col_offsets, weights=None, eps: float = 1e-6,
                  cos: Optional[torch.Tensor] = None, sin: Optional[torch.Tensor] = None, rope_row0: int = 0,
                  rows_per_batch: int = 0, norm: str = "per_head") -> torch.Tensor:
    _req(x, "x")
    rows = x.shape[0]
    ld = _rows2d(x, "x")
    parts = len(col_offsets)
    offs = (C.c_int * parts)(*[int(o) for o in col_offsets])
    wptr = None
    if weights is not None:
        for w_ in weights:
            if w_ is not None:
                _req(w_, "weight")
        wptr = (C.c_void_p * parts)(*[(w_.data_ptr() if w_ is not None else None) for w_ in weights])
    if cos is not None:
        _req(cos, "cos", torch.float32), _req(sin, "sin", torch.float32)
        if cos.shape[-1] != head_dim or not cos.is_contiguous() or not sin.is_contiguous():
            raise ValueError("rmsnorm_rope_: cos / sin must be contiguous [rows][head_dim] fp32")
    mode = {"none": 0, "per_head": 1, "across_heads": 2}[norm]
    L.check(L.load().da_rmsnorm_rope_bf16(x.data_ptr(), ld, rows, rows_per_batch or rows, heads, head_dim, parts, offs,
                                          wptr, eps, _ptr(cos), _ptr(sin), rope_row0, mode, _stream()),
            "da_rmsnorm_rope_bf16")
    return x


def _dt(t: torch.Tensor) -> int:
    if t.dtype == bf16:
        return L.DTYPE_BF16
    if t.dtype == torch.float32:
        return L.DTYPE_F32
    raise TypeError(f"sampler kernels support bf16 / fp32 latents, got {t.dtype}")


def _check_sampler(what: str, x: torch.Tensor, model_out: torch.Tensor, out: Optional[torch.Tensor], cfg: bool,
# ... 390 lines not shown
```

diffusers_amd/unet_2d_condition.py:

```python
from __future__ import annotations

from dataclasses import dataclass
from typing import Any, Dict, List, Optional

import torch

from . import ops
from .config_utils import check_to
from .loading import PretrainedMixin
from .layers import (Downsample2D, GroupNorm, ResnetBlock2D, TimeProjections, TimestepEmbedding, Transformer2DModel,
                     Upsample2D, Weights, encoder_mask_bias, pad_encoder_states)

bf16 = torch.bfloat16


@dataclass
class UNet2DConditionOutput:
    sample: torch.Tensor


class FrozenConfig(dict):
    def __getattr__(self, k):
        try:
            return self[k]
# ... 181 lines not shown
            return cond
        self._cond_cache = (key, cond, (encoder_hidden_states, added.get("text_embeds"), added.get("time_ids"),
                                        encoder_attention_mask))
        return cond

    @staticmethod
    def _nhwc(r: torch.Tensor, like: torch.Tensor) -> torch.Tensor:
        ops.require_hip(r, "additional residual", (bf16, torch.float16, torch.float32))
        if r.dim() != 4 or tuple(r.shape) != (like.shape[0], like.shape[3], like.shape[1], like.shape[2]):
            raise ValueError(f"additional residual of shape {tuple(r.shape)} does not match the activation "
                             f"{(like.shape[0], like.shape[3], like.shape[1], like.shape[2])} (NCHW)")
        return r.to(bf16).permute(0, 2, 3, 1).contiguous()

    def _text_time_embedding(self, added_cond_kwargs, B):
        if added_cond_kwargs is None or "text_embeds" not in added_cond_kwargs:
            raise ValueError(f"{self.__class__} has the config param `addition_embed_type` set to 'text_time' which "
                             "requires the keyword argument `text_embeds` to be passed in `added_cond_kwargs`")
        if "time_ids" not in added_cond_kwargs:
            raise ValueError(f"{self.__class__} has the config param `addition_embed_type` set to 'text_time' which "
                             "requires the keyword argument `time_ids` to be passed in `added_cond_kwargs`")
        text_embeds = added_cond_kwargs["text_embeds"].to(device=self.device, dtype=bf16).contiguous()
        time_ids = added_cond_kwargs["time_ids"].to(device=self.device, dtype=torch.float32).contiguous()
        c = self.config
        n_ids = time_ids.shape[1]
        te = ops.timestep_embedding(time_ids.reshape(-1), c.addition_time_embed_dim, batch=B * n_ids,
                                    flip_sin_to_cos=c.flip_sin_to_cos, shift=float(c.freq_shift))
        te = te.view(B, n_ids * c.addition_time_embed_dim)
        add = torch.cat([text_embeds, te], dim=-1).contiguous()
        return self.add_embedding(add)

    def __call__(self, *a, **k):
        return self.forward(*a, **k)

    def forward(self, sample: torch.Tensor, timestep, encoder_hidden_states: torch.Tensor, class_labels=None,
                timestep_cond=None, attention_mask=None, cross_attention_kwargs=None, added_cond_kwargs=None,
                down_block_additional_residuals=None, mid_block_additional_residual=None,
                down_intrablock_additional_residuals=None, encoder_attention_mask=None, return_dict: bool = True,
                conditioning: Optional[Dict[str, Any]] = None, sampler_table=None, step_idx=None):
        if not self._built:
            raise RuntimeError("UNet2DConditionModel: call load_state_dict() first")
        for name, v in (("class_labels", class_labels), ("timestep_cond", timestep_cond),
                        ("attention_mask", attention_mask),
                        ("down_intrablock_additional_residuals", down_intrablock_additional_residuals)):
            if v is not None:
                raise ValueError(f"diffusers_amd UNet2DConditionModel.forward: `{name}` is not supported on the HIP path")
        if cross_attention_kwargs:
            extra = {k: v for k, v in cross_attention_kwargs.items() if not (k == "scale" and float(v) == 1.0)}
            if extra:
                raise ValueError(f"diffusers_amd UNet2DConditionModel.forward: cross_attention_kwargs {sorted(extra)} are not "
                                 "supported on the HIP path (LoRA scales: fuse_lora(scale) packs them into the weights)")
        if (down_block_additional_residuals is None) != (mid_block_additional_residual is None):
            raise ValueError("ControlNet residuals: pass both down_block_additional_residuals and "
                             "mid_block_additional_residual (unet_2d_condition.py:1104)")
        ops.require_hip(sample, "sample")
        c = self.config
        B, Cin, H, W_ = sample.shape
        n_up = len(c.block_out_channels) - 1
        if H % (2 ** n_up) or W_ % (2 ** n_up):
            raise ValueError("sample height/width must be divisible by 2**(num_upsamplers)")
        if conditioning is None:
            conditioning = self._cached_conditioning(encoder_hidden_states, added_cond_kwargs, encoder_attention_mask)
        elif encoder_attention_mask is not None:
            raise ValueError("pass encoder_attention_mask to precompute_conditioning() when `conditioning` is given")
        if conditioning["batch"] != B:
            raise ValueError("conditioning batch does not match sample batch")
        kvs = conditioning["kvs"]

        if sampler_table is not None:
            t_emb = ops.timestep_embedding(None, c.block_out_channels[0], batch=B, flip_sin_to_cos=c.flip_sin_to_cos,
                                           shift=float(c.freq_shift), table=sampler_table, step_idx=step_idx)
        else:
            if not torch.is_tensor(timestep):
                timestep = torch.tensor([float(timestep)], dtype=torch.float32)
            t = timestep.to(device=self.device, dtype=torch.float32).reshape(-1)
            if t.numel() == 1:
                t = t.expand(B)
            t_emb = ops.timestep_embedding(t.contiguous(), c.block_out_channels[0], batch=B,
                                           flip_sin_to_cos=c.flip_sin_to_cos, shift=float(c.freq_shift))
        emb = self.time_embedding(t_emb, residual=conditioning["aug_emb"])
        emb = self.time_proj(emb)

        x = ops.conv_thin_in(sample.contiguous(), self.conv_in_w, self.conv_in_b, ksize=3, in_nchw=True)

        ki = 0
        skips = [x]
        for st in self.down:
            for j, rn in enumerate(st["resnets"]):
                x = rn(x, emb)
                if st["attns"]:
                    x = st["attns"][j](x, kvs[ki])
                    ki += 1
                skips.append(x)
            if st["down"] is not None:
                x = st["down"](x)
                skips.append(x)

        if down_block_additional_residuals is not None:
            if len(down_block_additional_residuals) != len(skips):
                raise ValueError(f"down_block_additional_residuals: expected {len(skips)} tensors, got "
                                 f"{len(down_block_additional_residuals)}")
            skips = [s_ + self._nhwc(r, s_) for s_, r in zip(skips, down_block_additional_residuals)]

        x = self.mid["resnets"][0](x, emb)
        x = self.mid["attns"][0](x, kvs[ki])
        ki += 1
        x = self.mid["resnets"][1](x, emb)
        if mid_block_additional_residual is not None:
            x = x + self._nhwc(mid_block_additional_residual, x)

        for st in self.up:
            for j, rn in enumerate(st["resnets"]):
                skip = skips.pop()
                x = rn(x, emb, skip=skip)
                if st["attns"]:
                    x = st["attns"][j](x, kvs[ki])
                    ki += 1
            if st["up"] is not None:
                x = st["up"](x)

        x = self.conv_norm_out(x, silu=True)
        out = ops.conv_thin_out(x, self.conv_out_w, self.conv_out_b)
        if not return_dict:
            return (out,)
        return UNet2DConditionOutput(sample=out)
```

include/diffusers_amd.h:

```cpp
#ifndef DIFFUSERS_AMD_H
#define DIFFUSERS_AMD_H

#include <stddef.h>
#include <stdint.h>

#ifdef __cplusplus
extern "C" {
#endif

#define DA_OK 0
#define DA_ERR_INVALID 1
#define DA_ERR_LAUNCH 2
#define DA_ERR_UNSUPPORTED 3

#define DA_ACT_NONE 0
#define DA_ACT_GEGLU 1
#define DA_ACT_GELU_TANH 2
#define DA_ACT_SILU 3
#define DA_ACT_GELU_ERF 4
#define DA_ACT_QUICK_GELU 5
#define DA_ACT_GEGLU_TANH 6

#define DA_TILE_AUTO 0
#define DA_TILE_128x128 1
#define DA_TILE_64x128 2
#define DA_TILE_128x64 3
#define DA_TILE_64x64 4
#define DA_TILE_256x128 5
#define DA_TILE_128x256 6
#define DA_TILE_256x256 7
#define DA_TILE_128x128_W8 8

#define DA_TILE_K2_128x128 9
#define DA_TILE_K2_128x80 10
#define DA_TILE_K2_128x160 11
#define DA_TILE_K2_80x128 12
#define DA_TILE_K2_128x64 13
#define DA_TILE_K1_128x320 14
#define DA_TILE_K1_256x128 15
#define DA_TILE_K1_128x256 16
#define DA_TILE_K1_256x160 17
#define DA_TILE_K1_256x256 18
#define DA_TILE_K1_256x320 19
#define DA_TILE_K3_256x256 20
#define DA_TILE_K3_256x320 21
#define DA_TILE_COUNT 22
#define DA_TILE_FAMILY_1 (-1)
#define DA_TILE_FAMILY_K2 (-2)

#define DA_STAGE_REGISTER 0
#define DA_STAGE_LDS_DIRECT 1
#define DA_STAGE_LDS_DIRECT3 2
#define DA_STAGE_LDS_DIRECT4 3
#define DA_STAGE_LDS_DIRECT6 4
#define DA_STAGE_LDS_DIRECT8 5
#define DA_STAGE_PINGPONG 6
#define DA_STAGE_PINGPONG3 7

#define DA_ABI_VERSION 6
int da_version(void);
size_t da_sizeof_gemm_params(void);
size_t da_sizeof_attention_params(void);
int da_set_launch_events(void* start_event, void* stop_event);
int da_set_launch_flags(unsigned flags);
int da_mfma_probe(int blocks, int iters, void* sink, double* flop, void* stream);
const char* da_last_error(void);

typedef struct da_gemm_params {
  const void* A;
  const void* A2;
  const void* W;
  void* C;
  const void* bias;
  const void* rowvec;
  const void* residual;
  const void* bias_rows;
  const void* gate;
  int M, N, K;
  int lda, ldw, ldc, ldr, ld_rowvec, ld_gate;
  int rows_per_batch;
  float alpha;
  float out_scale;
  int act;
  int out_f32;
  int conv;
  int Hin, Win, C1, C2, Hout, Wout, stride, up, pad;
  int tile;
  int staging;
  int gate_f32;
  int split_k;
  void* workspace;
  void* sync_flags;
  long long workspace_bytes;
  float* stats_out;
  int stats_ld;
  const float* ln_stats;
  int ln_stats_ld, ln_parts;
  const float* ln_s;
  const float* ln_c;
  float ln_eps;
  int k_valid;
  const void* prefetch;
  long long prefetch_bytes;
  void* vt;
  int vt_col0;
  long long ld_vt;
  const void* xa_k;
  const void* xa_vt;
  int xa_skv, xa_skv_alloc, xa_k_ld;
  long long xa_vt_ld;
  float xa_scale;
} da_gemm_params;

int da_gemm_stats_parts(const da_gemm_params* p);

int da_conv_chunk_channels(const da_gemm_params* p, int tile);

#define DA_LN_MAX_PARTS 64
#define DA_LN_PAIR_LOADS 6
#define DA_SPLITK_FLAGS 4096
#define DA_SPLITK_MAX 24
#define DA_SPLITK_ERR_SLOT (DA_SPLITK_FLAGS - 1)

int da_gemm_bf16(const da_gemm_params* p, void* stream);

int da_gemm_pair_bf16(const da_gemm_params* a, const da_gemm_params* b, void* stream);

int da_gemm_tune(const da_gemm_params* p, const da_gemm_params* pair, void* stream, int iters, void* scratch,
                 size_t scratch_bytes, int* best_tile, int* best_staging, int* best_split, float* best_us);

typedef struct da_attention_params {
  const void* q;
  const void* k;
  const void* vt;
  void* out;
  int B, H, Sq, Skv, Skv_alloc, D;
  long long q_batch_stride, k_batch_stride, vt_batch_stride, o_batch_stride;
  int q_row_stride, k_row_stride, vt_ld, o_row_stride;
  float scale;
  int ring_slots;
  const void* bias;
  long long bias_batch_stride, bias_head_stride;
  int bias_row_stride, bias_f32, causal;
  int q_block;
  int pv_delay;
  int algo;
  void* split_ws;
  long long split_ws_bytes;
  int kv_split;
} da_attention_params;
#define DA_ATTN_SPLIT_COUNTER_BYTES 16384
long long da_attention_split_plan(const da_attention_params* p, int* full_blocks, int* tail_blocks, int* units_per_tail_block);

int da_attention_bf16(const da_attention_params* p, void* stream);

size_t da_groupnorm_workspace_bytes(int B, int HW, int C, int G);
size_t da_groupnorm_sync_bytes(void);
int da_groupnorm_nhwc_bf16(const void* x, const void* x2, int C1, const void* gamma, const void* beta, void* y,
                           void* workspace, int B, int HW, int C, int G, float eps, int act, void* sync, void* stream);
int da_rmsnorm_bf16(const void* x, const void* gamma, void* y, int M, int C, int ldx, int ldy, float eps, void* stream);
int da_layernorm_bf16(const void* x, const void* gamma, const void* beta, void* y, const void* mod_scale,
                      const void* mod_shift, int mod_ld, int mod_f32, int rows_per_batch, int M, int C, int ldx, int ldy,
                      float eps, void* stream);
int da_rmsnorm_rope_bf16(void* x, int ld, int rows, int rows_per_batch, int heads, int D, int parts, const int* col_off,
                         const void* const* weight, float eps, const float* cos, const float* sin, int rope_row0,
                         int do_norm, void* stream);
int da_softmax_rows_f32_bf16(const void* scores, void* probs, int M, int N, long long ld, long long ldo, void* stream);
int da_rmsnorm_channels_bf16(const void* x, const void* gamma, void* y, long long rows, int C, float scale, int act,
                             void* stream);

#define DA_DTYPE_BF16 0
#define DA_DTYPE_F32 1
#define DA_PRED_EPSILON 0
#define DA_PRED_V 1
#define DA_PRED_SAMPLE 2
int da_euler_scale_model_input(const void* x, void* out, const float* table, const int* step_idx, int rep, long long n,
                               int dtype, void* stream);
int da_euler_step(const void* eps, const void* x, void* out, const float* table, const int* step_idx, int cfg,
                  float guidance, long long n, int dtype, int pred_type, void* stream);
int da_x0_linear_step(const void* eps, const void* x, const void* noise, long long noise_step_stride, void* out,
                      const float* table, const int* step_idx, int cfg, float guidance, long long n, int dtype,
                      int pred_type, void* stream);
int da_flowmatch_step(const void* v, const void* x, void* out, const float* table, const int* step_idx, int cfg,
                      float guidance, long long n, int dtype, int x_dtype, void* stream);
int da_unipc_flow_step(const void* v, void* x, void* last, void* m1, void* m2, const float* coef, const int* step_idx,
                       int cfg, float guidance, long long n, int x_dtype, int v_dtype, void* stream);
int da_advance_step(int* step_idx, void* stream);
int da_cfg_rescale(const void* eps, void* out, float* ratio_ws, int B, long long n_per, float guidance, float guidance_rescale,
                   int dtype, void* stream);
int da_cast_f32_bf16(const float* x, void* out, int rep, long long n, void* stream);
int da_mul_scalar(const void* x, void* out, float s, int rep, long long n, int dtype, void* stream);

int da_bcast_add_f32(const float* a, const void* m_bf16, float* out, int B, int n, void* stream);
int da_patchify3d_bf16(const void* x, void* tokens, int B, int C, int F, int H, int W, int pt, int ph, int pw, void* stream);
int da_unpatchify3d_bf16(const void* tokens, void* x, int B, int C, int F, int H, int W, int pt, int ph, int pw,
                         void* stream);
int da_transpose_bf16(const void* in, void* out, int R, int C, long long ldi, long long ldo, void* stream);
int da_nhwc_take_nchw_bf16(const void* in, void* out, long long B, long long HW, int cpad, int cout, void* stream);
int da_nhwc_take_postprocess(const void* in, void* out, long long B, long long HW, int cpad, int cout, int mode, void* stream);
int da_permute_0213_bf16(const void* src, void* dst, long long D0, int D1, int D2, int D3, void* stream);
int da_image_postprocess(const void* img, void* out, int B, int C, long long HW, int in_f32, int mode, void* stream);
int da_frames_to_ncthw_bf16(const void* src, void* dst, int B, int T, long long HW, int Cs, int C, float lo, float hi,
                            int out_f32, void* stream);
int da_timestep_embedding(const float* t, const float* table, const int* step_idx, void* out, int B, int dim,
                          int flip_sin_to_cos, float shift, float scale, float max_period, int out_f32, void* stream);
int da_linear_small_m_bf16(const void* x, const void* W, const void* bias, const void* res, void* out, int M, int N,
                           int K, int ldx, int ldo, int ldr, int act_in, int act_out, void* stream);
int da_conv_thin_in_bf16(const void* x, const void* w, const void* bias, void* y, int B, int H, int W, int Cin, int Cout,
                         int ksize, int in_nchw, float in_div, float in_add, void* stream);
int da_conv_thin_out_bf16(const void* x, const void* w, const void* bias, void* y, int B, int H, int W, int Cin,
                          int Cout, int out_f32, void* stream);

#define DA_IMAGE_F32_NCHW 0
#define DA_IMAGE_F32_NHWC 1
#define DA_IMAGE_U8_NHWC 2
#define DA_POSTERIOR_MOMENTS 0
#define DA_POSTERIOR_MEAN 1
#define DA_POSTERIOR_SAMPLE 2
#define DA_POSTERIOR_NOISE 3
#define DA_LATENTS_SHIFT 1
#define DA_LATENTS_SCALE 2
int da_vae_conv_in_image(const void* x, int src, const void* w, const void* bias, void* y, int B, int H, int W, int Cout,
                         int normalize, void* stream);
int da_vae_posterior_latents(const void* in, long long sB, long long sC, long long sP, const void* wq, const void* bq,
                             const void* eps1, const void* eps2, void* out, int B, long long HW, int L, int mode, int flags,
                             float shift, float scale, float a, float b, void* stream);

#define DA_FN_GEMM 1
#define DA_FN_GEMM_PAIR 2
#define DA_FN_ATTENTION 3
#define DA_FN_GROUPNORM_NHWC 4
#define DA_FN_RMSNORM 5
#define DA_FN_LAYERNORM 6
#define DA_FN_RMSNORM_ROPE 7
#define DA_FN_SOFTMAX_ROWS 8
#define DA_FN_RMSNORM_CHANNELS 9
#define DA_FN_EULER_SCALE_MODEL_INPUT 10
#define DA_FN_EULER_STEP 11
#define DA_FN_X0_LINEAR_STEP 12
#define DA_FN_FLOWMATCH_STEP 13
#define DA_FN_UNIPC_FLOW_STEP 14
#define DA_FN_ADVANCE_STEP 15
#define DA_FN_CFG_RESCALE 16
#define DA_FN_CAST_F32_BF16 17
#define DA_FN_MUL_SCALAR 18
#define DA_FN_BCAST_ADD_F32 19
#define DA_FN_PATCHIFY3D 20
#define DA_FN_UNPATCHIFY3D 21
#define DA_FN_TRANSPOSE 22
#define DA_FN_NHWC_TAKE_NCHW 23
#define DA_FN_NHWC_TAKE_POSTPROCESS 24
#define DA_FN_PERMUTE_0213 25
#define DA_FN_IMAGE_POSTPROCESS 26
#define DA_FN_FRAMES_TO_NCTHW 27
#define DA_FN_TIMESTEP_EMBEDDING 28
#define DA_FN_LINEAR_SMALL_M 29
#define DA_FN_CONV_THIN_IN 30
#define DA_FN_CONV_THIN_OUT 31
#define DA_FN_COUNT 32
#define DA_PLAN_MAX_ARGS 16

typedef struct da_plan_op {
  int fn;
  int reserved;
  unsigned long long arg[DA_PLAN_MAX_ARGS];
} da_plan_op;
typedef struct da_plan da_plan;

int da_plan_create(const da_plan_op* ops, int n_ops, da_plan** out);
int da_plan_launch(const da_plan* plan, void* stream, int* failed_op);
int da_plan_relocate(da_plan* plan, int n_regions, const void* const* old_base, const unsigned long long* bytes,
                     void* const* new_base, int* unmatched);
int da_plan_op_count(const da_plan* plan);
void da_plan_destroy(da_plan* plan);
int da_plan_arg_count(int fn);
const char* da_plan_arg_kinds(int fn);

#ifdef __cplusplus
}
#endif
#endif
```

Baseline: 1.023.

## Fuse GroupNorm statistics into producing GEMM/conv epilogues for SDXL UNet

Adds a GNS variant of the k2/k1 GEMM kernel whose epilogue reduces per-128-row, per-group sum and sum-of-squares of the bf16 output into a parts buffer, for up to two downstream GroupNorm consumers (next norm and the skip-connection's concat norm). A new groupnorm apply entry point then consumes the precomputed parts and skips the separate statistics pass over the activation. The UNet forward is rewired so each resnet, attention, downsample and upsample output feeds stats to the following norm. This adds LDS scratch and an epilogue reduction with extra barriers, and restricts those GEMMs to a few tile shapes.

```diff
diff --git a/diffusers_amd/_lib.py b/diffusers_amd/_lib.py
--- a/diffusers_amd/_lib.py
+++ b/diffusers_amd/_lib.py
@@ -51,6 +51,9 @@
         ("vt", C.c_void_p), ("vt_col0", C.c_int), ("ld_vt", C.c_longlong),
         ("xa_k", C.c_void_p), ("xa_vt", C.c_void_p), ("xa_skv", C.c_int), ("xa_skv_alloc", C.c_int), ("xa_k_ld", C.c_int),
         ("xa_vt_ld", C.c_longlong), ("xa_scale", C.c_float),
+        ("gn_out", C.c_void_p), ("gn_groups", C.c_int), ("gn_cpg", C.c_int), ("gn_coff", C.c_int),
+        ("gn2_out", C.c_void_p), ("gn2_groups", C.c_int), ("gn2_cpg", C.c_int), ("gn2_coff", C.c_int),
+        ("gn_rows", C.c_int),
     ]
 
 
@@ -80,7 +83,7 @@
     "da_mul_scalar", "da_bcast_add_f32", "da_patchify3d_bf16", "da_unpatchify3d_bf16", "da_transpose_bf16",
     "da_nhwc_take_nchw_bf16", "da_nhwc_take_postprocess", "da_permute_0213_bf16", "da_image_postprocess",
     "da_frames_to_ncthw_bf16", "da_timestep_embedding", "da_linear_small_m_bf16", "da_conv_thin_in_bf16",
-    "da_conv_thin_out_bf16"))}
+    "da_conv_thin_out_bf16", "da_groupnorm_parts_nhwc_bf16"))}
 FN_COUNT = len(FN_IDS) + 1
 
 
@@ -108,6 +111,9 @@
     "da_attention_split_plan": (_ll, [C.POINTER(AttentionParams), C.POINTER(C.c_int), C.POINTER(C.c_int), C.POINTER(C.c_int)]),
     "da_groupnorm_workspace_bytes": (C.c_size_t, [_i, _i, _i, _i]),
     "da_groupnorm_sync_bytes": (C.c_size_t, []),
+    "da_groupnorm_two_pass": (_i, [_i, _i, _i, _i, _i, _i]),
+    "da_groupnorm_parts_nhwc_bf16": (_i, [_vp, _vp, _i, _vp, _vp, _vp, _vp, _i, _i, _i, _i, _f, _i, _vp]),
+    "da_gemm_gn_parts_bytes": (C.c_size_t, [_i, _i]),
     "da_groupnorm_nhwc_bf16": (_i, [_vp, _vp, _i, _vp, _vp, _vp, _vp, _i, _i, _i, _i, _f, _i, _vp, _vp]),
     "da_rmsnorm_bf16": (_i, [_vp, _vp, _vp, _i, _i, _i, _i, _f, _vp]),
     "da_layernorm_bf16": (_i, [_vp, _vp, _vp, _vp, _vp, _vp, _i, _i, _i, _i, _i, _i, _i, _f, _vp]),
@@ -153,7 +159,7 @@
 POSTERIOR_MOMENTS, POSTERIOR_MEAN, POSTERIOR_SAMPLE, POSTERIOR_NOISE = 0, 1, 2, 3
 LATENTS_SHIFT, LATENTS_SCALE = 1, 2
 
-ABI_VERSION = 6
+ABI_VERSION = 7
 _lib = None
 _tls = threading.local()
 
diff --git a/diffusers_amd/csrc/gemm.hip b/diffusers_amd/csrc/gemm.hip
--- a/diffusers_amd/csrc/gemm.hip
+++ b/diffusers_amd/csrc/gemm.hip
@@ -74,6 +74,7 @@
   if (p.split_k < 0 || p.split_k > DA_SPLITK_MAX) return DA_ERR_INVALID;
   if (p.split_k > 1 && (p.stats_out || p.ln_stats)) return DA_ERR_UNSUPPORTED;
   if (p.k_valid < 0 || (p.k_valid > 0 && (p.k_valid > (p.conv ? p.C1 : p.K) || (p.conv && p.C2 != 0)))) return DA_ERR_INVALID;
+  if (p.gn2_out && !p.gn_out) return DA_ERR_INVALID;
   if (p.stats_out && (p.conv || p.out_f32 || p.act == DA_ACT_GEGLU || p.act == DA_ACT_GEGLU_TANH || p.stats_ld <= 0 || (p.stats_ld & 1)))
     return DA_ERR_UNSUPPORTED;
   if (p.ln_stats && (p.conv || !p.ln_s || !p.ln_c || p.ln_parts <= 0 || p.ln_parts > 4 * DA_LN_PAIR_LOADS ||
@@ -92,6 +93,7 @@
 
 bool tile_ok(const da_gemm_params& p, int tile) {
   if (tile <= 0 || tile >= kNumTiles) return false;
+  if ((p.gn_out || p.gn2_out) && (!is_k2(tile) || p.split_k > 1)) return false;
   if (is_k3(tile)) {
     if (p.conv || p.split_k > 1 || p.stats_out || (p.ln_stats && tile != DA_TILE_K3_256x320) || p.vt || p.xa_k) return false;
     if (tile == DA_TILE_K3_256x320)
@@ -162,6 +164,11 @@
   if (tile == DA_TILE_AUTO) tile = pick_tile(*pp);
   if (tile <= 0 || tile >= kNumTiles) return 0;
   return stats_parts(*pp, tile);
+}
+
+extern "C" size_t da_gemm_gn_parts_bytes(int M, int G) {
+  if (M <= 0 || G <= 0 || (M % 128)) return 0;
+  return (size_t)(M / 128) * 2 * G * 2 * sizeof(float);
 }
 
 extern "C" int da_conv_chunk_channels(const da_gemm_params* pp, int tile) {
diff --git a/diffusers_amd/csrc/gemm2_kernel.cuh b/diffusers_amd/csrc/gemm2_kernel.cuh
--- a/diffusers_amd/csrc/gemm2_kernel.cuh
+++ b/diffusers_amd/csrc/gemm2_kernel.cuh
@@ -7,6 +7,14 @@
 #include "gemm2_shared.cuh"
 
 namespace da_gemm2 {
+
+struct GnDst {
+  float* out;
+  int groups, cpg, coff;
+};
+__host__ __device__ __forceinline__ GnDst gn_dst(const da_gemm_params& p, int c) {
+  return c ? GnDst{p.gn2_out, p.gn2_groups, p.gn2_cpg, p.gn2_coff} : GnDst{p.gn_out, p.gn_groups, p.gn_cpg, p.gn_coff};
+}
 
 
 #if defined(DA_GEMM2_TRACE)
@@ -19,7 +27,7 @@
 
 
 template <int KG, int WM, int WN, int MT, int NT, int NSLOT, bool CONV, bool PP = false, bool STREAMW = false, bool GIL = false,
-          bool LNF = false, int XA = 0>
+          bool LNF = false, int XA = 0, bool GNS = false>
 __global__ __launch_bounds__(512) void igemm2_bf16_kernel(const da_gemm_params p, const int xcd_gx_chunk) {
 #if defined(__HIP_DEVICE_COMPILE__)
   const int xcd_gx = xcd_gx_chunk & 255;
@@ -31,6 +39,7 @@
   static_assert(!STREAMW || (KG == 1 && NSLOT == 2 && !CONV), "streaming-W loop: one K-group, two-slice ring, nn.Linear");
   static_assert(!GIL || (KG == 1 && !CONV && WN == 2 && (NT % 2) == 0), "GEGLU-interleaved ownership: two wave columns, value / gate tile pairs");
   static_assert(!LNF || (!CONV && !STREAMW), "LayerNorm fold: nn.Linear instantiations of the ring loops");
+  static_assert(!GNS || (!LNF && !STREAMW && !GIL && XA == 0 && (KG == 1 || (MT % 2) == 0)), "GroupNorm statistics: plain ring loops, row-split K-groups");
   static_assert(XA == 0 || (LNF && KG == 2 && WM == 2 && WN == 2 && MT == 4 && NT == 4 && NSLOT == 2 && XA <= 8),
                 "cross-attention epilogue: the 128 x 128 two-K-group tile (a wave finishes 32 rows x one 64-wide head)");
   constexpr int SW = PP ? 4 : 8;
@@ -270,6 +279,9 @@
   static_assert(!STG || (KG == 2 ? 4 * MT * NT * 1024 : 0) + 8 * 16 * ROWB <= NSLOT * PAIR, "output staging does not fit the ring");
   constexpr int STATS_OFF = (KG == 2 ? 4 * MT * NT * 1024 : 0) + 8 * 16 * ROWB;
   static_assert(!(LNF && STG) || STATS_OFF + 8 * TT * 64 * 8 <= NSLOT * PAIR, "statistics scratch does not fit the ring");
+  constexpr int GN_CJ = (8 * NH + 63) / 64, GN_RB = BM / 128, GN_B_OFF = STATS_OFF + 8 * 8 * NH * 16;
+  static_assert(!GNS || (STG && BM % 128 == 0 && GN_B_OFF + GN_RB * (BN / 2) * 16 <= NSLOT * PAIR),
+                "GroupNorm statistics scratch does not fit the ring");
   const bool wide = STG && !GIL && !geglu && !p.out_f32 && !(p.ldc & 7) && !((size_t)p.C & 15) && !(p.N & 7) &&
                     (!p.residual || (!(p.ldr & 7) && !((size_t)p.residual & 15)));
   const int band_col0 = n0 + (wn * NT + (SPLIT_M ? 0 : g * NH)) * 16;
@@ -856,6 +868,72 @@
     }
     return;
   }
+  float4 gacc[GNS ? GN_CJ : 1];
+#pragma unroll
+  for (int j = 0; j < (GNS ? GN_CJ : 1); ++j) gacc[j] = make_float4(0.f, 0.f, 0.f, 0.f);
+  auto gn_epilogue = [&]() {
+    if constexpr (GNS) {
+      float4* ga = (float4*)(smem + STATS_OFF);
+      float4* gb = (float4*)(smem + GN_B_OFF);
+#pragma unroll
+      for (int j = 0; j < GN_CJ; ++j)
+        if (lane + 64 * j < 8 * NH) ga[wave * (8 * NH) + lane + 64 * j] = gacc[j];
+      asm volatile("s_waitcnt lgkmcnt(0)" ::: "memory");
+      __builtin_amdgcn_s_barrier();
+      asm volatile("" ::: "memory");
+      for (int i = t; i < GN_RB * (BN / 2); i += 512) {
+        const int rb = i / (BN / 2), jp = i - rb * (BN / 2);
+        const int wc = jp / (8 * NH), jw = jp - wc * (8 * NH);
+        float4 a = make_float4(0.f, 0.f, 0.f, 0.f);
+#pragma unroll
+        for (int w = 0; w < 8; ++w) {
+          const int wq_ = KG == 2 ? (w & 3) : w, g_ = KG == 2 ? (w >> 2) : 0;
+          const int wm_ = wq_ / WN, wn_ = wq_ - (wq_ / WN) * WN;
+          if (((wm_ * MT + g_ * MH) * 16) / 128 != rb || wn_ != wc) continue;
+          const float4 v = ga[w * (8 * NH) + jw];
+          a.x += v.x;
+          a.y += v.y;
+          a.z += v.z;
+          a.w += v.w;
+        }
+        gb[i] = a;
+      }
+      asm volatile("s_waitcnt lgkmcnt(0)" ::: "memory");
+      __builtin_amdgcn_s_barrier();
+      asm volatile("" ::: "memory");
+      const __attribute__((address_space(4))) unsigned char* ka =
+          (const __attribute__((address_space(4))) unsigned char*)__builtin_amdgcn_kernarg_segment_ptr();
+      asm volatile("" : "+s"(ka)::"memory");
+      using KArg = const __attribute__((address_space(4))) da_gemm_params;
+      KArg* pk = (KArg*)ka;
+      for (int c = 0; c < 2; ++c) {
+        const GnDst d = c ? GnDst{pk->gn2_out, pk->gn2_groups, pk->gn2_cpg, pk->gn2_coff}
+                          : GnDst{pk->gn_out, pk->gn_groups, pk->gn_cpg, pk->gn_coff};
+        if (!d.out) break;
+        const int cpg = d.cpg, G = d.groups;
+        const int lo = d.coff + n0, hi = d.coff + min(n0 + BN, p.N);
+        const int g0 = lo / cpg, np = (hi - 1) / cpg - g0 + 1;
+        for (int i = t; i < GN_RB * np; i += 512) {
+          const int rb = i / np, gi = g0 + (i - rb * np);
+          const int a = max(gi * cpg, lo), b = min((gi + 1) * cpg, hi);
+          const float4* src = gb + rb * (BN / 2);
+          float s1 = 0.f, s2 = 0.f;
+#pragma unroll 4
+          for (int jp = (a - lo) >> 1; jp < ((b - lo) >> 1); ++jp) {
+            const float4 v = src[jp];
+            s1 += v.x;
+            s1 += v.z;
+            s2 += v.y;
+            s2 += v.w;
+          }
+          const int piece = a > gi * cpg ? 1 : 0;
+          float2* o = (float2*)d.out + (size_t)((m0 >> 7) + rb) * 2 * G + gi;
+          o[piece * G] = make_float2(s1, s2);
+          if (!piece && (gi + 1) * cpg <= hi) o[G] = make_float2(0.f, 0.f);
+        }
+      }
+    }
+  };
   auto wide_body = [&](auto act_c, auto gate_c, auto packed_c) __attribute__((always_inline)) {
     constexpr int ACT = decltype(act_c)::value, GATE = decltype(gate_c)::value;
     constexpr bool PACKED = decltype(packed_c)::value;
@@ -920,6 +998,7 @@
 #pragma unroll
             for (int e = 0; e < 8; ++e) o[e] *= p.out_scale;
             pk.x = pack_bf2(o[0], o[1]); pk.y = pack_bf2(o[2], o[3]); pk.z = pack_bf2(o[4], o[5]); pk.w = pack_bf2(o[6], o[7]);
+            if constexpr (GNS) *(uint4*)(stg + row * ROWB + c8 * 32) = pk;
           }
           if (inside) *(uint4*)((uint16_t*)p.C + (size_t)mo * p.ldc + no) = pk;
           if constexpr (LNF) {
@@ -950,6 +1029,26 @@
             }
             asm volatile("s_waitcnt lgkmcnt(0)" ::: "memory");
           }
+        }
+        if constexpr (GNS) {
+          asm volatile("s_waitcnt lgkmcnt(0)" ::: "memory");
+#pragma unroll
+          for (int j = 0; j < GN_CJ; ++j) {
+            const int jp = min(lane + 64 * j, 8 * NH - 1);
+            const unsigned char* src = stg + (PACKED ? jp * 4 : (jp >> 2) * 32 + (jp & 3) * 4);
+            unsigned v[16];
+#pragma unroll
+            for (int r = 0; r < 16; ++r) v[r] = *(const unsigned*)(src + r * (PACKED ? ROWB / 2 : ROWB));
+#pragma unroll
+            for (int r = 0; r < 16; ++r) {
+              const float a = bf_lo(v[r]), b = bf_hi(v[r]);
+              gacc[j].x += a;
+              gacc[j].y += a * a;
+              gacc[j].z += b;
+              gacc[j].w += b * b;
+            }
+          }
+          asm volatile("s_waitcnt lgkmcnt(0)" ::: "memory");
         }
       }
     }
@@ -1031,6 +1130,7 @@
       else if (p.gate) wide_body(RT, integral_constant<int, 1>{}, std::false_type{});
       else if (packed) by_act(wide_body, G0, std::true_type{});
       else by_act(wide_body, G0, std::false_type{});
+      if constexpr (GNS) gn_epilogue();
     } else {
       if (p.gate && p.gate_f32) narrow_body(RT, integral_constant<int, 2>{});
       else if (p.gate) narrow_body(RT, integral_constant<int, 1>{});
@@ -1051,12 +1151,12 @@
 
 
 template <int KG, int WM, int WN, int MT, int NT, int NSLOT, bool CONV, bool PP = false, bool STREAMW = false, bool GIL = false,
-          bool LNF = false, int XA = 0>
+          bool LNF = false, int XA = 0, bool GNS = false>
 int launch(const da_gemm_params& p, hipStream_t s) {
   constexpr int BM = 16 * MT * WM, BN = 16 * NT * WN;
   const LaunchGeom geom = launch_geom(p, BM, BN, CONV);
   constexpr size_t lds = (size_t)NSLOT * KG * (BM + BN) * 128 + 1024 + (LNF ? 2 * BN * 4 : 0);
-  auto kern = igemm2_bf16_kernel<KG, WM, WN, MT, NT, NSLOT, CONV, PP, STREAMW, GIL, LNF, XA>;
+  auto kern = igemm2_bf16_kernel<KG, WM, WN, MT, NT, NSLOT, CONV, PP, STREAMW, GIL, LNF, XA, GNS>;
   static bool attr_set = false;
   if (!attr_set) {
     if (hipFuncSetAttribute((const void*)kern, hipFuncAttributeMaxDynamicSharedMemorySize, (int)lds) != hipSuccess)
@@ -1126,9 +1226,75 @@
   return DA_ERR_UNSUPPORTED;
 }
 
+inline int tile_bm(int tile) {
+  return (tile == DA_TILE_K1_256x128 || tile == DA_TILE_K1_256x160 || tile == DA_TILE_K1_256x256 || tile == DA_TILE_K1_256x320) ? 256
+         : tile == DA_TILE_K2_80x128 ? 80 : 128;
+}
+inline int tile_bn(int tile) {
+  switch (tile) {
+    case DA_TILE_K2_128x80: return 80;
+    case DA_TILE_K2_128x160: case DA_TILE_K1_256x160: return 160;
+    case DA_TILE_K2_128x64: return 64;
+    case DA_TILE_K1_128x320: case DA_TILE_K1_256x320: return 320;
+    case DA_TILE_K1_128x256: case DA_TILE_K1_256x256: return 256;
+    default: return 128;
+  }
+}
+
+inline bool gn_ok(const da_gemm_params& p, int tile) {
+  const int BM = tile_bm(tile), BN = tile_bn(tile);
+  const bool geglu = (p.act == DA_ACT_GEGLU || p.act == DA_ACT_GEGLU_TANH);
+  if (geglu || p.out_f32 || p.gate || (p.ldc & 7) || ((size_t)p.C & 15) || (p.N & 7) || p.stats_out || p.ln_stats || p.vt || p.xa_k ||
+      (p.residual && ((p.ldr & 7) || ((size_t)p.residual & 15))))
+    return false;
+  if (p.gn_rows <= 0 || p.gn_rows % BM || p.gn_rows % 128 || p.M % p.gn_rows) return false;
+  if (!p.gn_out) return false;
+  for (int c = 0; c < 2; ++c) {
+    const GnDst d = gn_dst(p, c);
+    if (!d.out) continue;
+    const int cpg = d.cpg, coff = d.coff;
+    if (cpg < 2 || (cpg & 1) || cpg > BN || coff < 0 || (coff & 1) || d.groups <= 0 ||
+        (long long)coff + p.N > (long long)d.groups * cpg || ((size_t)d.out & 7))
+      return false;
+    if ((coff + p.N) % cpg && p.N % BN) return false;
+  }
+  return true;
+}
+
+template <bool CONV>
+int dispatch_gn(const da_gemm_params& p, int tile, int staging, hipStream_t s) {
+  if (!gn_ok(p, tile)) return DA_ERR_UNSUPPORTED;
+  const int ns = (staging == DA_STAGE_LDS_DIRECT || staging == DA_STAGE_PINGPONG) ? 2
+                 : (staging == DA_STAGE_LDS_DIRECT3 || staging == DA_STAGE_PINGPONG3) ? 3 : 0;
+  const bool pp = staging == DA_STAGE_PINGPONG || staging == DA_STAGE_PINGPONG3;
+  if (ns == 0) return DA_ERR_UNSUPPORTED;
+  switch (tile) {
+    case DA_TILE_K2_128x80:
+      if (!pp) break;
+      return ns == 2 ? launch<2, 4, 1, 2, 5, 2, CONV, true, false, false, false, 0, true>(p, s)
+                     : launch<2, 4, 1, 2, 5, 3, CONV, true, false, false, false, 0, true>(p, s);
+    case DA_TILE_K2_128x160:
+      if (ns != 2) break;
+      return pp ? launch<2, 2, 2, 4, 5, 2, CONV, true, false, false, false, 0, true>(p, s)
+                : launch<2, 2, 2, 4, 5, 2, CONV, false, false, false, false, 0, true>(p, s);
+    case DA_TILE_K1_256x160:
+      if constexpr (CONV) {
+        if (ns == 2 && !pp) return launch<1, 4, 2, 4, 5, 2, true, false, false, false, false, 0, true>(p, s);
+      }
+      break;
+    case DA_TILE_K1_128x320:
+      if constexpr (CONV) {
+        if (ns == 2 && !pp) return launch<1, 4, 2, 2, 10, 2, true, false, false, false, false, 0, true>(p, s);
+      }
+      break;
+  }
+  return DA_ERR_UNSUPPORTED;
+}
+
 template <bool CONV>
 int dispatch(const da_gemm_params& p, int tile, int staging, hipStream_t s) {
   if (p.split_k > 1 || !staging_fits(p)) return DA_ERR_UNSUPPORTED;
+  if (p.gn_out || p.gn2_out) return dispatch_gn<CONV>(p, tile, staging, s);
   if (p.stats_out || p.ln_stats || p.vt || p.xa_k) {
     if constexpr (CONV) return DA_ERR_UNSUPPORTED;
     else return dispatch_lnf(p, tile, staging, s);
diff --git a/diffusers_amd/csrc/norm.hip b/diffusers_amd/csrc/norm.hip
--- a/diffusers_amd/csrc/norm.hip
+++ b/diffusers_amd/csrc/norm.hip
@@ -731,6 +731,28 @@
   return DA_OK;
 }
 
+extern "C" int da_groupnorm_two_pass(int B, int HW, int C, int C1, int G, int have_sync) {
+  if (B <= 0 || HW <= 0 || C <= 0 || G <= 0 || G > 64 || (C % G) || (C & 7) || C / 8 > 512) return 0;
+  if (C1 <= 0 || C1 > C) C1 = C;
+  if (gn_fused_plan(B, HW, C, C1, G, have_sync != 0).gs) return 0;
+  return (size_t)gn_plan(B, HW, C).krows * C * 2 * sizeof(float) <= 64 * 1024 ? 1 : 0;
+}
+
+extern "C" int da_groupnorm_parts_nhwc_bf16(const void* x, const void* x2, int C1, const void* gamma, const void* beta, void* y,
+                                            const void* parts, int B, int HW, int C, int G, float eps, int act, void* stream) {
+  if (!x || !gamma || !beta || !y || !parts) return DA_ERR_INVALID;
+  if (!x2) C1 = C;
+  if (C1 <= 0 || C1 > C || (C1 & 7) || (x2 == nullptr && C1 != C)) return DA_ERR_INVALID;
+  if (B <= 0 || HW <= 0 || C <= 0 || G <= 0 || G > 64 || (C % G) || (C & 7) || (HW % 128)) return DA_ERR_UNSUPPORTED;
+  if (C / 8 > 512) return DA_ERR_UNSUPPORTED;
+  const GnPlan g = gn_plan(B, HW, C);
+  DA_LAUNCH(gn_apply_kernel, dim3(g.nblk, B), dim3(g.threads), 0, (hipStream_t)stream, (const uint16_t*)x, (const uint16_t*)x2, C1,
+            (const uint16_t*)gamma, (const uint16_t*)beta, (uint16_t*)y, (const float*)parts, 2 * (HW / 128), HW, C, G, eps, act,
+            g.pix_per_blk, g.krows);
+  DA_CHECK_LAUNCH();
+  return DA_OK;
+}
+
 template <int NCH>
 __global__ __launch_bounds__(256) void rmsnorm_rows_kernel(const uint16_t* __restrict__ x, const uint16_t* __restrict__ gamma,
                                                            uint16_t* __restrict__ y, int M, int C, int ldx, int ldy, float eps) {
diff --git a/diffusers_amd/csrc/plan.hip b/diffusers_amd/csrc/plan.hip
--- a/diffusers_amd/csrc/plan.hip
+++ b/diffusers_amd/csrc/plan.hip
@@ -40,6 +40,7 @@
      "pppppiiiiiiii",
      "ppppiiiiiiiff",
      "ppppiiiiii",
+     "ppippppiiiifi",
 };
 
 struct Op {
@@ -84,6 +85,7 @@
     f(g->workspace), f(g->sync_flags);
     { void* q = g->stats_out; f(q); g->stats_out = (float*)q; }
     cf(g->ln_stats), cf(g->ln_s), cf(g->ln_c), cv(g->prefetch), f(g->vt), cv(g->xa_k), cv(g->xa_vt);
+    for (float** gp : {&g->gn_out, &g->gn2_out}) { void* q = *gp; f(q); *gp = (float*)q; }
   }
   for (auto& t : plan->attn) cv(t->q), cv(t->k), cv(t->vt), f(t->out), cv(t->bias), f(t->split_ws);
   for (auto& v : plan->ptrs)
@@ -140,6 +142,8 @@
     case DA_FN_CONV_THIN_IN:
       return da_conv_thin_in_bf16(P(0), P(1), P(2), P(3), I(4), I(5), I(6), I(7), I(8), I(9), I(10), F(11), F(12), s);
     case DA_FN_CONV_THIN_OUT: return da_conv_thin_out_bf16(P(0), P(1), P(2), P(3), I(4), I(5), I(6), I(7), I(8), I(9), s);
+    case DA_FN_GROUPNORM_PARTS_NHWC:
+      return da_groupnorm_parts_nhwc_bf16(P(0), P(1), I(2), P(3), P(4), P(5), P(6), I(7), I(8), I(9), I(10), F(11), I(12), s);
   }
 #undef P
 #undef CF
diff --git a/diffusers_amd/layers.py b/diffusers_amd/layers.py
--- a/diffusers_amd/layers.py
+++ b/diffusers_amd/layers.py
@@ -90,8 +90,15 @@
         self.bias = w.get(prefix + ".bias")
         self.groups, self.eps = groups, eps
 
-    def __call__(self, x, silu=False, x2=None):
+    def __call__(self, x, silu=False, x2=None, stats=None):
+        if stats is not None:
+            return ops.group_norm_nhwc(x, self.weight, self.bias, self.groups, self.eps, silu=silu, x2=x2, stats=stats)
         return ops.group_norm_nhwc(x, self.weight, self.bias, self.groups, self.eps, silu=silu, x2=x2)
+
+
+def gn_kw(targets) -> dict:
+    t = [(s, off) for s, off in (targets or ()) if s is not None]
+    return {"gn_out": t} if t else {}
 
 
 class LayerNorm:
@@ -117,8 +124,8 @@
         self.shortcut = Conv1x1(w, prefix + ".conv_shortcut") if w.has(prefix + ".conv_shortcut.weight") else None
         self.out_scale = 1.0 / output_scale_factor
 
-    def __call__(self, x, temb=None, skip=None):
-        h = self.norm1(x, silu=True, x2=skip)
+    def __call__(self, x, temb=None, skip=None, stats=None, out_gn=None):
+        h = self.norm1(x, silu=True, x2=skip, stats=stats)
         tvec = None
         if self.has_temb and temb is not None:
             if isinstance(temb, ProjectedTemb):
@@ -127,15 +134,16 @@
                 raise ValueError("ResnetBlock2D: this block's time_emb_proj lives in the model's TimeProjections; pass its output")
             else:
                 tvec = ops.linear_small_m(temb, self.time_emb_proj.weight, self.time_emb_proj.bias, act_in=L.ACT_SILU)
-        h = self.conv1(h, rowvec=tvec)
-        h = self.norm2(h, silu=True)
+        n2 = ops.gn_stats_for(x.shape[0], x.shape[1] * x.shape[2], self.conv1.weight.shape[0], self.norm2.groups, x.device)
+        h = self.conv1(h, rowvec=tvec, **gn_kw([(n2, 0)]))
+        h = self.norm2(h, silu=True, stats=n2)
         if self.shortcut is not None:
             res = self.shortcut(x, x2=skip)
         else:
             if skip is not None:
                 raise ValueError("ResnetBlock2D: concat input requires a conv_shortcut")
             res = x
-        return self.conv2(h, residual=res, out_scale=self.out_scale)
+        return self.conv2(h, residual=res, out_scale=self.out_scale, **gn_kw(out_gn))
 
 
 class ProjectedTemb:
@@ -176,10 +184,14 @@
         self.conv = Conv3x3(w, prefix + ".conv")
         self.padding = padding
 
-    def __call__(self, x):
+    def out_hw(self, h: int, w: int):
+        pad, after = (1, 0) if self.padding == 1 else (0, 1)
+        return (h + 2 * pad + after - 3) // 2 + 1, (w + 2 * pad + after - 3) // 2 + 1
+
+    def __call__(self, x, out_gn=None):
         if self.padding == 1:
-            return self.conv(x, stride=2)
-        return self.conv(x, stride=2, pad=0, pad_after=1)
+            return self.conv(x, stride=2, **gn_kw(out_gn))
+        return self.conv(x, stride=2, pad=0, pad_after=1, **gn_kw(out_gn))
 
 
 class Upsample2D:
@@ -187,8 +199,8 @@
     def __init__(self, w: Weights, prefix: str):
         self.conv = Conv3x3(w, prefix + ".conv")
 
-    def __call__(self, x):
-        return self.conv(x, up=True)
+    def __call__(self, x, out_gn=None):
+        return self.conv(x, up=True, **gn_kw(out_gn))
 
 
 class CrossKV:
@@ -387,10 +399,10 @@
     def precompute_kv(self, ehs_pad, batch, skv, skv_alloc, bias=None):
         return [blk.attn2.precompute_kv(ehs_pad, batch, skv, skv_alloc, bias) for blk in self.blocks]
 
-    def __call__(self, x, kvs):
+    def __call__(self, x, kvs, stats=None, out_gn=None):
         B, H, W_, C = x.shape
         res = x.view(B * H * W_, C)
-        h = self.norm(x).view(B * H * W_, C)
+        h = self.norm(x, stats=stats).view(B * H * W_, C)
         chain = bool(ops.LN_FOLD) and ops.LN_FOLD_NORM1 and all(b.folds_norm1 for b in self.blocks)
         st = ops.RowStats(h.shape[0], h.device) if chain else None
         h = ops.linear(h, self.proj_in_w, self.proj_in_b, stats_out=st)
@@ -398,7 +410,7 @@
             nxt = ops.RowStats(h.shape[0], h.device) if chain and i + 1 < len(self.blocks) else None
             h = blk(h, B, H * W_, kv, stats_in=st, stats_out=nxt)
             st = nxt
-        h = ops.linear(h, self.proj_out_w, self.proj_out_b, residual=res)
+        h = ops.linear(h, self.proj_out_w, self.proj_out_b, residual=res, **gn_kw(out_gn))
         return h.view(B, H, W_, C)
 
 
diff --git a/diffusers_amd/ops.py b/diffusers_amd/ops.py
--- a/diffusers_amd/ops.py
+++ b/diffusers_amd/ops.py
@@ -1,6 +1,7 @@
 from __future__ import annotations
 
 import ctypes as C
+import inspect
 import os
 import threading
 import weakref
@@ -148,6 +149,80 @@
         self.parts = 0
 
 
+GN_FOLD = os.environ.get("DIFFUSERS_AMD_GN_FOLD", "1") == "1"
+
+
+class GNStats:
+
+    __slots__ = ("buf", "B", "HW", "C", "groups", "covered")
+
+    def __init__(self, B: int, HW: int, C: int, groups: int, device):
+        nbytes = int(L.load().da_gemm_gn_parts_bytes(B * HW, groups)) if HW % 128 == 0 else 0
+        self.buf = torch.empty((nbytes // 4,), device=device, dtype=torch.float32) if nbytes else None
+        self.B, self.HW, self.C, self.groups = B, HW, C, groups
+        self.covered = 0
+
+    @property
+    def complete(self) -> bool:
+        return self.buf is not None and self.covered == self.C
+
+
+_accepts_cache: dict = {}
+
+
+def accepts(fn, name: str) -> bool:
+    key = (fn, name)
+    r = _accepts_cache.get(key)
+    if r is None:
+        try:
+            ps = inspect.signature(fn).parameters
+            r = name in ps or any(q.kind == inspect.Parameter.VAR_KEYWORD for q in ps.values())
+        except (TypeError, ValueError):
+            r = False
+        _accepts_cache[key] = r
+    return r
+
+
+def gn_stats_for(B: int, HW: int, C: int, groups: int, device, C1: int = 0) -> Optional[GNStats]:
+    g = globals()
+    if not (GN_FOLD and accepts(g["conv2d_nhwc"], "gn_out") and accepts(g["linear"], "gn_out")
+            and accepts(g["group_norm_nhwc"], "stats")):
+        return None
+    if HW % 128 or C % groups:
+        return None
+    sync = GN_MULTI and B * HW * C >= (1 << 20)
+    if not L.load().da_groupnorm_two_pass(B, HW, C, C1 or C, groups, int(sync)):
+        return None
+    st = GNStats(B, HW, C, groups, device)
+    return st if st.buf is not None else None
+
+
+def _gn_targets(gn_out, M: int):
+    if not gn_out:
+        return ()
+    t = tuple((s, int(off)) for s, off in gn_out if s is not None and s.buf is not None and s.B * s.HW == M)
+    if len(t) > 2:
+        raise ValueError("gn_out: at most two GroupNorm consumers per launch")
+    return t
+
+
+_GN_FIELDS = (("gn_out", "gn_groups", "gn_cpg", "gn_coff"), ("gn2_out", "gn2_groups", "gn2_cpg", "gn2_coff"))
+
+
+def _set_gn(p: "L.GemmParams", targets, rows: int) -> None:
+    for names, (s, off) in zip(_GN_FIELDS, targets):
+        for n, v in zip(names, (s.buf.data_ptr(), s.groups, s.C // s.groups, off)):
+            setattr(p, n, v)
+    p.gn_rows = rows if targets else 0
+
+
+def _clear_gn(p: "L.GemmParams") -> None:
+    for names in _GN_FIELDS:
+        for n, v in zip(names, (None, 0, 0, 0)):
+            setattr(p, n, v)
+    p.gn_rows = 0
+
+
 def geglu_fold_on_k3(rows: int, n_packed: int, k: int) -> bool:
     if not (LN_FOLD_K3 and TUNING) or rows % 256 or n_packed % 320:
         return False
@@ -196,12 +271,18 @@
 DA_ERR_UNSUPPORTED = 3
 
 
-def _launch_gemm(p: "L.GemmParams", st: int, what: str) -> None:
+def _launch_gemm(p: "L.GemmParams", st: int, what: str, gn=()) -> None:
     rc = L.load().da_gemm_bf16(C.byref(p), st)
+    if rc == DA_ERR_UNSUPPORTED and gn:
+        _clear_gn(p)
+        gn = ()
+        rc = L.load().da_gemm_bf16(C.byref(p), st)
     if rc == DA_ERR_UNSUPPORTED and getattr(p, "_auto", False) and p.tile != L.TILE_AUTO:
         p.tile, p.staging, p.split_k = L.TILE_AUTO, L.STAGE_LDS_DIRECT, 1
         rc = L.load().da_gemm_bf16(C.byref(p), st)
     L.check(rc, what)
+    for s, _ in gn:
+        s.covered += p.N
 
 
 def _ptr(t: Optional[torch.Tensor]) -> Optional[int]:
@@ -295,14 +376,16 @@
            tile: Optional[int] = None, staging: Optional[int] = None, split_k: Optional[int] = None,
            stats_out: Optional[RowStats] = None, ln: Optional[tuple] = None, k_valid: int = 0,
            prefetch: Optional[torch.Tensor] = None, vt_out: Optional[tuple] = None,
-           xattn: Optional[dict] = None) -> torch.Tensor:
+           xattn: Optional[dict] = None, gn_out=None) -> torch.Tensor:
     p, st = _linear_params(x, w, bias, act=act, residual=residual, rowvec=rowvec, rows_per_batch=rows_per_batch,
                            alpha=alpha, out_scale=out_scale, out=out, out_f32=out_f32, bias_rows=bias_rows, gate=gate,
                            tile=tile, staging=staging, split_k=split_k, stats_out=stats_out, ln=ln, k_valid=k_valid,
                            prefetch=prefetch, vt_out=vt_out, xattn=xattn)
     if p is None:
         return st
-    _launch_gemm(p, st, "da_gemm_bf16(linear)")
+    gn = _gn_targets(gn_out, p.M)
+    _set_gn(p, gn, gn[0][0].HW if gn else 0)
+    _launch_gemm(p, st, "da_gemm_bf16(linear)", gn)
     return p._out
 
 
@@ -447,7 +530,7 @@
                 rowvec: Optional[torch.Tensor] = None, residual: Optional[torch.Tensor] = None,
                 out_scale: float = 1.0, act: int = L.ACT_NONE, tile: Optional[int] = None,
                 staging: Optional[int] = None, pad_after: int = 0, out: Optional[torch.Tensor] = None,
-                split_k: Optional[int] = None, k_valid: int = 0) -> torch.Tensor:
+                split_k: Optional[int] = None, k_valid: int = 0, gn_out=None) -> torch.Tensor:
     _req(x, "x"), _req(w, "w")
     if x2 is not None:
         _req(x2, "x2")
@@ -479,7 +562,9 @@
     _prefetch_hook(p, x, w)
     st = _stream()
     _select_variant(p, tile, staging, st, inplace=inplace, split_k=split_k, device=x.device)
-    _launch_gemm(p, st, "da_gemm_bf16(conv)")
+    gn = _gn_targets(gn_out, p.M)
+    _set_gn(p, gn, Hout * Wout)
+    _launch_gemm(p, st, "da_gemm_bf16(conv)", gn)
     return out
 
 
@@ -629,7 +714,7 @@
 
 
 def group_norm_nhwc(x: torch.Tensor, gamma: torch.Tensor, beta: torch.Tensor, groups: int, eps: float,
-                    silu: bool = False, x2: Optional[torch.Tensor] = None) -> torch.Tensor:
+                    silu: bool = False, x2: Optional[torch.Tensor] = None, stats: Optional[GNStats] = None) -> torch.Tensor:
     _req(x, "x"), _req(gamma, "gamma"), _req(beta, "beta")
     if not x.is_contiguous() or (x2 is not None and not x2.is_contiguous()):
         raise ValueError("group_norm_nhwc: contiguous channels-last input required")
@@ -638,6 +723,12 @@
     Ctot = C1 + (x2.shape[-1] if x2 is not None else 0)
     HW = x.numel() // (B * C1)
     lib = L.load()
+    if stats is not None and stats.complete and (stats.B, stats.HW, stats.C, stats.groups) == (B, HW, Ctot, groups):
+        y = torch.empty(tuple(x.shape[:-1]) + (Ctot,), device=x.device, dtype=bf16)
+        L.check(lib.da_groupnorm_parts_nhwc_bf16(x.data_ptr(), _ptr(x2), C1, gamma.data_ptr(), beta.data_ptr(), y.data_ptr(),
+                                                 stats.buf.data_ptr(), B, HW, Ctot, groups, eps,
+                                                 L.ACT_SILU if silu else L.ACT_NONE, _stream()), "da_groupnorm_parts_nhwc_bf16")
+        return y
     nbytes = lib.da_groupnorm_workspace_bytes(B, HW, Ctot, groups)
     ws = torch.empty((max(nbytes, 4) // 4,), device=x.device, dtype=torch.float32)
     y = torch.empty(tuple(x.shape[:-1]) + (Ctot,), device=x.device, dtype=bf16)
diff --git a/diffusers_amd/unet_2d_condition.py b/diffusers_amd/unet_2d_condition.py
--- a/diffusers_amd/unet_2d_condition.py
+++ b/diffusers_amd/unet_2d_condition.py
@@ -287,18 +287,53 @@
 
         x = ops.conv_thin_in(sample.contiguous(), self.conv_in_w, self.conv_in_b, ksize=3, in_nchw=True)
 
+        up_rn = [rn for st_ in self.up for rn in st_["resnets"]]
+        n_skips = 1 + sum(len(st_["resnets"]) + (st_["down"] is not None) for st_ in self.down)
+        use_gn = (down_block_additional_residuals is None and mid_block_additional_residual is None and len(up_rn) == n_skips)
+        dev = x.device
+
+        def gn_for(norm, B_, HW, C_, C1=0):
+            return ops.gn_stats_for(B_, HW, C_, norm.groups, dev, C1) if use_gn else None
+
+        def skip_target(k, B_, HW, Cs):
+            rn_ = up_rn[n_skips - 1 - k]
+            Ct = rn_.norm1.weight.numel()
+            return gn_for(rn_.norm1, B_, HW, Ct, Ct - Cs), Ct - Cs
+
         ki = 0
-        skips = [x]
-        for st in self.down:
+        skips, skip_st = [x], [(None, 0)]
+        x_st = None
+        for si, st in enumerate(self.down):
             for j, rn in enumerate(st["resnets"]):
-                x = rn(x, emb)
+                B_, H_, W_ = x.shape[:3]
+                Co = rn.conv2.weight.shape[0]
+                if j + 1 < len(st["resnets"]):
+                    nxt = st["resnets"][j + 1].norm1
+                else:
+                    nxt = None if st["down"] is not None else self.mid["resnets"][0].norm1
+                nxt_st = gn_for(nxt, B_, H_ * W_, Co) if nxt is not None else None
+                sk = skip_target(len(skips), B_, H_ * W_, Co)
                 if st["attns"]:
-                    x = st["attns"][j](x, kvs[ki])
+                    a = st["attns"][j]
+                    a_st = gn_for(a.norm, B_, H_ * W_, Co)
+                    x = rn(x, emb, stats=x_st, out_gn=[(a_st, 0)])
+                    x = a(x, kvs[ki], stats=a_st, out_gn=[(nxt_st, 0), sk])
                     ki += 1
+                else:
+                    x = rn(x, emb, stats=x_st, out_gn=[(nxt_st, 0), sk])
+                x_st = nxt_st
                 skips.append(x)
+                skip_st.append(sk)
             if st["down"] is not None:
-                x = st["down"](x)
+                B_, H_, W_ = x.shape[:3]
+                Ho, Wo = st["down"].out_hw(H_, W_)
+                Co = st["down"].conv.weight.shape[0]
+                nxt_st = gn_for(self.down[si + 1]["resnets"][0].norm1, B_, Ho * Wo, Co) if si + 1 < len(self.down) else None
+                sk = skip_target(len(skips), B_, Ho * Wo, Co)
+                x = st["down"](x, out_gn=[(nxt_st, 0), sk])
+                x_st = nxt_st
                 skips.append(x)
+                skip_st.append(sk)
 
         if down_block_additional_residuals is not None:
             if len(down_block_additional_residuals) != len(skips):
@@ -306,24 +341,42 @@
                                  f"{len(down_block_additional_residuals)}")
             skips = [s_ + self._nhwc(r, s_) for s_, r in zip(skips, down_block_additional_residuals)]
 
-        x = self.mid["resnets"][0](x, emb)
-        x = self.mid["attns"][0](x, kvs[ki])
+        B_, H_, W_, Cm = x.shape
+        r0, r1 = self.mid["resnets"]
+        a_st = gn_for(self.mid["attns"][0].norm, B_, H_ * W_, Cm)
+        r1_st = gn_for(r1.norm1, B_, H_ * W_, Cm)
+        x = r0(x, emb, stats=x_st, out_gn=[(a_st, 0)])
+        x = self.mid["attns"][0](x, kvs[ki], stats=a_st, out_gn=[(r1_st, 0)])
         ki += 1
-        x = self.mid["resnets"][1](x, emb)
+        x = r1(x, emb, stats=r1_st, out_gn=[(skip_st[-1][0], 0)])
         if mid_block_additional_residual is not None:
             x = x + self._nhwc(mid_block_additional_residual, x)
 
-        for st in self.up:
+        for si, st in enumerate(self.up):
             for j, rn in enumerate(st["resnets"]):
                 skip = skips.pop()
-                x = rn(x, emb, skip=skip)
+                x_st = skip_st.pop()[0]
+                B_, H_, W_ = x.shape[:3]
+                Co = rn.conv2.weight.shape[0]
+                if j + 1 < len(st["resnets"]):
+                    nxt_st = skip_st[-1][0]
+                elif st["up"] is not None:
+                    nxt_st = None
+                else:
+                    nxt_st = gn_for(self.conv_norm_out, B_, H_ * W_, Co)
                 if st["attns"]:
-                    x = st["attns"][j](x, kvs[ki])
+                    a = st["attns"][j]
+                    a_st = gn_for(a.norm, B_, H_ * W_, Co)
+                    x = rn(x, emb, skip=skip, stats=x_st, out_gn=[(a_st, 0)])
+                    x = a(x, kvs[ki], stats=a_st, out_gn=[(nxt_st, 0)])
                     ki += 1
+                else:
+                    x = rn(x, emb, skip=skip, stats=x_st, out_gn=[(nxt_st, 0)])
+                x_st = nxt_st
             if st["up"] is not None:
-                x = st["up"](x)
-
-        x = self.conv_norm_out(x, silu=True)
+                x = st["up"](x, out_gn=[(skip_st[-1][0] if skip_st else None, 0)])
+
+        x = self.conv_norm_out(x, silu=True, stats=x_st)
         out = ops.conv_thin_out(x, self.conv_out_w, self.conv_out_b)
         if not return_dict:
             return (out,)
diff --git a/include/diffusers_amd.h b/include/diffusers_amd.h
--- a/include/diffusers_amd.h
+++ b/include/diffusers_amd.h
@@ -57,7 +57,7 @@
 #define DA_STAGE_PINGPONG 6
 #define DA_STAGE_PINGPONG3 7
 
-#define DA_ABI_VERSION 6
+#define DA_ABI_VERSION 7
 int da_version(void);
 size_t da_sizeof_gemm_params(void);
 size_t da_sizeof_attention_params(void);
@@ -110,9 +110,15 @@
   int xa_skv, xa_skv_alloc, xa_k_ld;
   long long xa_vt_ld;
   float xa_scale;
+  float* gn_out;
+  int gn_groups, gn_cpg, gn_coff;
+  float* gn2_out;
+  int gn2_groups, gn2_cpg, gn2_coff;
+  int gn_rows;
 } da_gemm_params;
 
 int da_gemm_stats_parts(const da_gemm_params* p);
+size_t da_gemm_gn_parts_bytes(int M, int G);
 
 int da_conv_chunk_channels(const da_gemm_params* p, int tile);
 
@@ -156,6 +162,9 @@
 
 size_t da_groupnorm_workspace_bytes(int B, int HW, int C, int G);
 size_t da_groupnorm_sync_bytes(void);
+int da_groupnorm_two_pass(int B, int HW, int C, int C1, int G, int have_sync);
+int da_groupnorm_parts_nhwc_bf16(const void* x, const void* x2, int C1, const void* gamma, const void* beta, void* y,
+                                 const void* parts, int B, int HW, int C, int G, float eps, int act, void* stream);
 int da_groupnorm_nhwc_bf16(const void* x, const void* x2, int C1, const void* gamma, const void* beta, void* y,
                            void* workspace, int B, int HW, int C, int G, float eps, int act, void* sync, void* stream);
 int da_rmsnorm_bf16(const void* x, const void* gamma, void* y, int M, int C, int ldx, int ldy, float eps, void* stream);
@@ -257,7 +266,8 @@
 #define DA_FN_LINEAR_SMALL_M 29
 #define DA_FN_CONV_THIN_IN 30
 #define DA_FN_CONV_THIN_OUT 31
-#define DA_FN_COUNT 32
+#define DA_FN_GROUPNORM_PARTS_NHWC 32
+#define DA_FN_COUNT 33
 #define DA_PLAN_MAX_ARGS 16
 
 typedef struct da_plan_op {
```

New measurement: 1.027, median of 6. Within noise of the previous version (+0.4%).
